# RunpeiDong/ACT

Hardware: AMD Instinct MI355X
Metric: stage2_pretrain_point_clouds_per_sec (higher is better)
Workload: dtype f32

## Files before the change

### act_amd/_abi.py

```python
import ctypes

_vp, _i, _f, _sz = ctypes.c_void_p, ctypes.c_int, ctypes.c_float, ctypes.c_size_t
_u, _u64, _ll, _str = ctypes.c_uint, ctypes.c_uint64, ctypes.c_longlong, ctypes.c_char_p
_d = ctypes.c_double
_P = ctypes.POINTER


class GemmEpilogue(ctypes.Structure):
    _fields_ = [("alpha", _f), ("act", _i), ("accumulate", _i), ("rows_per_scale", _i), ("ldr", _i), ("ldaux", _i),
                ("res_row_div", _i), ("bias", _vp), ("rowscale", _vp), ("res", _vp), ("aux", _vp)]


class GemmTnProblem(ctypes.Structure):
    _fields_ = [("A", _vp), ("lda", _i), ("B", _vp), ("ldb", _i), ("C", _vp), ("ldc", _i), ("M", _i), ("N", _i), ("bias_out", _vp)]


class GemmFx(ctypes.Structure):
    _fields_ = ([(n, _vp) for n in ("a_scale", "a_shift", "b_scale", "b_shift", "tile_stats", "gmax", "garg")] + [("group", _i), ("store_c", _i)]
                + [(n, _vp) for n in ("sa_src", "sa_arg", "ep_src", "ep_arg", "row_groups")])


class BlockParams(ctypes.Structure):
    _fields_ = [(n, _vp) for n in ("norm1_w", "norm1_b", "qkv_w", "qkv_b", "proj_w", "proj_b", "norm2_w", "norm2_b",
                                   "fc1_w", "fc1_b", "fc2_w", "fc2_b")]


class BlockDims(ctypes.Structure):
    _fields_ = [("B", _i), ("S", _i), ("D", _i), ("heads", _i), ("hidden", _i), ("eps", _f)]


class BlockStack(ctypes.Structure):
    _fields_ = [("depth", _i), ("blocks", _vp), ("gate1", _vp), ("gate2", _vp)]


class PrefixVit(ctypes.Structure):
    _fields_ = ([(n, _i) for n in ("B", "P", "G", "D", "heads", "hidden", "depth", "tokens_dims", "pos_hidden")] +
                [("eps", _f), ("drop_p", _f), ("seed_base", _u64), ("seed_dev", _vp)] +
                [(n, _vp) for n in ("pos_w0", "pos_b0", "pos_w1", "pos_b1", "pre_w", "pre_b", "post_w", "post_b", "norm_w", "norm_b")] +
                [("prompt_tok", _P(_vp)), ("prompt_pos", _P(_vp)), ("blocks", _P(BlockParams))])


class VitBf16x3(ctypes.Structure):
    _fields_ = [("w_planes", _vp), ("a_planes", _vp), ("a_planes_elems", _sz)]


class VitF16x3(ctypes.Structure):
    _fields_ = [("w_planes", _vp), ("w_inv_scale", _vp), ("a_scale", _vp), ("a_planes", _vp), ("a_planes_elems", _sz)]


class PointnetParams(ctypes.Structure):
    _fields_ = [(n, _vp) for n in ("c1_w", "c1_b", "bn1_w", "bn1_b", "c2_w", "c2_b", "c3_w", "c3_b", "bn2_w", "bn2_b", "c4_w", "c4_b",
                                   "bn1_mean", "bn1_var", "bn2_mean", "bn2_var")]


class PointnetGrads(ctypes.Structure):
    _fields_ = [(n, _vp) for n in ("c1_w", "c1_b", "bn1_w", "bn1_b", "c2_w", "c2_b", "c3_w", "c3_b", "bn2_w", "bn2_b", "c4_w", "c4_b")]


class PointnetDims(ctypes.Structure):
    _fields_ = [("BG", _i), ("n", _i), ("C", _i), ("eps1", _f), ("eps2", _f), ("momentum1", _f), ("momentum2", _f)]


class Dgcnn(ctypes.Structure):
    _fields_ = ([(n, _i) for n in ("B", "G", "k", "Cin", "Cout", "groups")] + [("eps", _f), ("slope", _f)] +
                [(n, _vp) for n in ("w_in", "b_in", "w5")] + [("stacked", _vp * 4), ("gn_w", _vp * 4), ("gn_b", _vp * 4)])


class DgcnnF16x3(ctypes.Structure):
    _fields_ = [("w5_planes", _vp), ("w5_inv_scale", _vp), ("a_scale", _f), ("a_planes", _vp), ("a_planes_elems", _sz), ("layers", _i),
                ("st_planes", _vp * 3), ("st_inv_scale", _vp * 3)]


class PointnetF16x3(ctypes.Structure):
    _fields_ = [("c4_planes", _vp), ("c4_inv_scale", _vp), ("a_scale", _f)]


class AugmentOp(ctypes.Structure):
    _fields_ = [("kind", _i), ("p0", _f), ("p1", _f), ("p2", _f), ("draws", _vp), ("draws2", _vp)]


STRUCTS = {
    "act_gemm_epilogue_t": GemmEpilogue, "act_gemm_tn_problem_t": GemmTnProblem, "act_gemm_fx_t": GemmFx,
    "act_block_params_t": BlockParams, "act_block_grads_t": BlockParams, "act_block_dims_t": BlockDims, "act_block_stack_t": BlockStack,
    "act_prefix_vit_t": PrefixVit, "act_vit_bf16x3_t": VitBf16x3, "act_vit_f16x3_t": VitF16x3,
    "act_pointnet_params_t": PointnetParams,
    "act_pointnet_grads_t": PointnetGrads, "act_pointnet_dims_t": PointnetDims, "act_dgcnn_t": Dgcnn, "act_dgcnn_f16x3_t": DgcnnF16x3,
    "act_pointnet_f16x3_t": PointnetF16x3,
    "act_augment_op_t": AugmentOp,
}

_epi, _probs, _fx = _P(GemmEpilogue), _P(GemmTnProblem), _P(GemmFx)
_dims, _blk, _x3 = _P(BlockDims), _P(BlockParams), _P(VitBf16x3)
_pnd, _pnp = _P(PointnetDims), _P(PointnetParams)

_TABLE = {
    "act_version": [],
    "act_arch": (_str, []),
    "act_prof_enable": [_i],
    "act_prof_reset": [],
    "act_prof_num_kernels": [],
    "act_prof_kernel_name": (_str, [_i]),
    "act_prof_read": [_i, _vp, _vp, _vp, _vp],
    "act_fps_scratch_floats": (_sz, [_i, _i]),
    "act_fps_f32": [_vp, _i, _i, _i, _vp, _vp, _i, _vp, _vp],
    "act_fps_chain_probe": [_i, _i, _vp, _vp, _vp, _vp],
    "act_knn_group_f32": [_vp, _vp, _i, _i, _i, _i, _vp, _i, _vp, _vp, _vp],
    "act_gather_points_f32": [_vp, _vp, _i, _i, _i, _i, _vp, _vp],
# ... 39 lines not shown
    "act_col_mean_var_f32": [_vp, _i, _i, _vp, _vp, _vp, _sz, _vp],
    "act_bn_bwd_sums_f32": [_vp, _vp, _vp, _vp, _vp, _vp, _i, _i, _i, _vp, _vp, _vp, _sz, _vp],
    "act_bn_bwd_apply_f32": [_vp, _vp, _vp, _vp, _vp, _vp, _vp, _vp, _f, _i, _i, _i, _vp, _vp],
    "act_group_max_f32": [_vp, _i, _i, _i, _vp, _vp, _vp],
    "act_group_max_bwd_f32": [_vp, _vp, _i, _i, _i, _i, _vp, _vp],
    "act_group_max_bwd_matmul_f32": [_vp, _vp, _i, _i, _i, _vp, _i, _i, _vp, _i, _vp],
    "act_group_live_i32": [_vp, _i, _i, _vp, _vp],
    "act_group_max_bwd_matmul_live_f32": [_vp, _vp, _i, _i, _i, _vp, _i, _i, _vp, _i, _vp, _vp],
    "act_group_max_bwd_wgrad_workspace": (_sz, [_i, _i, _i, _i]),
    "act_group_max_bwd_wgrad_f32": [_vp, _vp, _i, _i, _i, _vp, _i, _i, _vp, _vp, _vp, _i, _vp, _sz, _vp],
    "act_group_sum_f32": [_vp, _i, _i, _i, _vp, _vp],
    "act_edge_gn_lrelu_max_f32": [_vp, _i, _i, _vp, _i, _i, _i, _i, _i, _vp, _vp, _f, _f, _vp, _vp, _i, _i, _vp],
    "act_edge_gn_lrelu_max_bwd_f32": [_vp, _i, _i, _vp, _i, _i, _i, _i, _i, _vp, _vp, _vp, _f, _vp, _i, _vp, _vp, _vp, _vp],
    "act_edge_bwd_lds": [_i],
    "act_gn_gumbel_argmax_gather_f32": [_vp, _i, _i, _i, _i, _vp, _vp, _f, _f, _vp, _u64, _vp, _f, _vp, _i, _vp, _vp, _vp, _vp, _vp],
    "act_gumbel_softmax_fwd_f32": [_vp, _i, _i, _vp, _u64, _f, _vp, _vp],
    "act_gumbel_softmax_bwd_f32": [_vp, _vp, _i, _i, _f, _vp, _vp],
    "act_kl_uniform_fwd_f32": [_vp, _i, _i, _i, _vp, _vp, _vp, _vp],
    "act_kl_uniform_bwd_f32": [_vp, _vp, _vp, _vp, _i, _i, _i, _vp, _vp],
    "act_split_bf16x2_f32": [_vp, _i, _i, _i, _vp, _vp, _vp],
    "act_sgemm_nt_bf16x3_supported": [_i, _i, _i],
    "act_sgemm_nt_bf16x3_f32": [_i, _i, _i, _vp, _vp, _vp, _vp, _vp, _i, _epi, _vp],
    "act_layernorm_fwd_planes_f32": [_vp, _vp, _vp, _vp, _vp, _vp, _vp, _vp, _vp, _vp, _i, _i, _f, _vp],
    "act_prompt_layernorm_fwd_planes_f32": [_vp, _vp, _i, _i, _i, _f, _u64, _vp, _vp, _vp, _f, _vp, _vp, _vp],
    "act_attention_fwd_prefix_planes_f32": [_vp, _i, _vp, _i, _vp, _vp, _vp, _vp, _i, _i, _i, _f, _vp],
    "act_sgemm_nt_bf16x3_planes_f32": [_i, _i, _i, _vp, _vp, _vp, _vp, _vp, _i, _vp, _vp, _epi, _vp],
    "act_split_f16x2_f32": [_vp, _i, _i, _i, _f, _vp, _vp, _vp, _vp],
    "act_split_f16x2_ld_f32": [_vp, _i, _i, _i, _f, _vp, _vp, _i, _vp],
    "act_sgemm_nt_f16x3_supported": [_i, _i, _i],
    "act_sgemm_nt_f16x3_planes_f32": [_i, _i, _i, _vp, _vp, _f, _vp, _vp, _vp, _vp, _i, _vp, _vp, _f, _epi, _vp],
    "act_sgemm_nt_f16x3_pick_tile": [_i, _i, _i, _i],
    "act_sgemm_nt_f16x3_planes_tile_f32": [_i, _i, _i, _vp, _vp, _f, _vp, _vp, _vp, _vp, _i, _vp, _vp, _f, _epi, _vp, _i],
    "act_sgemm_nt_f16x3_planes_lda_f32": [_i, _i, _i, _vp, _vp, _i, _f, _vp, _vp, _vp, _vp, _i, _vp, _vp, _f, _epi, _vp, _i],
    "act_layernorm_fwd_f16_planes_f32": [_vp, _vp, _vp, _vp, _vp, _vp, _vp, _vp, _f, _vp, _vp, _i, _i, _f, _vp],
    "act_attention_fwd_prefix_f16_planes_f32": [_vp, _i, _vp, _i, _vp, _vp, _vp, _f, _vp, _i, _i, _i, _f, _vp],
    "act_prompt_layernorm_fwd_f16_planes_f32": [_vp, _vp, _i, _i, _i, _f, _u64, _vp, _vp, _vp, _f, _vp, _vp, _f, _vp],
    "act_split_f16x2_affine_relu_f32": [_vp, _i, _i, _i, _vp, _vp, _f, _vp, _vp, _vp],
    "act_sgemm_nt_f16x3_gmax_supported": [_i, _i, _i, _i],
    "act_sgemm_nt_f16x3_gmax_pick_tile": [_i, _i, _i, _i],
    "act_sgemm_nt_f16x3_gmax_f32": [_i, _i, _i, _vp, _i, _vp, _vp, _vp, _vp, _f, _vp, _vp, _vp, _vp, _i, _vp, _i, _i, _vp],
    "act_gemm_tune_set": [_i] * 7,
    "act_gemm_tune_get": [_i] * 5 + [_P(_i), _P(_i)],
    "act_gemm_tune_clear": [],
    "act_gemm_tile_info": [_i] + [_P(_i)] * 4,
    "act_scale_rows_f32": [_vp, _vp, _i, _i, _i, _vp, _vp],
    "act_bn_eval_affine_f32": [_vp, _vp, _vp, _vp, _f, _i, _vp, _vp, _vp],
    "act_composite_collect_begin": [],
    "act_composite_collect_end": [_P(_i), _i],
    "act_composite_shutdown": [],
    "act_block_saved_floats": (_sz, [_dims]),
    "act_block_fwd_f32": [_dims, _blk, _vp, _vp, _vp, _vp, _i, _vp, _vp, _vp, _sz, _vp],
    "act_block_bwd_scratch_floats": (_sz, [_dims]),
    "act_block_bwd_f32": [_dims, _blk, _vp, _vp, _vp, _vp, _vp, _blk, _vp, _vp, _sz, _vp, _sz, _vp, _vp],
    "act_block_stack_saved_floats": (_sz, [_dims, _i, _i]),
    "act_block_stack_bwd_scratch_floats": (_sz, [_dims, _i]),
    "act_block_stack_fwd_f32": [_dims, _P(BlockStack), _vp, _vp, _i, _vp, _vp, _vp, _sz, _vp],
    "act_block_stack_bwd_f32": [_dims, _P(BlockStack), _vp, _vp, _vp, _vp, _vp, _vp, _vp, _vp, _sz, _vp, _sz, _vp, _vp],
    "act_add_f32": [_vp, _vp, _vp, _ll, _vp],
    "act_prefix_block_saved_floats": (_sz, [_dims, _i]),
    "act_prefix_block_fwd_f32": [_dims, _i, _blk, _vp, _vp, _vp, _vp, _i, _vp, _vp, _vp, _sz, _vp],
    "act_prefix_block_fwd_kv_f32": [_dims, _i, _blk, _vp, _vp, _vp, _vp, _vp, _vp, _sz, _vp],
    "act_prompt_kv_sparse": [_i],
    "act_prompt_kv_workspace": (_sz, [_i, _i, _i, _i]),
    "act_prompt_kv_fwd_f32": [_vp, _vp, _i, _i, _i, _i, _f, _u64, _vp, _vp, _vp, _f, _vp, _vp, _vp, _vp, _sz, _vp, _sz, _vp],
    "act_prompt_kv_f16x3": [_i],
    "act_prompt_kv_fwd_f16x3_f32": [_vp, _vp, _i, _i, _i, _i, _f, _u64, _vp, _vp, _vp, _f, _vp, _vp, _vp, _f, _vp, _vp, _vp, _sz, _i, _vp],
    "act_prefix_block_bwd_scratch_floats": (_sz, [_dims, _i]),
    "act_prefix_block_bwd_f32": [_dims, _i, _blk, _vp, _vp, _vp, _vp, _vp, _vp, _vp, _sz, _vp],
    "act_prefix_vit_scratch_floats": (_sz, [_P(PrefixVit)]),
    "act_prefix_vit_fwd_bf16x3_f32": [_P(PrefixVit), _x3, _vp, _vp, _vp, _vp, _vp, _sz, _vp],
    "act_prefix_block_fwd_bf16x3_f32": [_dims, _i, _blk, _x3, _vp, _vp, _vp, _i, _vp, _vp, _vp, _sz, _vp],
    "act_prefix_block_bwd_bf16x3_f32": [_dims, _i, _blk, _x3, _vp, _vp, _vp, _vp, _vp, _vp, _vp, _sz, _vp],
    "act_prefix_vit_fwd_f32": [_P(PrefixVit), _vp, _vp, _vp, _vp, _vp, _sz, _vp],
    "act_prefix_vit_fwd_f16x3_f32": [_P(PrefixVit), _P(VitF16x3), _vp, _vp, _vp, _vp, _vp, _sz, _vp],
    "act_pointnet_saved_floats": (_sz, [_pnd]),
    "act_pointnet_fwd_f32": [_pnd, _pnp, _vp, _i, _i, _vp, _vp, _vp, _sz, _vp],
    "act_pointnet_fwd_groups_f32": [_pnd, _pnp, _vp, _i, _i, _vp, _vp, _vp, _i, _vp, _sz, _vp],
    "act_pointnet_fwd_groups_f16x3_f32": [_pnd, _pnp, _P(PointnetF16x3), _vp, _i, _i, _vp, _vp, _vp, _i, _vp, _sz, _vp],
    "act_pointnet_bwd_scratch_floats": (_sz, [_pnd]),
    "act_pointnet_bwd_f32": [_pnd, _pnp, _vp, _vp, _vp, _P(PointnetGrads), _vp, _vp, _sz, _vp],
    "act_dgcnn_scratch_floats": (_sz, [_P(Dgcnn)]),
    "act_dgcnn_features_f32": [_P(Dgcnn), _vp, _vp, _vp, _vp, _vp, _sz, _vp],
    "act_dgcnn_features_f16x3_f32": [_P(Dgcnn), _P(DgcnnF16x3), _vp, _vp, _vp, _vp, _vp, _sz, _vp],
    "act_log_softmax_fwd_f32": [_vp, _ll, _i, _vp, _vp],
    "act_log_softmax_bwd_f32": [_vp, _vp, _ll, _i, _vp, _vp],
    "act_nll_weighted_workspace": (_sz, [_ll]),
    "act_nll_weighted_fwd_f32": [_vp, _vp, _vp, _ll, _i, _vp, _vp, _vp, _vp, _sz, _vp],
    "act_nll_weighted_bwd_f32": [_vp, _vp, _vp, _vp, _ll, _i, _vp, _vp],
    "act_confusion_i64": [_vp, _vp, _ll, _i, _vp, _vp],
    "act_label_branch_fwd_f32": [_vp, _vp, _vp, _vp, _i, _i, _f, _f, _f, _vp, _vp, _vp, _vp],
    "act_label_branch_bwd_f32": [_vp, _vp, _vp, _vp, _vp, _i, _f, _f, _vp, _vp, _vp, _vp],
    "act_part_eval_f32": [_vp, _vp, _i, _i, _i, _vp, _vp, _i, _vp, _vp, _i, _i, _vp, _vp, _vp],
    "act_scene_member_workspace": (_sz, [_ll, _i, _i]),
    "act_scene_member_count": [_vp, _ll, _vp, _i, _i, _vp, _vp, _vp, _sz, _vp],
    "act_scene_member_fill": [_vp, _ll, _vp, _i, _i, _vp, _vp, _vp, _sz, _vp],
    "act_scene_rows": [_vp, _vp, _vp, _vp, _i, _ll, _i, _u, _u, _u, _vp, _vp],
    "act_scene_gather": [_vp, _ll, _vp, _vp, _vp, _vp, _i, _ll, _vp, _vp],
    "act_scene_vote": [_vp, _vp, _ll, _ll, _i, _vp, _vp, _vp, _vp],
    "act_scene_finish": [_vp, _vp, _ll, _i, _vp, _vp, _vp],
# ... 82 lines not shown
```

### act_amd/composite.py

```python
import ctypes
import math
import os
import weakref

import torch

from . import _C
from . import kernels as K
from ._abi import BlockDims, BlockParams, BlockStack, Dgcnn, PointnetDims, PointnetGrads, PointnetParams, PrefixVit, VitBf16x3, VitF16x3, DgcnnF16x3
from ._abi import PointnetF16x3
from ._abi import GemmFx

lib, check = _C.lib, _C.check
_vp, _i = ctypes.c_void_p, ctypes.c_int

ENABLED = os.environ.get("ACT_COMPOSITE", "1") != "0"


def _p(t):
    if t is None:
        return None
    if not t.is_cuda or not t.is_contiguous():
        raise _C.ActHipError("act_amd kernels need contiguous CUDA tensors (there is no CPU fallback)")
    _C._same_device(t)
# ... 198 lines not shown
        if dpos_in is not None:
            dpos_in = K._f32c(dpos_in).reshape(B * S, D)
        dpos = torch.empty(B, S, D, dtype=torch.float32, device=dev) if (ctx.has_pos and (depth > 1 or dpos_in is not None)) else None
        scratch = torch.empty(n_scratch, dtype=torch.float32, device=dev)
        grads, garr = (None,) * len(params), None
        if tw:
            grads = tuple(torch.empty_like(t) if t is not None else None for t in params)
            garr = _ptr_array(grads, dev.index)
        ws = K.workspace(dev)
        side, sws = None, None
        if tw == 2 and K.OVERLAP_DW:
            side = K.side_stream(dev, 1).cuda_stream
            sws = K.workspace(dev, stream_handle=side)
        args = (ctypes.byref(dims), ctypes.byref(st), saved.data_ptr(), dout.data_ptr(), dx.data_ptr(), dpos.data_ptr() if dpos is not None else None,
                dpos_in.data_ptr() if (dpos_in is not None and dpos is not None) else None,
                ctypes.cast(garr, _vp) if garr is not None else None, scratch.data_ptr(), ws.data_ptr(), ws.numel() * 4,
                sws.data_ptr() if sws is not None else None, (sws.numel() * 4 if sws is not None else 0))
        ensure_tuned(("stack_bwd", B, S, D, heads, hidden, depth, bool(tw)), lambda: lib.act_block_stack_bwd_f32(*args, _C.stream(), side), dev)
        check(lib.act_block_stack_bwd_f32(*args, _C.stream(), side), "act_block_stack_bwd_f32")
        return (dx, (dpos if dpos is not None else dx) if ctx.has_pos else None, None, None, None, None, None) + grads


_LEAVES = weakref.WeakKeyDictionary()
_VIT_LEAVES = weakref.WeakKeyDictionary()
_VIT_STRUCT = weakref.WeakKeyDictionary()
_VIT_PLANES = weakref.WeakKeyDictionary()
TEACHER_BF16X3 = os.environ.get("ACT_TEACHER_BF16X3", "0") == "1"
TEACHER_BF16X3_BWD = os.environ.get("ACT_TEACHER_BF16X3_BWD", "1") == "1"
TEACHER_F16X3 = os.environ.get("ACT_TEACHER_F16X3", "1") != "0"
_VIT_F16 = weakref.WeakKeyDictionary()
TOKENIZER_F16X3 = os.environ.get("ACT_TOKENIZER_F16X3", "1") != "0"
TOKENIZER_PN_F16X3 = os.environ.get("ACT_TOKENIZER_PN_F16X3", "1") != "0"
TOKENIZER_DGCNN_F16X3 = os.environ.get("ACT_TOKENIZER_DGCNN_F16X3", "1") != "0"
DGCNN_F16X3_MIN_T = 4096
_PN_F16 = weakref.WeakKeyDictionary()
_DGCNN_F16 = weakref.WeakKeyDictionary()


def _stack_leaves(blocks):
    cache = _LEAVES.get(blocks)
    if cache is None or len(cache) != len(blocks) or any(c[6] is not b for c, b in zip(cache, blocks)):
        cache = _LEAVES[blocks] = [(b.norm1, b.attn.qkv, b.attn.proj, b.norm2, b.mlp.fc1, b.mlp.fc2, b) for b in blocks]
    return cache


def _stock_blocks(blocks):
    from act_amd.models.act import Block
    for b in blocks:
        if type(b).forward is not Block.forward or b._forward_hooks or b._forward_pre_hooks or b._backward_hooks or b._backward_pre_hooks:
            return False
    return True


def block_stack(blocks, x, pos, gates, draws=None, tag="enc", chunk=None, taps=False):
    n = len(blocks)

    def per_block(x, draws):
        outs = []
        every = chunk if chunk else n
        for i, blk in enumerate(blocks):
            x = blk(x, pos, draws, f"{tag}.{i}", gates[i] if gates is not None else None)
            if (i + 1) % every == 0 or i == n - 1:
                outs.append(x)
        return outs if taps else x
    if not (ENABLED and STACK) or n == 0 or not _stock_blocks(blocks):
        return per_block(x, draws)
# ... 204 lines not shown
    if cache is None or cache[0] != sig:
        with torch.no_grad():
            planes = [K.split_bf16x2(w.detach()) for w in ws_]
        parr = (_vp * len(planes))(*[pl.data_ptr() for pl in planes])
        cache = _VIT_PLANES[tok] = (sig, planes, parr)
    a_planes = torch.empty(2 * act_elems, dtype=torch.bfloat16, device=dev)
    x3 = VitBf16x3(ctypes.cast(cache[2], _vp), a_planes.data_ptr(), a_planes.numel())
    return x3, (a_planes, cache)


def f16x3_act_scale(bound):
    bound = float(bound)
    if not math.isfinite(bound) or bound > 32768.0:
        return 0.0
    if bound < 2.0 ** -15:
        return 2.0 ** 30
    s = 2.0 ** (math.frexp(32768.0 / bound)[1] - 1)
    return s if bound * s <= 32768.0 else s / 2


def f16x3_vit_bounds(ts, depth, D):
    rows, rt = [], math.sqrt(D)
    for i in range(depth):
        n1w, n1b, wqkv, bqkv, _, _, n2w, n2b, w1, b1 = (None if t is None else t.detach().double() for t in ts[10 + _NPB * i: 20 + _NPB * i])
        u1, u2 = rt * n1w.abs() + n1b.abs(), rt * n2w.abs() + n2b.abs()
        v = wqkv[2 * D:].abs() @ u1 + (bqkv[2 * D:].abs() if bqkv is not None else 0)
        h = w1.abs() @ u2 + (b1.abs() if b1 is not None else 0)
        rows.append(torch.stack([u1.max(), v.max(), u2.max(), h.max()]))
    return torch.stack(rows)


def _vit_f16_planes(tok, ts, depth, act_elems, dev):
    blk = ts[10:10 + _NPB * depth]
    sig = tuple((t.data_ptr(), t._version) if t is not None else None for t in blk)
    cache = _VIT_F16.get(tok)
    if cache is None or cache[0] != sig:
        ws_ = [ts[10 + _NPB * i + j] for i in range(depth) for j in (2, 4, 8, 10)]
        with torch.no_grad():
            scales = [K.f16x3_row_scales(w) for w in ws_]
            planes = [K.split_f16x2(w.detach(), 1.0, sc[0]) for w, sc in zip(ws_, scales)]
            inv = [sc[1].contiguous() for sc in scales]
            a_scale = [f16x3_act_scale(b) for b in f16x3_vit_bounds(ts, depth, ws_[0].shape[1]).flatten().tolist()]
        parr = (_vp * len(planes))(*[pl.data_ptr() for pl in planes])
        iarr = (_vp * len(inv))(*[t.data_ptr() for t in inv])
        sarr = (ctypes.c_float * len(a_scale))(*a_scale)
        cache = _VIT_F16[tok] = (sig, planes, inv, a_scale, (parr, iarr, sarr))
    a_planes = torch.empty(2 * act_elems, dtype=torch.float16, device=dev)
    parr, iarr, sarr = cache[4]
    x3 = VitF16x3(ctypes.cast(parr, _vp), ctypes.cast(iarr, _vp), ctypes.cast(sarr, _vp), a_planes.data_ptr(), a_planes.numel())
    return x3, (a_planes, cache)


def _pointnet_structs(enc, BG, n):
    c1, bn1, _, c2 = enc.first_conv
    c3, bn2, _, c4 = enc.second_conv
    dims = PointnetDims(BG, n, c4.weight.shape[0], float(bn1.eps), float(bn2.eps), float(bn1.momentum), float(bn2.momentum))
    return dims, (c1, bn1, c2, c3, bn2, c4)


class PointnetFn(torch.autograd.Function):

    @staticmethod
    def forward(ctx, x, c1w, c1b, g1, b1, c2w, c2b, c3w, c3b, g2, b2, c4w, c4b, buffers, dims, training, groups=None, x3=None):
        dev = x.device
        x = K._f32c(x)
        need_grad = any(ctx.needs_input_grad)
        prm = PointnetParams(*[_p(t) for t in (c1w, c1b, g1, b1, c2w, c2b, c3w, c3b, g2, b2, c4w, c4b) + tuple(buffers)])
        saved = torch.empty(int(lib.act_pointnet_saved_floats(ctypes.byref(dims))), dtype=torch.float32, device=dev)
        out = torch.empty(dims.BG, dims.C, dtype=torch.float32, device=dev)
        ws = K.workspace(dev)
        ng = 0 if groups is None else int(groups.numel())
        args = (ctypes.byref(dims), ctypes.byref(prm), _p(x), int(training), int(need_grad), _p(saved), _p(out),
                _p(groups) if ng else None, ng, _p(ws), ws.numel() * 4)
        ensure_tuned(("pn_fwd", dims.BG, dims.n, dims.C, ng), lambda: lib.act_pointnet_fwd_groups_f32(*args, _C.stream()), dev)
        if x3 is not None and not need_grad:
            check(lib.act_pointnet_fwd_groups_f16x3_f32(args[0], args[1], ctypes.byref(x3), *args[2:], _C.stream()), "act_pointnet_fwd_groups_f16x3_f32")
        else:
            check(lib.act_pointnet_fwd_groups_f32(*args, _C.stream()), "act_pointnet_fwd_groups_f32")
        if need_grad:
            ctx.save_for_backward(x, saved, c1w, c1b, g1, b1, c2w, c2b, c3w, c3b, g2, b2, c4w, c4b)
            ctx.dims, ctx.training = dims, bool(training)
        return out

    @staticmethod
    def backward(ctx, dout):
        if not ctx.training:
            raise NotImplementedError("mini-PointNet backward in eval mode (running statistics) is off the training path")
        x, saved = ctx.saved_tensors[:2]
        params = ctx.saved_tensors[2:]
        dims = ctx.dims
        dev = dout.device
        dout = K._f32c(dout)
        prm = PointnetParams(*([_p(t) for t in params] + [None] * 4))
        grads = tuple(torch.empty_like(t) for t in params)
        gp = PointnetGrads(*[_p(g) for g in grads])
        scratch = torch.empty(int(lib.act_pointnet_bwd_scratch_floats(ctypes.byref(dims))), dtype=torch.float32, device=dev)
        ws = K.workspace(dev)
        args = (ctypes.byref(dims), ctypes.byref(prm), _p(x), _p(saved), _p(dout), ctypes.byref(gp), _p(scratch), _p(ws), ws.numel() * 4)
        ensure_tuned(("pn_bwd", dims.BG, dims.n, dims.C), lambda: lib.act_pointnet_bwd_f32(*args, _C.stream()), dev)
        check(lib.act_pointnet_bwd_f32(*args, _C.stream()), "act_pointnet_bwd_f32")
        return (None,) + grads + (None, None, None, None, None)


def f16x3_pointnet_bound(gmax, bmax, R):
    return math.sqrt(R) * gmax + bmax


def _pointnet_f16_planes(enc, R):
    bn2, c4 = enc.second_conv[1], enc.second_conv[3]
    sig = tuple((t.data_ptr(), t._version) for t in (c4.weight, bn2.weight, bn2.bias))
    cache = _PN_F16.get(enc)
    if cache is None or cache[0] != sig:
        with torch.no_grad():
            w = c4.weight.detach().reshape(c4.weight.shape[0], c4.weight.shape[1])
            scale, inv = K.f16x3_row_scales(w)
            planes = K.split_f16x2(w, 1.0, scale)
            inv = inv.contiguous()
            gmax, bmax = torch.stack([bn2.weight.detach().double().abs().max(), bn2.bias.detach().double().abs().max()]).tolist()
        cache = _PN_F16[enc] = (sig, planes, inv, gmax, bmax, {})
    _, planes, inv, gmax, bmax, scales = cache
    a_scale = scales.get(R)
    if a_scale is None:
        a_scale = scales[R] = f16x3_act_scale(f16x3_pointnet_bound(gmax, bmax, R))
    return PointnetF16x3(planes.data_ptr(), inv.data_ptr(), a_scale), cache


def pointnet_forward(enc, point_groups, need=None):
    bs, g, n, _ = point_groups.shape
    groups = None
    if need is not None and need.shape[1] < g and n in (32, 64):
        ids = (need + torch.arange(bs, device=need.device).unsqueeze(1) * g).reshape(-1).to(torch.int32)
        pad = (-ids.numel()) % (128 // n)
        groups = torch.cat([ids, ids[-1:].expand(pad)]) if pad else ids
        groups = groups.contiguous()
    dims, (c1, bn1, c2, c3, bn2, c4) = _pointnet_structs(enc, bs * g, n)
    training = enc.training
    if training:
        for bn in (bn1, bn2):
            if bn.num_batches_tracked is not None:
                bn.num_batches_tracked.add_(1)
    w2 = lambda c: c.weight.view(c.weight.shape[0], c.weight.shape[1])
    x3 = keep = None
    if (TOKENIZER_PN_F16X3 and groups is None and training and not torch.is_grad_enabled()
            and not any(p.requires_grad for p in enc.parameters())):
        x3, keep = _pointnet_f16_planes(enc, bs * g * n)
    out = PointnetFn.apply(point_groups.reshape(bs * g * n, 3), w2(c1), c1.bias, bn1.weight, bn1.bias, w2(c2), c2.bias, w2(c3), c3.bias,
                           bn2.weight, bn2.bias, w2(c4), c4.bias,
                           (bn1.running_mean, bn1.running_var, bn2.running_mean, bn2.running_var), dims, training, groups, x3)
    del keep
    return out.reshape(bs, g, dims.C)


def dgcnn_features(dg, f, idx, stacked):
    B, G, Cin = f.shape
    dev = f.device
    w5 = dg.layer5[0].weight
    m = Dgcnn()
    gn0 = dg.layer1[1]
    m.B, m.G, m.k, m.Cin, m.Cout, m.groups = B, G, idx.shape[1], Cin, w5.shape[0], gn0.num_groups
    m.eps, m.slope = float(gn0.eps), 0.2
    m.w_in, m.b_in, m.w5 = _p(dg.input_trans.weight), _p(dg.input_trans.bias), _p(w5)
    for l, layer in enumerate((dg.layer1, dg.layer2, dg.layer3, dg.layer4)):
        m.stacked[l], m.gn_w[l], m.gn_b[l] = _p(stacked[l]), _p(layer[1].weight), _p(layer[1].bias)
    scratch = torch.empty(int(lib.act_dgcnn_scratch_floats(ctypes.byref(m))), dtype=torch.float32, device=dev)
    h = torch.empty(B * G, m.Cout, dtype=torch.float32, device=dev)
    ws = K.workspace(dev)
    f = K._f32c(f)
    args = (ctypes.byref(m), _p(f), _p(idx), _p(h), _p(scratch), _p(ws), ws.numel() * 4)
    ensure_tuned(("dgcnn", B, G, Cin, m.Cout), lambda: lib.act_dgcnn_features_f32(*args, _C.stream()), dev)
    head, layers = TOKENIZER_F16X3 and m.Cout >= 1024, TOKENIZER_DGCNN_F16X3 and B * G >= DGCNN_F16X3_MIN_T
    if head or layers:
        x3, keep = _dgcnn_f16_planes(dg, B * G, G, m.k, dev, head=head, layers=layers)
        check(lib.act_dgcnn_features_f16x3_f32(args[0], ctypes.byref(x3), *args[1:], _C.stream()), "act_dgcnn_features_f16x3_f32")
        del keep
        return h
    check(lib.act_dgcnn_features_f32(*args, _C.stream()), "act_dgcnn_features_f32")
    return h


def f16x3_dgcnn_bound(gmax, bmax, couts, groups, G, k):
    return max(math.sqrt((c // g) * G * k) * gm + bm for gm, bm, c, g in zip(gmax, bmax, couts, groups))


def _dgcnn_f16_planes(dg, T, G, k, dev, head=True, layers=None):
    if layers is None:
        layers = TOKENIZER_DGCNN_F16X3 and T >= DGCNN_F16X3_MIN_T
    convs = [layer[0] for layer in (dg.layer2, dg.layer3, dg.layer4)]
    gns = [layer[1] for layer in (dg.layer1, dg.layer2, dg.layer3, dg.layer4)]
    w5 = dg.layer5[0].weight
    sig = tuple((t.data_ptr(), t._version) for t in [w5] + [t for gn in gns for t in (gn.weight, gn.bias)] + [c.weight for c in convs])
    cache = _DGCNN_F16.get(dg)
    if cache is None or cache[0] != sig:
        with torch.no_grad():
            mx = torch.stack([t.detach().double().abs().max() for gn in gns for t in (gn.weight, gn.bias)]).tolist()
        cache = _DGCNN_F16[dg] = [sig, None, None, mx[0::2], mx[1::2], [gn.num_channels for gn in gns], [gn.num_groups for gn in gns], {}, None]

    def planes_of(w):
        scale, inv = K.f16x3_row_scales(w)
        return K.split_f16x2(w, 1.0, scale), inv.contiguous()
    if head and cache[1] is None:
        with torch.no_grad():
            cache[1], cache[2] = planes_of(w5.detach().reshape(w5.shape[0], w5.shape[1]))
    if layers and cache[8] is None:
        with torch.no_grad():
            cache[8] = [planes_of(dg._stacked_weight(c).detach()) for c in convs]
    _, planes, inv, gmax, bmax, couts, groups, scales, st = cache
    a_scale = scales.get((G, k))
    if a_scale is None:
        a_scale = scales[(G, k)] = f16x3_act_scale(f16x3_dgcnn_bound(gmax, bmax, couts, groups, G, k))
    a_planes = torch.empty(2 * T * sum(couts), dtype=torch.float16, device=dev)
    x3 = DgcnnF16x3(planes.data_ptr() if head else None, inv.data_ptr() if head else None, a_scale, a_planes.data_ptr(), a_planes.numel())
    if layers:
        x3.layers = 1
        for i, (p, v) in enumerate(st):
            x3.st_planes[i], x3.st_inv_scale[i] = p.data_ptr(), v.data_ptr()
    return x3, (a_planes, cache)
```

### act_amd/csrc/composite.hip

```cpp
#include "common.h"
#include "split_planes.h"
#include <atomic>
#include <mutex>
#include <unordered_map>
#include <vector>
#include <stdlib.h>

#define CK(expr) do { const int rc__ = (expr); if (rc__ != 0) return rc__; } while (0)
#define RUN(expr) do { if (!t_collect) { const int rc__ = (expr); if (rc__ != 0) return rc__; } } while (0)

namespace {

struct GemmShape { int ak, bk, M, N, K; };
thread_local std::vector<GemmShape>* t_collect = nullptr;
inline bool collecting(int ak, int bk, int M, int N, int K) {
    if (!t_collect) return false;
    t_collect->push_back({ak, bk, M, N, K});
    return true;
}

struct EventRing {
    std::vector<hipEvent_t> ev;
    size_t next = 0;
    hipEvent_t get() {
// ... 57 lines not shown
    return c.used;
}
struct BlockBwdScratch { float *dy2, *dh, *dn2, *dx1, *dy1, *datt, *dqkv, *dn1; };
size_t carve_block_bwd(float* base, const act_block_dims_t& d, BlockBwdScratch& sc) {
    const size_t T = (size_t)d.B * d.S, D = d.D, Hd = d.hidden;
    Carver c(base);
    sc.dy2 = c.take(T * D); sc.dh = c.take(T * Hd); sc.dn2 = c.take(T * D); sc.dx1 = c.take(T * D); sc.dy1 = c.take(T * D);
    sc.datt = c.take(T * D); sc.dqkv = c.take(T * 3 * D); sc.dn1 = c.take(T * D);
    return c.used;
}
bool bad_dims(const act_block_dims_t* d) {
    return !d || d->B <= 0 || d->S <= 0 || d->D <= 0 || d->heads <= 0 || d->D % d->heads || d->hidden <= 0;
}

struct PrefixSaved { float *n1p, *meanp, *rstdp, *kvp, *xin, *n1x, *mean1, *rstd1, *qkvx, *att, *lse, *x1, *n2, *mean2, *rstd2, *hpre, *a; };
size_t carve_prefix(float* base, const act_block_dims_t& d, int P, PrefixSaved& sv) {
    const size_t TG = (size_t)d.B * d.S, TP = (size_t)d.B * P, D = d.D, Hd = d.hidden;
    Carver c(base);
    sv.n1p = c.take(TP * D); sv.kvp = c.take(TP * 2 * D); sv.xin = c.take(TG * D); sv.n1x = c.take(TG * D); sv.qkvx = c.take(TG * 3 * D);
    sv.att = c.take(TG * D); sv.x1 = c.take(TG * D); sv.n2 = c.take(TG * D); sv.hpre = c.take(TG * Hd); sv.a = c.take(TG * Hd);
    sv.meanp = c.take(TP); sv.rstdp = c.take(TP); sv.mean1 = c.take(TG); sv.rstd1 = c.take(TG); sv.mean2 = c.take(TG); sv.rstd2 = c.take(TG);
    sv.lse = c.take((size_t)d.B * d.heads * d.S);
    return c.used;
}
struct PrefixBwdScratch { float *dh, *dn2, *dx1, *datt, *dkvp, *dqkvx, *dn1x, *dn1p; };
size_t carve_prefix_bwd(float* base, const act_block_dims_t& d, int P, PrefixBwdScratch& sc) {
    const size_t TG = (size_t)d.B * d.S, TP = (size_t)d.B * P, D = d.D, Hd = d.hidden;
    Carver c(base);
    sc.dh = c.take(TG * Hd); sc.dn2 = c.take(TG * D); sc.dx1 = c.take(TG * D); sc.datt = c.take(TG * D); sc.dkvp = c.take(TP * 2 * D);
    sc.dqkvx = c.take(TG * 3 * D); sc.dn1x = c.take(TG * D); sc.dn1p = c.take(TP * D);
    return c.used;
}

struct X3Linear { const uint16_t *w1, *w2; const float* inv; PlaneFmt a_fmt; };
inline X3Linear x3_linear_of(const uint16_t* planes, size_t plane_elems, PlaneFmt a_fmt, const float* inv = nullptr) {
    return X3Linear{planes, planes ? planes + plane_elems : nullptr, inv, a_fmt};
}
inline bool x3_takes(const X3Linear& l, int M, int N, int K) {
    return l.w1 && (l.a_fmt.is_f16() ? act_sgemm_nt_f16x3_supported(M, N, K) : act_sgemm_nt_bf16x3_supported(M, N, K));
}
int x3_split(PlaneFmt fmt, const float* A, int M, int K, uint16_t* dst, hipStream_t s) {
    if (fmt.is_f16()) return act_split_f16x2_f32(A, M, K, K, fmt.f16_scale, nullptr, dst, dst + (size_t)M * K, s);
    return act_split_bf16x2_f32(A, M, K, K, dst, dst + (size_t)M * K, s);
}
int x3_multiply(const X3Linear& l, int M, int N, int K, const uint16_t* a, float* C, uint16_t* emit, PlaneFmt emit_fmt, const act_gemm_epilogue_t& e,
                hipStream_t s) {
    const uint16_t* a2 = a + (size_t)M * K; uint16_t* emit2 = emit ? emit + (size_t)M * N : nullptr;
    if (l.a_fmt.is_f16())
        return act_sgemm_nt_f16x3_planes_f32(M, N, K, a, a2, l.a_fmt.f16_scale, l.w1, l.w2, l.inv, emit ? nullptr : C, N, emit, emit2,
                                             emit ? emit_fmt.f16_scale : 0.f, &e, s);
    return act_sgemm_nt_bf16x3_planes_f32(M, N, K, a, a2, l.w1, l.w2, emit ? nullptr : C, N, emit, emit2, &e, s);
}
int x3_linear(const X3Linear& l, int M, int N, int K, const float* A, const uint16_t* pre, uint16_t* stage, float* C, uint16_t* emit, PlaneFmt emit_fmt,
              const act_gemm_epilogue_t& e, hipStream_t s) {
    if (t_collect) return 0;
    if (!pre) CK(x3_split(l.a_fmt, A, M, K, stage, s));
    return x3_multiply(l, M, N, K, pre ? pre : stage, C, emit, emit_fmt, e, s);
}
int x3_layernorm(PlaneFmt fmt, const float* x, const float* pos, const float* gamma, const float* beta, float* xin_out, uint16_t* dst, float* mean, float* rstd,
                 int T, int D, float eps, hipStream_t s) {
    uint16_t* dst2 = dst + (size_t)T * D;
    if (fmt.is_f16()) return act_layernorm_fwd_f16_planes_f32(x, pos, gamma, beta, xin_out, nullptr, dst, dst2, fmt.f16_scale, mean, rstd, T, D, eps, s);
    return act_layernorm_fwd_planes_f32(x, pos, gamma, beta, xin_out, nullptr, dst, dst2, mean, rstd, T, D, eps, s);
}
int x3_attention(PlaneFmt fmt, const float* kvp, int P, const float* qkvx, int G, float* att, uint16_t* dst, float* lse, int B, int H, int hd, hipStream_t s) {
    uint16_t* dst2 = dst + (size_t)B * G * H * hd;
    if (fmt.is_f16()) return act_attention_fwd_prefix_f16_planes_f32(kvp, P, qkvx, G, att, dst, dst2, fmt.f16_scale, lse, B, H, hd, attn_scale(hd), s);
    return act_attention_fwd_prefix_planes_f32(kvp, P, qkvx, G, att, dst, dst2, lse, B, H, hd, attn_scale(hd), s);
}

struct X3Block { X3Linear kv, qkv, proj, fc1, fc2; uint16_t* a_planes; size_t a_elems; bool n1p_is_planes; };
inline X3Block x3_block_bf16(const act_block_dims_t& d, const uint16_t* const* w_planes, uint16_t* a_planes, size_t a_elems) {
    const size_t D = d.D, Hd = d.hidden; const PlaneFmt bf = PlaneFmt::bf16();
    X3Block b{};
    b.qkv = x3_linear_of(w_planes[0], 3 * D * D, bf); b.proj = x3_linear_of(w_planes[1], D * D, bf);
    b.fc1 = x3_linear_of(w_planes[2], Hd * D, bf); b.fc2 = x3_linear_of(w_planes[3], D * Hd, bf);
    if (b.qkv.w1) b.kv = X3Linear{b.qkv.w1 + D * D, b.qkv.w2 + D * D, nullptr, bf};
    b.a_planes = a_planes; b.a_elems = a_elems;
    return b;
}
inline bool x3_fits(const act_block_dims_t& d, int P, size_t a_elems) {
    const size_t TG = (size_t)d.B * d.S, TP = (size_t)d.B * P;
    return a_elems >= 2 * TG * d.hidden + 2 * (TG > TP ? TG : TP) * d.D;
}
constexpr int kPromptKvTile = 0;

int prefix_block_core(const act_block_dims_t& d, int P, const act_block_params_t& w, const float* x, const float* pos, const float* n1p,
                      bool keep, PrefixSaved& sv, float* out, float* ws, size_t wsb, hipStream_t s, const X3Block* x3 = nullptr, bool kvp_ready = false) {
    const int B = d.B, G = d.S, D = d.D, H = d.heads, hd = D / H, Hd = d.hidden, TG = B * G, TP = B * P;
    static const X3Block none{};
    const X3Block& b = (x3 && x3_fits(d, P, x3->a_elems)) ? *x3 : none;
    uint16_t* tmp =b.a_planes ? b.a_planes + (size_t)2 * TG * Hd : nullptr;
    uint16_t* qkv_in = x3_takes(b.qkv, TG, 3 * D, D) ? tmp : nullptr;
    uint16_t* proj_in = x3_takes(b.proj, TG, D, D) ? tmp : nullptr;
    uint16_t* fc1_in = x3_takes(b.fc1, TG, Hd, D) ? tmp : nullptr;
    uint16_t* fc2_in = (fc1_in && x3_takes(b.fc2, TG, D, Hd)) ? b.a_planes : nullptr;
    const X3Linear fc2 = fc2_in ? b.fc2 : X3Linear{};
    auto linear = [&](const X3Linear& l, int M, int N, int K, const float* A, const float* W, float* C, const act_gemm_epilogue_t& e,
                      const uint16_t* pre = nullptr, uint16_t* emit = nullptr, const X3Linear* next = nullptr) -> int {
        if (x3_takes(l, M, N, K)) return x3_linear(l, M, N, K, A, pre, tmp, C, emit, next ? next->a_fmt : PlaneFmt::bf16(), e, s);
        return gemm_nt(M, N, K, A, K, W, K, C, N, e, ws, wsb, s);
    };
    float *mean1 = keep ? sv.mean1 : nullptr, *rstd1 = keep ? sv.rstd1 : nullptr, *mean2 = keep ? sv.mean2 : nullptr, *rstd2 = keep ? sv.rstd2 : nullptr;
    float* lse = keep ? sv.lse : nullptr;
    act_gemm_epilogue_t e = epi0();
    e.bias = w.qkv_b ? w.qkv_b + D : nullptr;
    if (!kvp_ready) CK(linear(b.kv, TP, 2 * D, D, n1p, w.qkv_w + (size_t)D * D, sv.kvp, e, b.n1p_is_planes ? tmp : nullptr));
    RUN(qkv_in ? x3_layernorm(b.qkv.a_fmt, x, pos, w.norm1_w, w.norm1_b, sv.xin, qkv_in, mean1, rstd1, TG, D, d.eps, s)
               : act_layernorm_fwd_f32(x, pos, w.norm1_w, w.norm1_b, sv.xin, sv.n1x, mean1, rstd1, TG, D, d.eps, s));
    e = epi0(); e.bias = w.qkv_b;
    CK(linear(b.qkv, TG, 3 * D, D, sv.n1x, w.qkv_w, sv.qkvx, e, qkv_in));
    RUN(proj_in ? x3_attention(b.proj.a_fmt, sv.kvp, P, sv.qkvx, G, keep ? sv.att : nullptr, proj_in, lse, B, H, hd, s)
                : act_attention_fwd_prefix_f32(sv.kvp, P, sv.qkvx, G, sv.att, lse, B, H, hd, attn_scale(hd), s));
    e = epi0(); e.bias = w.proj_b; e.res = sv.xin; e.ldr = D;
    CK(linear(b.proj, TG, D, D, sv.att, w.proj_w, sv.x1, e, proj_in));
    RUN(fc1_in ? x3_layernorm(b.fc1.a_fmt, sv.x1, nullptr, w.norm2_w, w.norm2_b, nullptr, fc1_in, mean2, rstd2, TG, D, d.eps, s)
               : act_layernorm_fwd_f32(sv.x1, nullptr, w.norm2_w, w.norm2_b, nullptr, sv.n2, mean2, rstd2, TG, D, d.eps, s));
    e = epi0(); e.bias = w.fc1_b; e.act = ACT_EPI_GELU; e.aux = keep ? sv.hpre : nullptr; e.ldaux = Hd;
    CK(linear(b.fc1, TG, Hd, D, sv.n2, w.fc1_w, sv.a, e, fc1_in, fc2_in, &fc2));
    e = epi0(); e.bias = w.fc2_b; e.res = sv.x1; e.ldr = D;
    CK(linear(fc2, TG, D, Hd, sv.a, w.fc2_w, out, e, fc2_in));
    return 0;
}

}

extern "C" {

int act_composite_shutdown(void) {
    std::lock_guard<std::mutex> g(g_ring_mu);
    int n = 0;
    for (auto& kv : g_rings)
        for (hipEvent_t e : kv.second.ev) { (void)hipEventDestroy(e); ++n; }
    g_rings.clear();
    return n;
}

int act_composite_collect_begin(void) {
    if (t_collect) return ACT_E_BADARG;
    t_collect = new std::vector<GemmShape>();
    return 0;
}
int act_composite_collect_end(int* shapes, int max) {
    if (!t_collect) return ACT_E_BADARG;
    const int n = (int)t_collect->size();
    for (int i = 0; i < n && i < max && shapes; ++i) {
        const GemmShape& g = (*t_collect)[i];
        shapes[5 * i] = g.ak; shapes[5 * i + 1] = g.bk; shapes[5 * i + 2] = g.M; shapes[5 * i + 3] = g.N; shapes[5 * i + 4] = g.K;
    }
    delete t_collect; t_collect = nullptr;
    return n;
}

size_t act_block_saved_floats(const act_block_dims_t* d) {
// ... 181 lines not shown
    if (!w || !x || !saved || !out || !kvp) return ACT_E_NULLPTR;
    if (bad_dims(d) || P <= 0) return ACT_E_BADARG;
    PrefixSaved sv; carve_prefix(saved, *d, P, sv);
    sv.kvp = const_cast<float*>(kvp);
    return prefix_block_core(*d, P, *w, x, pos, nullptr, false, sv, out, ws, wsb, (hipStream_t)stream, nullptr, true);
}

static std::atomic<int> g_prompt_kv_sparse{[] { const char* e = getenv("ACT_PROMPT_KV_SPARSE"); return !(e && e[0] == '0') ? 1 : 0; }()};
int act_prompt_kv_sparse(int on) { return on < 0 ? g_prompt_kv_sparse.load() : g_prompt_kv_sparse.exchange(on ? 1 : 0); }
size_t act_prompt_kv_workspace(int B, int P, int D, int N) {
    if (!act_prompt_kv_shape_ok(B, P, D, N)) return 0;
    ActPromptKvWs w; act_prompt_kv_carve(nullptr, B, P, D, N, w);
    return w.floats * sizeof(float);
}
int act_prompt_kv_fwd_f32(const float* tok, const float* ppos, int B, int P, int D, int N, float drop_p, uint64_t seed, const uint64_t* seed_dev,
                          const float* gamma, const float* beta, float eps, const float* W, const float* bias, float* kvp, float* scratch,
                          size_t scratch_bytes, float* ws, size_t wsb, act_stream_t stream) {
    if (!tok || !ppos || !gamma || !beta || !W || !kvp) return ACT_E_NULLPTR;
    if (B < 0 || P <= 0 || D <= 0 || N <= 0 || drop_p < 0.f || drop_p >= 1.f) return ACT_E_BADARG;
    if (!g_prompt_kv_sparse.load() || !act_prompt_kv_shape_ok(B ? B : 1, P, D, N) || (reinterpret_cast<uintptr_t>(W) & 15)) return ACT_E_UNSUPPORTED;
    if (B == 0) return 0;
    ActPromptKvWs pw; act_prompt_kv_carve(scratch, B, P, D, N, pw);
    if (!scratch) return ACT_E_NULLPTR;
    if (scratch_bytes < pw.floats * sizeof(float) || (reinterpret_cast<uintptr_t>(scratch) & 15)) return ACT_E_BADARG;
    hipStream_t s = (hipStream_t)stream;
    RUN(act_prompt_kv_rows(tok, ppos, B, P, D, drop_p, seed, seed_dev, gamma, beta, eps, pw, s));
    CK(gemm_nt(P + 2, N, D, pw.arows, D, W, D, pw.base, N, epi0(), ws, wsb, s));
    RUN(act_prompt_kv_correct(tok, B, P, D, N, drop_p, gamma, W, bias, pw, kvp, s));
    return 0;
}

static std::atomic<int> g_prompt_kv_f16x3{[] { const char* e = getenv("ACT_PROMPT_KV_F16X3"); return !(e && e[0] == '0') ? 1 : 0; }()};
int act_prompt_kv_f16x3(int on) { return on < 0 ? g_prompt_kv_f16x3.load() : g_prompt_kv_f16x3.exchange(on ? 1 : 0); }
int act_prompt_kv_fwd_f16x3_f32(const float* tok, const float* ppos, int B, int P, int D, int N, float drop_p, uint64_t seed, const uint64_t* seed_dev,
                                const float* gamma, const float* beta, float eps, const uint16_t* w_h1, const uint16_t* w_h2, const float* w_inv,
                                float a_scale, const float* bias, float* kv, uint16_t* planes, size_t planes_elems, int tile, act_stream_t stream) {
    if (B <= 0 || P <= 0 || D <= 0 || N <= 0) return ACT_E_BADARG;
    const size_t rows = (size_t)B * P;
    if (!g_prompt_kv_f16x3.load() || !(a_scale > 0.f) || !w_h1 || !w_h2 || !w_inv || !planes || planes_elems < 2 * rows * (size_t)D ||
        rows > (size_t)0x7fffffff || !act_sgemm_nt_f16x3_supported((int)rows, N, D))
        return ACT_E_UNSUPPORTED;
    if (!tok || !ppos || !gamma || !beta || !kv) return ACT_E_NULLPTR;
    if (drop_p < 0.f || drop_p >= 1.f || (tile != 0 && tile != 128 && !(tile == 192 && N % 192 == 0)) ||
        (((uintptr_t)planes | (uintptr_t)w_h1 | (uintptr_t)w_h2 | (uintptr_t)w_inv) & 15))
        return ACT_E_BADARG;
    uint16_t* p2 = planes + rows * D;
    RUN(act_prompt_layernorm_fwd_f16_planes_f32(tok, ppos, B, P, D, drop_p, seed, seed_dev, gamma, beta, eps, planes, p2, a_scale, stream));
    act_gemm_epilogue_t e = epi0(); e.bias = bias;
    RUN(act_sgemm_nt_f16x3_planes_tile_f32((int)rows, N, D, planes, p2, a_scale, w_h1, w_h2, w_inv, kv, N, nullptr, nullptr, 0.f, &e, stream, tile));
    return 0;
}

int act_prefix_block_fwd_bf16x3_f32(const act_block_dims_t* d, int P, const act_block_params_t* w, const act_vit_bf16x3_t* x3, const float* x, const float* pos,
                                    const float* prm, int keep_for_backward, float* saved, float* out, float* ws, size_t wsb, act_stream_t stream) {
    if (!w || !x || !saved || !out || !prm || !x3 || !x3->w_planes || !x3->a_planes) return ACT_E_NULLPTR;
    if (bad_dims(d) || P <= 0) return ACT_E_BADARG;
    hipStream_t s = (hipStream_t)stream;
    const bool keep = keep_for_backward != 0;
    PrefixSaved sv; carve_prefix(saved, *d, P, sv);
    X3Block xb = x3_block_bf16(*d, x3->w_planes, x3->a_planes, x3->a_planes_elems);
    const int TP = d->B * P, D = d->D;
    if (x3_fits(*d, P, xb.a_elems) && x3_takes(xb.kv, TP, 2 * D, D)) {
        uint16_t* tp = xb.a_planes + (size_t)2 * d->B * d->S * d->hidden;
        RUN(x3_layernorm(xb.kv.a_fmt, prm, nullptr, w->norm1_w, w->norm1_b, nullptr, tp, keep ? sv.meanp : nullptr, keep ? sv.rstdp : nullptr, TP, D, d->eps, s));
        xb.n1p_is_planes = true;
    } else {
        RUN(act_layernorm_fwd_f32(prm, nullptr, w->norm1_w, w->norm1_b, nullptr, sv.n1p, keep ? sv.meanp : nullptr, keep ? sv.rstdp : nullptr, TP, D, d->eps, s));
    }
    return prefix_block_core(*d, P, *w, x, pos, sv.n1p, keep, sv, out, ws, wsb, s, &xb);
}

int act_prefix_block_bwd_f32(const act_block_dims_t* d, int P, const act_block_params_t* w, const float* prm, const float* saved,
                             const float* dout, float* dx, float* dprm, float* scratch, float* ws, size_t wsb, act_stream_t stream) {
    if (!w || !prm || !saved || !dout || !dx || !dprm || !scratch) return ACT_E_NULLPTR;
    if (bad_dims(d) || P <= 0) return ACT_E_BADARG;
    hipStream_t s = (hipStream_t)stream;
    const int B = d->B, G = d->S, D = d->D, H = d->heads, hd = D / H, Hd = d->hidden, TG = B * G, TP = B * P;
    PrefixSaved sv; carve_prefix(const_cast<float*>(saved), *d, P, sv);
    PrefixBwdScratch sc; carve_prefix_bwd(scratch, *d, P, sc);
    act_gemm_epilogue_t e = epi0(); e.act = ACT_EPI_MUL_GELU_GRAD; e.aux = sv.hpre; e.ldaux = Hd;
    CK(gemm_nn(TG, Hd, D, dout, D, w->fc2_w, Hd, sc.dh, Hd, e, ws, wsb, s));
    CK(gemm_nn(TG, D, Hd, sc.dh, Hd, w->fc1_w, D, sc.dn2, D, epi0(), ws, wsb, s));
// ... 47 lines not shown
    act_block_dims_t d{m.B, m.G, m.D, m.heads, m.hidden, m.eps};
    PrefixSaved sv;
    Carver c(base);
    pos_h = c.take(TG * m.pos_hidden); pos = c.take(TG * D); xa = c.take(TG * D); xb = c.take(TG * D); n1p = c.take(TP * D); feat = c.take(TG * D);
    blk = c.take(carve_prefix(nullptr, d, m.P, sv));
    float* kv_scratch = c.take(act_prompt_kv_workspace(m.B, m.P, m.D, 2 * m.D) / sizeof(float));
    if (pkv) *pkv = kv_scratch;
    return c.used;
}
static bool bad_vit(const act_prefix_vit_t* m) {
    return !m || m->B <= 0 || m->P <= 0 || m->G <= 0 || m->D <= 0 || m->heads <= 0 || m->D % m->heads || m->hidden <= 0 || m->depth <= 0 ||
           m->tokens_dims <= 0 || m->pos_hidden <= 0;
}
size_t act_prefix_vit_scratch_floats(const act_prefix_vit_t* m) {
    if (bad_vit(m)) return 0;
    float *a, *b, *c, *d, *e, *f, *g;
    return carve_vit(nullptr, *m, a, b, c, d, e, f, g);
}

static int prefix_vit_fwd(const act_prefix_vit_t* m, const act_vit_bf16x3_t* x3, const act_vit_f16x3_t* h3, const float* tokens, const float* center, float* out,
                          float* scratch, float* ws, size_t wsb, act_stream_t stream);
int act_prefix_vit_fwd_f32(const act_prefix_vit_t* m, const float* tokens, const float* center, float* out, float* scratch, float* ws,
                           size_t wsb, act_stream_t stream) {
    return prefix_vit_fwd(m, nullptr, nullptr, tokens, center, out, scratch, ws, wsb, stream);
}
int act_prefix_vit_fwd_bf16x3_f32(const act_prefix_vit_t* m, const act_vit_bf16x3_t* x3, const float* tokens, const float* center, float* out,
                                  float* scratch, float* ws, size_t wsb, act_stream_t stream) {
    if (!x3 || !x3->w_planes || !x3->a_planes) return ACT_E_NULLPTR;
    return prefix_vit_fwd(m, x3, nullptr, tokens, center, out, scratch, ws, wsb, stream);
}
int act_prefix_vit_fwd_f16x3_f32(const act_prefix_vit_t* m, const act_vit_f16x3_t* h3, const float* tokens, const float* center, float* out,
                                 float* scratch, float* ws, size_t wsb, act_stream_t stream) {
    if (!h3 || !h3->w_planes || !h3->w_inv_scale || !h3->a_scale || !h3->a_planes) return ACT_E_NULLPTR;
    return prefix_vit_fwd(m, nullptr, h3, tokens, center, out, scratch, ws, wsb, stream);
}
static int prefix_vit_fwd(const act_prefix_vit_t* m, const act_vit_bf16x3_t* x3, const act_vit_f16x3_t* h3, const float* tokens, const float* center, float* out,
                          float* scratch, float* ws, size_t wsb, act_stream_t stream) {
    if (bad_vit(m)) return ACT_E_BADARG;
    if (!tokens || !center || !out || !scratch || !m->blocks || !m->prompt_tok || !m->prompt_pos) return ACT_E_NULLPTR;
    hipStream_t s = (hipStream_t)stream;
    const int TG = m->B * m->G, D = m->D;
    float *pos_h, *pos, *xa, *xb, *n1p, *blk, *feat, *pkv;
    carve_vit(scratch, *m, pos_h, pos, xa, xb, n1p, blk, feat, &pkv);
    const size_t pkv_bytes = act_prompt_kv_workspace(m->B, m->P, m->D, 2 * m->D);
    const act_block_dims_t d{m->B, m->G, m->D, m->heads, m->hidden, m->eps};
    PrefixSaved sv; carve_prefix(blk, d, m->P, sv);
    act_gemm_epilogue_t e = epi0(); e.bias = m->pos_b0; e.act = ACT_EPI_GELU;
    CK(gemm_nt(TG, m->pos_hidden, 3, center, 3, m->pos_w0, 3, pos_h, m->pos_hidden, e, ws, wsb, s));
    e = epi0(); e.bias = m->pos_b1;
    CK(gemm_nt(TG, D, m->pos_hidden, pos_h, m->pos_hidden, m->pos_w1, m->pos_hidden, pos, D, e, ws, wsb, s));
    e = epi0(); e.bias = m->pre_b;
    CK(gemm_nt(TG, D, m->tokens_dims, tokens, m->tokens_dims, m->pre_w, m->tokens_dims, xa, D, e, ws, wsb, s));
    float* cur = xa; float* nxt = xb;
    for (int i = 0; i < m->depth; ++i) {
        const act_block_params_t& w = m->blocks[i];
        const uint64_t seed = (m->seed_base + 7919ull * (uint64_t)(i + 1)) & ((1ull << 62) - 1);
        X3Block hb{};
        if (h3) {
            hb.a_planes = h3->a_planes; hb.a_elems = h3->a_planes_elems;
            const size_t sD = D, sHd = m->hidden, elems[4] = {3 * sD * sD, sD * sD, sHd * sD, sD * sHd};
            X3Linear* lin[4] = {&hb.qkv, &hb.proj, &hb.fc1, &hb.fc2};
            for (int j = 0; j < 4; ++j) {
                const float sa = h3->a_scale[4 * i + j];
                if (sa > 0.f && h3->w_planes[4 * i + j] && h3->w_inv_scale[4 * i + j])
                    *lin[j] = x3_linear_of(h3->w_planes[4 * i + j], elems[j], PlaneFmt::f16(sa), h3->w_inv_scale[4 * i + j]);
            }
            if (hb.qkv.w1) hb.kv = X3Linear{hb.qkv.w1 + sD * sD, hb.qkv.w2 + sD * sD, hb.qkv.inv + sD, hb.qkv.a_fmt};
        }
        if (h3 && !x3) {
            uint16_t* tp = x3_fits(d, m->P, hb.a_elems) ? hb.a_planes + (size_t)2 * TG * m->hidden : nullptr;
            const int rc = act_prompt_kv_fwd_f16x3_f32(m->prompt_tok[i], m->prompt_pos[i], m->B, m->P, D, 2 * D, m->drop_p, seed, m->seed_dev, w.norm1_w, w.norm1_b,
                                                       m->eps, hb.kv.w1, hb.kv.w2, hb.kv.inv, hb.kv.a_fmt.f16_scale, w.qkv_b ? w.qkv_b + D : nullptr, sv.kvp, tp,
                                                       tp ? hb.a_elems - (size_t)2 * TG * m->hidden : 0, kPromptKvTile, stream);
            if (rc == 0) {
                (void)collecting(1, 1, m->B * m->P, 2 * D, D);
                CK(prefix_block_core(d, m->P, w, cur, pos, nullptr, false, sv, nxt, ws, wsb, s, &hb, true));
                float* t = cur; cur = nxt; nxt = t;
                continue;
            }
            if (rc != ACT_E_UNSUPPORTED) return rc;
        }
        if (!x3) {
            const int rc = act_prompt_kv_fwd_f32(m->prompt_tok[i], m->prompt_pos[i], m->B, m->P, D, 2 * D, m->drop_p, seed, m->seed_dev, w.norm1_w, w.norm1_b,
                                                 m->eps, w.qkv_w + (size_t)D * D, w.qkv_b ? w.qkv_b + D : nullptr, sv.kvp, pkv, pkv_bytes, ws, wsb, stream);
            if (rc == 0) {
                (void)collecting(1, 1, m->B * m->P, 2 * D, D);
                CK(prefix_block_core(d, m->P, w, cur, pos, nullptr, false, sv, nxt, ws, wsb, s, h3 ? &hb : nullptr, true));
                float* t = cur; cur = nxt; nxt = t;
                continue;
            }
            if (rc != ACT_E_UNSUPPORTED) return rc;
        }
        X3Block xb{};
        if (x3) xb = x3_block_bf16(d, x3->w_planes + 4 * i, x3->a_planes, x3->a_planes_elems);
        if (x3 && x3_fits(d, m->P, x3->a_planes_elems) && x3_takes(xb.kv, m->B * m->P, 2 * D, D)) {
            uint16_t* tp = x3->a_planes + (size_t)2 * TG * m->hidden;
            RUN(act_prompt_layernorm_fwd_planes_f32(m->prompt_tok[i], m->prompt_pos[i], m->B, m->P, D, m->drop_p, seed, m->seed_dev, w.norm1_w, w.norm1_b,
                                                   m->eps, tp, tp + (size_t)m->B * m->P * D, s));
            xb.n1p_is_planes = true;
        } else
        RUN(act_prompt_layernorm_fwd_f32(m->prompt_tok[i], m->prompt_pos[i], m->B, m->P, D, m->drop_p, seed, m->seed_dev, w.norm1_w, w.norm1_b,
                                        m->eps, n1p, s));
        CK(prefix_block_core(d, m->P, w, cur, pos, n1p, false, sv, nxt, ws, wsb, s, x3 ? &xb : (h3 ? &hb : nullptr)));
        float* t = cur; cur = nxt; nxt = t;
    }
    RUN(act_layernorm_fwd_f32(cur, nullptr, m->norm_w, m->norm_b, nullptr, feat, nullptr, nullptr, TG, D, m->eps, s));
// ... 115 lines not shown
        CK(gemm_nt(1, 512, 256, w->c2_b, 256, w->c3_w + 256, 512, sv.b32, 512, epi0(), ws, wsb, s));
    }
    e = epi0(); e.bias = w->c3_b;
    CK(gemm_nt(BG, 512, 256, sv.fg, 256, w->c3_w, 512, sv.gw, 512, e, ws, wsb, s));
    e = epi0(); e.res = sv.gw; e.ldr = 512; e.res_row_div = n;
    if (!fused) {
        CK(gemm_nt(R, 512, 256, sv.h2, 256, w->c3_w + 256, 512, sv.h3, 512, e, ws, wsb, s));
        CK(stats(sv.h3, 512, w->bn2_w, w->bn2_b, w->bn2_mean, w->bn2_var, d->eps2, d->momentum2, sv.st2));
        RUN(act_affine_act_f32(sv.h3, scale2, shift2, 1, R, 512, sv.a3, s));
        e = epi0(); e.bias = w->c4_b;
        CK(gemm_nt(R, C, 512, sv.a3, 512, w->c4_w, 512, sv.h4, C, e, ws, wsb, s));
        RUN(act_group_max_f32(sv.h4, BG, n, C, out, keep_for_backward ? sv.arg2 : nullptr, s));
        return 0;
    }
    if (composed) {
        e.bias = sv.b32;
        act_gemm_fx_t fx{}; fx.a_scale = scale1; fx.a_shift = shift1; fx.tile_stats = training ? sv.tstats : nullptr; fx.store_c = 1;
        CK(gemm_fx(1, 1, R, 512, 128, sv.h1, 128, sv.w32, 128, sv.h3, 512, e, fx, ws, wsb, s));
        if (training) RUN(act_bn_tiles_finalize_f32(sv.tstats, R / 128, 128, 512, w->bn2_w, w->bn2_b, d->eps2, d->momentum2, w->bn2_mean, w->bn2_var, sv.st2,
                                                    sv.st2 + 512, scale2, shift2, s));
        else RUN(act_bn_eval_affine_f32(w->bn2_w, w->bn2_b, w->bn2_mean, w->bn2_var, d->eps2, 512, scale2, shift2, s));
    } else if (training) {
        act_gemm_fx_t fx{}; fx.tile_stats = sv.tstats; fx.store_c = 1;
        CK(gemm_fx(1, 1, R, 512, 256, sv.h2, 256, w->c3_w + 256, 512, sv.h3, 512, e, fx, ws, wsb, s));
        RUN(act_bn_tiles_finalize_f32(sv.tstats, R / 128, 128, 512, w->bn2_w, w->bn2_b, d->eps2, d->momentum2, w->bn2_mean, w->bn2_var, sv.st2, sv.st2 + 512,
                                      scale2, shift2, s));
    } else {
        CK(gemm_nt(R, 512, 256, sv.h2, 256, w->c3_w + 256, 512, sv.h3, 512, e, ws, wsb, s));
        RUN(act_bn_eval_affine_f32(w->bn2_w, w->bn2_b, w->bn2_mean, w->bn2_var, d->eps2, 512, scale2, shift2, s));
    }
    if (x3 && x3->c4_planes && x3->c4_inv_scale && x3->a_scale > 0.f && !keep_for_backward && !groups && C % 128 == 0 &&
        act_sgemm_nt_f16x3_gmax_supported(R, C, 512, n)) {
        if (collecting(1, 1, R, C, 512)) return 0;
        return act_sgemm_nt_f16x3_gmax_f32(R, C, 512, sv.h3, 512, scale2, shift2, nullptr, nullptr, x3->a_scale, x3->c4_planes,
                                           x3->c4_planes + (size_t)C * 512, x3->c4_inv_scale, w->c4_b, n, out, C, 0, s);
    }
    {
        act_gemm_fx_t fx{}; fx.a_scale = scale2; fx.a_shift = shift2; fx.gmax = out; fx.garg = keep_for_backward ? sv.arg2 : nullptr; fx.group = n; fx.store_c = 0;
        e = epi0(); e.bias = w->c4_b;
        if (groups) {
            if (!t_collect) {
                if (hipMemsetAsync(out, 0, (size_t)BG * C * sizeof(float), s) != hipSuccess) return ACT_E_BADARG;
                if (keep_for_backward && hipMemsetAsync(sv.arg2, 0xFF, (size_t)BG * C * sizeof(int32_t), s) != hipSuccess) return ACT_E_BADARG;
            }
            fx.row_groups = groups;
            CK(gemm_fx(1, 1, n_groups * n, C, 512, sv.h3, 512, w->c4_w, 512, nullptr, C, e, fx, ws, wsb, s));
        } else {
            CK(gemm_fx(1, 1, R, C, 512, sv.h3, 512, w->c4_w, 512, nullptr, C, e, fx, ws, wsb, s));
        }
    }
    return 0;
}

int act_pointnet_bwd_f32(const act_pointnet_dims_t* d, const act_pointnet_params_t* w, const float* x, const float* saved, const float* dout,
                         const act_pointnet_grads_t* g, float* scratch, float* ws, size_t wsb, act_stream_t stream) {
    if (!w || !x || !saved || !dout || !g || !scratch) return ACT_E_NULLPTR;
    if (bad_pn(d)) return ACT_E_BADARG;
    hipStream_t s = (hipStream_t)stream;
    const int BG = d->BG, n = d->n, C = d->C, R = BG * n;
    const bool fused = pn_fused(*d), composed = pn_compose(*d);
    PnSaved sv; carve_pn(const_cast<float*>(saved), *d, sv);
    PnBwdScratch sc; carve_pn_bwd(scratch, *d, sc);
    auto st = [](float* base, int Cc, int which) { return base + which * Cc; };
    auto wgrad_act = [&](const float* dy, int N_, const float* h, const float* a, float* stt, int Cc, float* dw) -> int {
        if (!fused) return gemm_tn(N_, Cc, R, dy, N_, a, Cc, dw, Cc, ws, wsb, s);
        if (N_ % 128 == 0 && Cc % 128 == 0) {
            act_gemm_fx_t fx{}; fx.b_scale = st(stt, Cc, 2); fx.b_shift = st(stt, Cc, 3);
            return gemm_fx(0, 0, N_, Cc, R, dy, N_, h, Cc, dw, Cc, epi0(), fx, ws, wsb, s);
// ... 29 lines not shown
    CK(gemm_tn(512, 256, BG, sc.dgw, 512, sv.fg, 256, g->c3_w, 512, ws, wsb, s));
    CK(colsum(sc.dgw, BG, 512, g->c3_b, ws, wsb, s));
    CK(gemm_nn(BG, 256, 512, sc.dgw, 512, w->c3_w, 512, sc.dfg, 256, epi0(), ws, wsb, s));
    if (composed) {
        act_gemm_epilogue_t ea = epi0(); ea.accumulate = 1;
        CK(wgrad_act(sc.dh3, 512, sv.h1, nullptr, sv.st1, 128, sc.g32));
        CK(gemm_nt(512, 256, 128, sc.g32, 128, w->c2_w, 128, g->c3_w + 256, 512, epi0(), ws, wsb, s));
        CK(gemm_nt(512, 256, 1, g->c3_b, 1, w->c2_b, 1, g->c3_w + 256, 512, ea, ws, wsb, s));
        RUN(act_group_max_bwd_wgrad_f32(sc.dfg, sv.arg1, BG, n, 256, sv.h1, 128, 128, st(sv.st1, 128, 2), st(sv.st1, 128, 3), g->c2_w, 128, ws, wsb, s));
        CK(gemm_tn(256, 128, 512, w->c3_w + 256, 512, sc.g32, 128, g->c2_w, 128, ea, ws, wsb, s));
        CK(colsum(sc.dfg, BG, 256, g->c2_b, ws, wsb, s));
        CK(gemm_nn(1, 256, 512, g->c3_b, 512, w->c3_w + 256, 512, g->c2_b, 256, ea, ws, wsb, s));
        RUN(act_group_max_bwd_matmul_live_f32(sc.dfg, sv.arg1, BG, n, 256, w->c2_w, 128, 128, sc.da1, 128, nullptr, s));
        CK(gemm_nn(R, 128, 512, sc.dh3, 512, sv.w32, 128, sc.da1, 128, ea, ws, wsb, s));
    } else {
        if (pool_on_load) {
            act_gemm_fx_t fe{}; fe.ep_src = sc.dfg; fe.ep_arg = sv.arg1; fe.group = n;
            CK(gemm_fx(1, 0, R, 256, 512, sc.dh3, 512, w->c3_w + 256, 512, sc.dh2, 256, epi0(), fe, ws, wsb, s));
        } else {
            CK(gemm_nn(R, 256, 512, sc.dh3, 512, w->c3_w + 256, 512, sc.dh2, 256, epi0(), ws, wsb, s));
            RUN(act_group_max_bwd_f32(sc.dfg, sv.arg1, BG, n, 256, 1, sc.dh2, s));
        }
        CK(wgrad_act(sc.dh2, 256, sv.h1, sv.a1, sv.st1, 128, g->c2_w));
        CK(colsum(sc.dh2, R, 256, g->c2_b, ws, wsb, s));
        CK(gemm_nn(R, 128, 256, sc.dh2, 256, w->c2_w, 128, sc.da1, 128, epi0(), ws, wsb, s));
    }
    RUN(act_bn_bwd_f32(sv.h1, sc.da1, st(sv.st1, 128, 2), st(sv.st1, 128, 3), st(sv.st1, 128, 0), st(sv.st1, 128, 1), 1, R, 128, sc.dh1, g->bn1_w, g->bn1_b,
                       ws, wsb, s));
    CK(gemm_tn(128, 3, R, sc.dh1, 128, x, 3, g->c1_w, 3, ws, wsb, s));
    CK(colsum(sc.dh1, R, 128, g->c1_b, ws, wsb, s));
    return 0;
}

static const int kDgcnnCin[4] = {128, 256, 512, 512}, kDgcnnCout[4] = {256, 512, 512, 1024};
static size_t carve_dgcnn(float* base, const act_dgcnn_t& m, float*& x0, float*& yz, float*& cat, float*& stats) {
    const size_t T = (size_t)m.B * m.G;
    Carver c(base);
    x0 = c.take(T * 128); yz = c.take(T * 2048); cat = c.take(T * 2304); stats = c.take((size_t)18 * m.B * m.groups);
    return c.used;
}
size_t act_dgcnn_scratch_floats(const act_dgcnn_t* m) {
    if (!m || m->B <= 0 || m->G <= 0 || m->groups <= 0) return 0;
    float *a, *b, *c, *d; return carve_dgcnn(nullptr, *m, a, b, c, d);
}
static int dgcnn_features(const act_dgcnn_t* m, const act_dgcnn_f16x3_t* x3, const float* f, const int64_t* idx, float* h, float* scratch, float* ws, size_t wsb,
                          act_stream_t stream);
int act_dgcnn_features_f32(const act_dgcnn_t* m, const float* f, const int64_t* idx, float* h, float* scratch, float* ws, size_t wsb,
                           act_stream_t stream) {
    return dgcnn_features(m, nullptr, f, idx, h, scratch, ws, wsb, stream);
}
int act_dgcnn_features_f16x3_f32(const act_dgcnn_t* m, const act_dgcnn_f16x3_t* x3, const float* f, const int64_t* idx, float* h, float* scratch,
                                 float* ws, size_t wsb, act_stream_t stream) {
    return dgcnn_features(m, x3, f, idx, h, scratch, ws, wsb, stream);
}
static int dgcnn_features(const act_dgcnn_t* m, const act_dgcnn_f16x3_t* x3, const float* f, const int64_t* idx, float* h, float* scratch, float* ws, size_t wsb,
                          act_stream_t stream) {
    if (!m || !f || !idx || !h || !scratch) return ACT_E_NULLPTR;
    if (m->B <= 0 || m->G <= 0 || m->k <= 0 || m->Cin <= 0 || m->Cout <= 0 || m->groups <= 0) return ACT_E_BADARG;
    hipStream_t s = (hipStream_t)stream;
    const int T = m->B * m->G;
    float *x0, *yz, *cat, *stats;
    carve_dgcnn(scratch, *m, x0, yz, cat, stats);
    const bool planes_ok = x3 && x3->a_planes && x3->a_scale > 0.f && x3->a_planes_elems >= (size_t)2 * T * 2304 && T % 128 == 0 &&
                           ((uintptr_t)x3->a_planes & 15) == 0;
    bool layers = planes_ok && x3->layers;
    for (int l = 1; layers && l < 4; ++l)
        layers = x3->st_planes[l - 1] && x3->st_inv_scale[l - 1] && act_sgemm_nt_f16x3_supported(T, 2 * kDgcnnCout[l], kDgcnnCin[l]);
    const bool head = planes_ok && x3->w5_planes && x3->w5_inv_scale && act_sgemm_nt_f16x3_supported(T, m->Cout, 2304) &&
                      (layers || !x3->layers);
    uint16_t* const ap1 = planes_ok ? x3->a_planes : nullptr;
    uint16_t* const ap2 = planes_ok ? x3->a_planes + (size_t)T * 2304 : nullptr;
    act_gemm_epilogue_t e = epi0(); e.bias = m->b_in;
    CK(gemm_nt(T, 128, m->Cin, f, m->Cin, m->w_in, m->Cin, x0, 128, e, ws, wsb, s));
    const float* xin = x0; int ldx = 128, off = 0;
    for (int l = 0; l < 4; ++l) {
        const int cin = kDgcnnCin[l], cout = kDgcnnCout[l];
        if (layers && l > 0 && !t_collect) {
            const size_t prev = (size_t)(off - cin);
            const uint16_t* w1 = x3->st_planes[l - 1];
            const act_gemm_epilogue_t e0 = epi0();
            RUN(act_sgemm_nt_f16x3_planes_lda_f32(T, 2 * cout, cin, ap1 + prev, ap2 + prev, 2304, x3->a_scale, w1, w1 + (size_t)2 * cout * cin,
                                                  x3->st_inv_scale[l - 1], yz, 2 * cout, nullptr, nullptr, 0.f, &e0, s, 0));
        } else {
            CK(gemm_nt(T, 2 * cout, cin, xin, ldx, m->stacked[l], cin, yz, 2 * cout, epi0(), ws, wsb, s));
        }
        RUN(act_edge_gn_lrelu_max_f32(yz, 2 * cout, cout, idx, m->B, m->G, m->k, cout, m->groups, m->gn_w[l], m->gn_b[l], m->eps, m->slope, stats,
                                     cat, 2304, off, s));
        if (layers && (l < 3 || head) && !t_collect)
            RUN(act_split_f16x2_ld_f32(cat + off, T, cout, 2304, x3->a_scale, ap1 + off, ap2 + off, 2304, s));
        xin = cat + off; ldx = 2304; off += cout;
    }
    if (head) {
        const X3Linear w5 = x3_linear_of(x3->w5_planes, (size_t)m->Cout * 2304, PlaneFmt::f16(x3->a_scale), x3->w5_inv_scale);
        return x3_linear(w5, T, m->Cout, 2304, cat, layers ? x3->a_planes : nullptr, x3->a_planes, h, nullptr, w5.a_fmt, epi0(), s);
    }
    CK(gemm_nt(T, m->Cout, 2304, cat, 2304, m->w5, 2304, h, m->Cout, epi0(), ws, wsb, s));
    return 0;
}

}
```

### act_amd/csrc/gemm_bf16x3.hip

```cpp
#include "gemm_common.h"
#include "split_planes.h"
#include <stdlib.h>

typedef short bf16x8 __attribute__((ext_vector_type(8)));
typedef _Float16 f16x8 __attribute__((ext_vector_type(8)));
typedef unsigned u32x4v __attribute__((ext_vector_type(4)));

namespace {

__device__ __forceinline__ float4 x3_affine_relu4(const float4& a, const float4& sc, const float4& sh) {
    return make_float4(fmaxf(__builtin_fmaf(a.x, sc.x, sh.x), 0.f), fmaxf(__builtin_fmaf(a.y, sc.y, sh.y), 0.f),
                       fmaxf(__builtin_fmaf(a.z, sc.z, sh.z), 0.f), fmaxf(__builtin_fmaf(a.w, sc.w, sh.w), 0.f));
}
__device__ __forceinline__ float4 x3_scale4(const float4& a, float s) { return make_float4(a.x * s, a.y * s, a.z * s, a.w * s); }

template <bool F16, bool AFF = false>
__global__ __launch_bounds__(256) void split_planes_kernel(const float* __restrict__ x, int K4, int ldx, int ldp4, long long n4, float scale,
                                                           const float* __restrict__ row_scale, unsigned short* __restrict__ p1, unsigned short* __restrict__ p2,
                                                           const float* __restrict__ col_scale = nullptr, const float* __restrict__ col_shift = nullptr) {
    for (long long i = (long long)blockIdx.x * blockDim.x + threadIdx.x; i < n4; i += (long long)gridDim.x * blockDim.x) {
        const long long row = i / K4; const int c4 = (int)(i - row * K4);
        const float4 v = *reinterpret_cast<const float4*>(x + row * ldx + c4 * 4);
        const size_t o4 = (size_t)(row * ldp4 + c4);
        if constexpr (AFF) {
            const float4 sc = x3_scale4(*reinterpret_cast<const float4*>(col_scale + c4 * 4), scale), sh = x3_scale4(*reinterpret_cast<const float4*>(col_shift + c4 * 4), scale);
            store_planes4<F16>(p1, p2, o4, x3_affine_relu4(v, sc, sh), 1.0f);
        } else {
            store_planes4<F16>(p1, p2, o4, v, F16 && row_scale ? scale * row_scale[row] : scale);
        }
    }
}

constexpr int BK = 32;
constexpr int LROW = 40;

struct X3Params {
    const unsigned short *Ah, *Al, *Bh, *Bl;
    float* C; int ldc;
    unsigned short *Oh, *Ol;
    int M, N, K;
    act_gemm_epilogue_t epi;
    const float* b_inv; float a_inv, o_scale;
    const float *A32, *a_sc, *a_sh; int lda; float a_fold;
    int group;
};

__device__ __forceinline__ void x3_affine_split8(const u32x4v& a0, const u32x4v& a1, const float* sc, const float* sh, u32x4v& h1, u32x4v& h2) {
#pragma unroll
    for (int half = 0; half < 2; ++half) {
        const float4 c = *reinterpret_cast<const float4*>(sc + half * (LROW / 2)), s = *reinterpret_cast<const float4*>(sh + half * (LROW / 2));
        const float4 v = x3_affine_relu4(__builtin_bit_cast(float4, half ? a1 : a0), c, s);
        const float e[4] = {v.x, v.y, v.z, v.w};
        unsigned h[4], l[4];
#pragma unroll
        for (int j = 0; j < 4; ++j) split_f16x2(e[j], h[j], l[j]);
        h1[2 * half] = h[0] | (h[1] << 16); h1[2 * half + 1] = h[2] | (h[3] << 16);
        h2[2 * half] = l[0] | (l[1] << 16); h2[2 * half + 1] = l[2] | (l[3] << 16);
        __builtin_amdgcn_sched_barrier(0);
    }
}

template <bool F16>
__device__ __forceinline__ f32x4 x3_mfma(const bf16x8& b, const bf16x8& a, const f32x4& c) {
    if constexpr (F16) return __builtin_amdgcn_mfma_f32_16x16x32_f16(__builtin_bit_cast(f16x8, b), __builtin_bit_cast(f16x8, a), c, 0, 0, 0);
    else return __builtin_amdgcn_mfma_f32_16x16x32_bf16(b, a, c, 0, 0, 0);
}

constexpr int x3_wgs_per_cu(int waves) { return waves <= 4 ? 2 : 1; }

template <int BM, int BN, int WGM, int WGN, int ACT, bool PLANES, bool F16, bool A32 = false, bool GMAX = false>
__global__ __launch_bounds__(64 * WGM * WGN, x3_wgs_per_cu(WGM * WGN) * WGM * WGN / 4) void sgemm_nt_bf16x3_kernel(const X3Params p) {
    static_assert(F16 || !(A32 || GMAX), "the on-load split and the group max belong to the f16 form");
    static_assert(!GMAX || (BM / WGM == 64 && !PLANES), "a group of 32 or 64 rows lies inside one wave's 64-row block");
    constexpr int NT = 64 * WGM * WGN, RP = NT / 4;
    constexpr int WM = BM / WGM, WN = BN / WGN;
    constexpr int TM = WM / 16, TN = WN / 16;
    constexpr int PA = BM * LROW, PB = BN * LROW;
    constexpr int NA = (BM + RP - 1) / RP, NB = (BN + RP - 1) / RP;
    constexpr int STAGE = 2 * (PA + PB);
    static_assert(WM % 16 == 0 && WN % 16 == 0 && BM % 16 == 0 && BN % 16 == 0, "whole 16 x 16 blocks per wave, whole waves per staging row test");
    __shared__ __attribute__((aligned(16))) unsigned short L[2 * STAGE];
    const int tid = threadIdx.x, lane = tid & 63, wave = tid >> 6;
    const int wm = wave / WGN, wn = wave % WGN;
    const int tiles_n = p.N / BN, tiles_m = p.M / BM;
    int wg = blockIdx.x;
    {
        const int nwg = tiles_m * tiles_n, q = nwg >> 3, r = nwg & 7, xcd = wg & 7, loc = wg >> 3;
        wg = (xcd < r ? xcd * (q + 1) : r * (q + 1) + (xcd - r) * q) + loc;
    }
    constexpr int GM = 8;
    const int per_group = GM * tiles_n, group = wg / per_group, first_m = group * GM;
    const int gsz = min(tiles_m - first_m, GM), in_group = wg - group * per_group;
    const int tile_m = first_m + in_group % gsz, tile_n = in_group / gsz;
    const int m0 = tile_m * BM, n0 = tile_n * BN;
    const int K = p.K, ntiles = K / BK, last = ntiles - 1;

    constexpr int X = F16 ? 1 : 0;
    f32x4 acc[X + 1][TM][TN];
#pragma unroll
    for (int x = 0; x <= X; ++x)
#pragma unroll
        for (int i = 0; i < TM; ++i)
#pragma unroll
            for (int j = 0; j < TN; ++j) acc[x][i][j] = f32x4{0.f, 0.f, 0.f, 0.f};

    const int srow = tid >> 2, sch = tid & 3;
    const int lda = p.lda;
    const size_t goa = (size_t)(m0 + srow) * lda + sch * 8, gob = (size_t)(n0 + srow) * K + sch * 8;
    const float* gA32[2] = {A32 ? p.A32 + goa : nullptr, A32 ? p.A32 + goa + 4 : nullptr};
    const unsigned short* gA[2] = {A32 ? nullptr : p.Ah + goa, A32 ? nullptr : p.Al + goa};
    const unsigned short* gB[2] = {p.Bh + gob, p.Bl + gob};
    u32x4v ra0[2][NA], rb0[2][NB], ra1[2][NA], rb1[2][NB];
    const int s_off = srow * LROW + sch * 8;
    const int r = lane & 15, g = lane >> 4;
    const int a_off = (wm * WM + r) * LROW + g * 8, b_off = (wn * WN + r) * LROW + g * 8;
    const long long ta = (long long)(min(srow + RP * (NA - 1), BM - 1) - srow) * lda, tb = (long long)(min(srow + RP * (NB - 1), BN - 1) - srow) * K;
    const float* Lf = reinterpret_cast<const float*>(L);
    const int sx_off = sch * 2 * (LROW / 2) + 16;
#define X3_WHOLE(I, ROWS) (RP * ((I) + 1) <= (ROWS))
#define X3_LOAD(RA, RB, T)                                                                                                             \
    _Pragma("unroll") for (int s_ = 0; s_ < 2; ++s_) {                                                                                 \
        _Pragma("unroll") for (int i_ = 0; i_ < NA; ++i_)                                                                              \
            if constexpr (A32)                                                                                                         \
                RA[s_][i_] = *reinterpret_cast<const u32x4v*>(gA32[s_] + (X3_WHOLE(i_, BM) ? (long long)(RP * i_) * lda : ta) + (T) * BK); \
            else                                                                                                                       \
                RA[s_][i_] = *reinterpret_cast<const u32x4v*>(gA[s_] + (X3_WHOLE(i_, BM) ? (long long)(RP * i_) * lda : ta) + (T) * BK); \
        _Pragma("unroll") for (int i_ = 0; i_ < NB; ++i_)                                                                              \
            RB[s_][i_] = *reinterpret_cast<const u32x4v*>(gB[s_] + (X3_WHOLE(i_, BN) ? (long long)(RP * i_) * K : tb) + (T) * BK);      \
    }
#define X3_STORE(RA, RB, STG, T)                                                                                                       \
    if constexpr (A32) {                                                                                                               \
        __builtin_amdgcn_sched_barrier(0);                                                                                             \
        _Pragma("unroll") for (int i_ = 0; i_ < NA; ++i_)                                                                              \
            if (X3_WHOLE(i_, BM) || srow + RP * i_ < BM) {                                                                             \
                u32x4v h1_, h2_;                                                                                                       \
                x3_affine_split8(RA[0][i_], RA[1][i_], Lf + sx_off + (T) * 8 * (LROW / 2), Lf + PA / 2 + sx_off + (T) * 8 * (LROW / 2), h1_, h2_); \
                *reinterpret_cast<u32x4v*>(&L[(STG) * STAGE + s_off + RP * i_ * LROW]) = h1_;                                          \
                *reinterpret_cast<u32x4v*>(&L[(STG) * STAGE + PA + s_off + RP * i_ * LROW]) = h2_;                                     \
            }                                                                                                                          \
    }                                                                                                                                  \
    _Pragma("unroll") for (int s_ = 0; s_ < 2; ++s_) {                                                                                 \
        _Pragma("unroll") for (int i_ = 0; i_ < NA; ++i_)                                                                              \
            if (!A32 && (X3_WHOLE(i_, BM) || srow + RP * i_ < BM))                                                                     \
                *reinterpret_cast<u32x4v*>(&L[(STG) * STAGE + s_ * PA + s_off + RP * i_ * LROW]) = RA[s_][i_];                         \
        _Pragma("unroll") for (int i_ = 0; i_ < NB; ++i_)                                                                              \
            if (X3_WHOLE(i_, BN) || srow + RP * i_ < BN)                                                                               \
                *reinterpret_cast<u32x4v*>(&L[(STG) * STAGE + 2 * PA + s_ * PB + s_off + RP * i_ * LROW]) = RB[s_][i_];                \
    }
#define X3_COMPUTE(STG)                                                                                                                \
    {                                                                                                                                  \
        const unsigned short* As_ = L + (STG) * STAGE; const unsigned short* Bs_ = As_ + 2 * PA;                                       \
        bf16x8 af[TM][2];                                                                                                              \
        _Pragma("unroll") for (int i_ = 0; i_ < TM; ++i_)                                                                              \
            _Pragma("unroll") for (int s_ = 0; s_ < 2; ++s_) af[i_][s_] = *reinterpret_cast<const bf16x8*>(&As_[s_ * PA + a_off + i_ * 16 * LROW]); \
        _Pragma("unroll") for (int j_ = 0; j_ < TN; ++j_) {                                                                            \
            bf16x8 bf[2];                                                                                                              \
            _Pragma("unroll") for (int s_ = 0; s_ < 2; ++s_) bf[s_] = *reinterpret_cast<const bf16x8*>(&Bs_[s_ * PB + b_off + j_ * 16 * LROW]); \
             \
             \
            _Pragma("unroll") for (int i_ = 0; i_ < TM; ++i_) acc[X][i_][j_] = x3_mfma<F16>(bf[0], af[i_][1], acc[X][i_][j_]);           \
            _Pragma("unroll") for (int i_ = 0; i_ < TM; ++i_) acc[X][i_][j_] = x3_mfma<F16>(bf[1], af[i_][0], acc[X][i_][j_]);           \
// ... 53 lines not shown
            for (int i = 0; i < TM; ++i) {
                const float4 v = value(i, j, m0 + wm * WM + i * 16 + r, col);
                float4& d = m[i / (TM / 2)];
                d.x = fmaxf(d.x, v.x); d.y = fmaxf(d.y, v.y); d.z = fmaxf(d.z, v.z); d.w = fmaxf(d.w, v.w);
            }
            if (p.group == 64) { m[0].x = fmaxf(m[0].x, m[1].x); m[0].y = fmaxf(m[0].y, m[1].y); m[0].z = fmaxf(m[0].z, m[1].z); m[0].w = fmaxf(m[0].w, m[1].w); }
#pragma unroll
            for (int h = 0; h < 2; ++h) {
                if (h == 1 && p.group == 64) break;
#pragma unroll
                for (int off = 1; off < 16; off <<= 1) {
                    m[h].x = fmaxf(m[h].x, __shfl_xor(m[h].x, off)); m[h].y = fmaxf(m[h].y, __shfl_xor(m[h].y, off));
                    m[h].z = fmaxf(m[h].z, __shfl_xor(m[h].z, off)); m[h].w = fmaxf(m[h].w, __shfl_xor(m[h].w, off));
                }
                if (r == 0) {
                    float* cp = p.C + (size_t)((m0 + wm * WM + h * 32) / p.group) * p.ldc + col;
                    if (vec) *reinterpret_cast<float4*>(cp) = m[h]; else { cp[0] = m[h].x; cp[1] = m[h].y; cp[2] = m[h].z; cp[3] = m[h].w; }
                }
            }
        }
        return;
    }
#pragma unroll
    for (int i = 0; i < TM; ++i)
#pragma unroll
        for (int j = 0; j < TN; ++j) {
            const int row = m0 + wm * WM + i * 16 + r;
            const int col = n0 + wn * WN + j * 16 + g * 4;
            const float4 v = value(i, j, row, col);
            if (!PLANES || p.C) {
                float* cp = p.C + (size_t)row * p.ldc + col;
                if (vec) *reinterpret_cast<float4*>(cp) = v; else { cp[0] = v.x; cp[1] = v.y; cp[2] = v.z; cp[3] = v.w; }
            }
            if constexpr (PLANES) store_planes4<F16>(p.Oh, p.Ol, ((size_t)row * p.N + col) >> 2, v, p.o_scale);
        }
}

template <int BM, int BN, int WGM, int WGN, bool F16>
int launch_x3(const X3Params& p, hipStream_t s) {
    const dim3 grid((p.M / BM) * (p.N / BN)), block(64 * WGM * WGN);
    const bool planes = p.Oh != nullptr;
    switch (p.epi.act) {
        case ACT_EPI_NONE:
            if (planes) hipLaunchKernelGGL((sgemm_nt_bf16x3_kernel<BM, BN, WGM, WGN, ACT_EPI_NONE, true, F16>), grid, block, 0, s, p);
            else        hipLaunchKernelGGL((sgemm_nt_bf16x3_kernel<BM, BN, WGM, WGN, ACT_EPI_NONE, false, F16>), grid, block, 0, s, p);
            break;
        case ACT_EPI_GELU:
            if (planes) hipLaunchKernelGGL((sgemm_nt_bf16x3_kernel<BM, BN, WGM, WGN, ACT_EPI_GELU, true, F16>), grid, block, 0, s, p);
            else        hipLaunchKernelGGL((sgemm_nt_bf16x3_kernel<BM, BN, WGM, WGN, ACT_EPI_GELU, false, F16>), grid, block, 0, s, p);
            break;
        case ACT_EPI_MUL_GELU_GRAD:
            if (planes) hipLaunchKernelGGL((sgemm_nt_bf16x3_kernel<BM, BN, WGM, WGN, ACT_EPI_MUL_GELU_GRAD, true, F16>), grid, block, 0, s, p);
            else        hipLaunchKernelGGL((sgemm_nt_bf16x3_kernel<BM, BN, WGM, WGN, ACT_EPI_MUL_GELU_GRAD, false, F16>), grid, block, 0, s, p);
            break;
        default: return ACT_E_BADARG;
    }
    ACT_LAUNCH_CHECK();
    return 0;
}

template <int BM, int BN, int WGM, int WGN>
int launch_x3_gmax(const X3Params& p, bool a32, hipStream_t s) {
    const dim3 grid((p.M / BM) * (p.N / BN)), block(64 * WGM * WGN);
    if (a32) hipLaunchKernelGGL((sgemm_nt_bf16x3_kernel<BM, BN, WGM, WGN, ACT_EPI_NONE, false, true, true, true>), grid, block, 0, s, p);
    else     hipLaunchKernelGGL((sgemm_nt_bf16x3_kernel<BM, BN, WGM, WGN, ACT_EPI_NONE, false, true, false, true>), grid, block, 0, s, p);
    ACT_LAUNCH_CHECK();
    return 0;
// ... 21 lines not shown
                                   act_stream_t stream) {
    return split_planes<true>(x, R, K, ldx, scale, row_scale, h1, h2, K, stream);
}
extern "C" int act_split_f16x2_ld_f32(const float* x, int R, int K, int ldx, float scale, uint16_t* h1, uint16_t* h2, int ldp, act_stream_t stream) {
    if (ldp & 7) return ACT_E_BADARG;
    return split_planes<true>(x, R, K, ldx, scale, nullptr, h1, h2, ldp, stream);
}

extern "C" int act_sgemm_nt_bf16x3_supported(int M, int N, int K) { return M > 0 && N > 0 && K > 0 && M % 128 == 0 && N % 128 == 0 && K % 64 == 0; }
extern "C" int act_sgemm_nt_f16x3_supported(int M, int N, int K) { return act_sgemm_nt_bf16x3_supported(M, N, K); }

extern "C" int act_sgemm_nt_f16x3_pick_tile(int M, int N, int K, int cus) {
    if (!act_sgemm_nt_f16x3_supported(M, N, K) || cus <= 0) return 0;
    if (N % 384) return 128;
    const long long t128 = (long long)(M / 128) * (N / 128), t192 = (long long)(M / 128) * (N / 192);
    const long long tail = t128 % (2 * cus);
    const long long c128 = t128 / (2 * cus) * 4 + (tail == 0 ? 0 : tail <= cus ? 2 : 4), c192 = (t192 + cus - 1) / cus * 3;
    return 8 * c192 <= 7 * c128 ? 192 : 128;
}

namespace {
int x3_cu_count() {
    static const int n = [] {
        int dev = 0, v = 0;
        if (hipGetDevice(&dev) != hipSuccess || hipDeviceGetAttribute(&v, hipDeviceAttributeMultiprocessorCount, dev) != hipSuccess || v <= 0) v = 256;
        return v;
    }();
    return n;
}
bool x3_only_128() {
    static const bool v = [] { const char* e = getenv("ACT_X3_TILE"); return e && atoi(e) == 128; }();
    return v;
}
template <bool F16>
int multiply_planes(int M, int N, int K, const uint16_t* a1, const uint16_t* a2, float a_scale, const uint16_t* b1, const uint16_t* b2, const float* b_inv,
                    float* C, int ldc, uint16_t* o1, uint16_t* o2, float out_scale, const act_gemm_epilogue_t* epilogue, act_stream_t stream, int tile,
                    int lda = 0) {
    if (lda == 0) lda = K;
    if (lda < K || (lda & 7)) return ACT_E_BADARG;
    if (!a1 || !a2 || !b1 || !b2 || (F16 && !b_inv) || (!C && !o1) || ((o1 == nullptr) != (o2 == nullptr))) return ACT_E_NULLPTR;
    if (!act_sgemm_nt_bf16x3_supported(M, N, K) || (C && ldc < N) || (F16 && (!(a_scale > 0.f) || (o1 && !(out_scale > 0.f))))) return ACT_E_BADARG;
    if ((((uintptr_t)a1 | (uintptr_t)a2 | (uintptr_t)b1 | (uintptr_t)b2 | (uintptr_t)o1 | (uintptr_t)o2 | (uintptr_t)b_inv) & 15)) return ACT_E_BADARG;
    if (F16 && tile != 0 && tile != 128 && !(tile == 192 && N % 192 == 0)) return ACT_E_BADARG;
    if (F16 && tile == 0) tile = x3_only_128() ? 128 : act_sgemm_nt_f16x3_pick_tile(M, N, K, x3_cu_count());
    X3Params p{};
    p.Ah = a1; p.Al = a2; p.Bh = b1; p.Bl = b2; p.C = C; p.ldc = ldc; p.M = M; p.N = N; p.K = K; p.Oh = o1; p.Ol = o2; p.lda = lda;
    if (F16) { p.b_inv = b_inv; p.a_inv = 1.0f / a_scale; p.o_scale = out_scale; }
    if (epilogue) p.epi = *epilogue; else { p.epi = act_gemm_epilogue_t{}; p.epi.alpha = 1.0f; }
    if (p.epi.accumulate || (p.epi.act != ACT_EPI_NONE && p.epi.act != ACT_EPI_GELU && p.epi.act != ACT_EPI_MUL_GELU_GRAD)) return ACT_E_BADARG;
    hipStream_t s = (hipStream_t)stream;
    ActProfScope ps(KID_GEMM_BF16X3, s, 2.0 * M * (double)N * K, 4.0 * ((double)M * K + (double)N * K + (double)M * N));
    if constexpr (F16) return tile == 192 ? launch_x3<128, 192, 2, 4, true>(p, s) : launch_x3<128, 128, 2, 2, true>(p, s);
    else return launch_x3<128, 128, 2, 2, false>(p, s);
}
}

extern "C" int act_split_f16x2_affine_relu_f32(const float* x, int R, int K, int ldx, const float* col_scale, const float* col_shift, float scale, uint16_t* h1,
                                               uint16_t* h2, act_stream_t stream) {
    if (!x || !col_scale || !col_shift || !h1 || !h2) return ACT_E_NULLPTR;
    if (R < 0 || K <= 0 || (K & 3) || ldx < K || (ldx & 3) || !(scale > 0.f)) return ACT_E_BADARG;
    if (((uintptr_t)x | (uintptr_t)h1 | (uintptr_t)h2 | (uintptr_t)col_scale | (uintptr_t)col_shift) & 15) return ACT_E_BADARG;
    const long long n4 = (long long)R * K / 4; if (n4 == 0) return 0;
    hipStream_t s = (hipStream_t)stream;
    ActProfScope ps(KID_ELTWISE, s, 0.0, 8.0 * R * (double)K);
    long long g = (n4 + 255) / 256; if (g > 8192) g = 8192;
    hipLaunchKernelGGL((split_planes_kernel<true, true>), dim3((unsigned)g), dim3(256), 0, s, x, K / 4, ldx, K / 4, n4, scale, nullptr, h1, h2, col_scale, col_shift);
    ACT_LAUNCH_CHECK(); return 0;
}
extern "C" int act_sgemm_nt_f16x3_gmax_supported(int M, int N, int K, int group) {
    return act_sgemm_nt_f16x3_supported(M, N, K) && K <= 512 && (group == 32 || group == 64);
}
extern "C" int act_sgemm_nt_f16x3_gmax_pick_tile(int M, int N, int K, int cus) { return act_sgemm_nt_f16x3_pick_tile(M, N, K, cus); }
extern "C" int act_sgemm_nt_f16x3_gmax_f32(int M, int N, int K, const float* A, int lda, const float* a_col_scale, const float* a_col_shift,
                                           const uint16_t* a_h1, const uint16_t* a_h2, float a_scale, const uint16_t* b_h1, const uint16_t* b_h2,
                                           const float* b_inv_scale, const float* bias, int group, float* out, int ldo, int tile, act_stream_t stream) {
    const bool a32 = A != nullptr;
    if (!b_h1 || !b_h2 || !b_inv_scale || !out || (a32 ? (!a_col_scale || !a_col_shift) : (!a_h1 || !a_h2))) return ACT_E_NULLPTR;
    if (!act_sgemm_nt_f16x3_gmax_supported(M, N, K, group) || ldo < N || !(a_scale > 0.f) || (a32 && (lda < K || (lda & 3)))) return ACT_E_BADARG;
    if (((uintptr_t)A | (uintptr_t)a_col_scale | (uintptr_t)a_col_shift | (uintptr_t)a_h1 | (uintptr_t)a_h2 | (uintptr_t)b_h1 | (uintptr_t)b_h2 |
         (uintptr_t)b_inv_scale) & 15) return ACT_E_BADARG;
    if (tile != 0 && tile != 128 && !(tile == 192 && N % 192 == 0)) return ACT_E_BADARG;
    if (tile == 0) tile = x3_only_128() ? 128 : act_sgemm_nt_f16x3_gmax_pick_tile(M, N, K, x3_cu_count());
    X3Params p{};
    p.A32 = A; p.lda = a32 ? lda : K; p.a_sc = a_col_scale; p.a_sh = a_col_shift; p.a_fold = a_scale; p.Ah = a_h1; p.Al = a_h2; p.Bh = b_h1; p.Bl = b_h2;
    p.C = out; p.ldc = ldo; p.M = M; p.N = N; p.K = K; p.group = group; p.b_inv = b_inv_scale; p.a_inv = 1.0f / a_scale;
    p.epi = act_gemm_epilogue_t{}; p.epi.alpha = 1.0f; p.epi.bias = bias;
    hipStream_t s = (hipStream_t)stream;
    ActProfScope ps(KID_GEMM_BF16X3, s, 2.0 * M * (double)N * K, 4.0 * ((double)M * K + (double)N * K + (double)(M / group) * N));
    return tile == 192 ? launch_x3_gmax<128, 192, 2, 4>(p, a32, s) : launch_x3_gmax<128, 128, 2, 2>(p, a32, s);
}

extern "C" int act_sgemm_nt_bf16x3_f32(int M, int N, int K, const uint16_t* a_hi, const uint16_t* a_lo, const uint16_t* b_hi, const uint16_t* b_lo,
                                       float* C, int ldc, const act_gemm_epilogue_t* epilogue, act_stream_t stream) {
    return multiply_planes<false>(M, N, K, a_hi, a_lo, 0.f, b_hi, b_lo, nullptr, C, ldc, nullptr, nullptr, 0.f, epilogue, stream, 128);
}
extern "C" int act_sgemm_nt_bf16x3_planes_f32(int M, int N, int K, const uint16_t* a_hi, const uint16_t* a_lo, const uint16_t* b_hi, const uint16_t* b_lo,
                                              float* C, int ldc, uint16_t* out_hi, uint16_t* out_lo, const act_gemm_epilogue_t* epilogue,
                                              act_stream_t stream) {
    return multiply_planes<false>(M, N, K, a_hi, a_lo, 0.f, b_hi, b_lo, nullptr, C, ldc, out_hi, out_lo, 0.f, epilogue, stream, 128);
}
extern "C" int act_sgemm_nt_f16x3_planes_f32(int M, int N, int K, const uint16_t* a_h1, const uint16_t* a_h2, float a_scale, const uint16_t* b_h1,
                                             const uint16_t* b_h2, const float* b_inv_scale, float* C, int ldc, uint16_t* out_h1, uint16_t* out_h2,
                                             float out_scale, const act_gemm_epilogue_t* epilogue, act_stream_t stream) {
    return multiply_planes<true>(M, N, K, a_h1, a_h2, a_scale, b_h1, b_h2, b_inv_scale, C, ldc, out_h1, out_h2, out_scale, epilogue, stream, 0);
}
extern "C" int act_sgemm_nt_f16x3_planes_tile_f32(int M, int N, int K, const uint16_t* a_h1, const uint16_t* a_h2, float a_scale, const uint16_t* b_h1,
                                                  const uint16_t* b_h2, const float* b_inv_scale, float* C, int ldc, uint16_t* out_h1, uint16_t* out_h2,
                                                  float out_scale, const act_gemm_epilogue_t* epilogue, act_stream_t stream, int tile) {
    return multiply_planes<true>(M, N, K, a_h1, a_h2, a_scale, b_h1, b_h2, b_inv_scale, C, ldc, out_h1, out_h2, out_scale, epilogue, stream, tile);
}
extern "C" int act_sgemm_nt_f16x3_planes_lda_f32(int M, int N, int K, const uint16_t* a_h1, const uint16_t* a_h2, int lda, float a_scale, const uint16_t* b_h1,
                                                 const uint16_t* b_h2, const float* b_inv_scale, float* C, int ldc, uint16_t* out_h1, uint16_t* out_h2,
                                                 float out_scale, const act_gemm_epilogue_t* epilogue, act_stream_t stream, int tile) {
    if (lda <= 0) return ACT_E_BADARG;
    return multiply_planes<true>(M, N, K, a_h1, a_h2, a_scale, b_h1, b_h2, b_inv_scale, C, ldc, out_h1, out_h2, out_scale, epilogue, stream, tile, lda);
}
```

### act_amd/kernels.py

```python
import ctypes
import os

import numpy as np

import torch

from . import _C
from ._abi import GemmEpilogue, GemmTnProblem

EPI_NONE, EPI_GELU, EPI_RELU, EPI_MUL_GELU_GRAD, EPI_MUL_RELU_MASK = 0, 1, 2, 3, 4

lib, ptr, stream, check = _C.lib, _C.ptr, _C.stream, _C.check

_WS = {}
_WS_BYTES = 160 << 20


def workspace(device, nbytes=_WS_BYTES, stream_handle=None):
    idx = device.index if device.index is not None else torch.cuda.current_device()
    key = (idx, _C.stream_handle(idx) if stream_handle is None else stream_handle)
    w = _WS.get(key)
    if w is None or w.numel() * 4 < nbytes:
        w = torch.empty(max(nbytes, _WS_BYTES) // 4, dtype=torch.float32, device=device)
        _WS[key] = w
# ... 174 lines not shown
    check(lib.act_split_f16x2_f32(_C.ptr_rows(x), R, Kd, x.stride(0), float(scale), ptr(_f32c(row_scale)) if row_scale is not None else None,
                                  ptr(out[0]), ptr(out[1]), stream()), "act_split_f16x2_f32")
    return out


def layernorm_f16_planes(x, gamma, beta, eps, scale, pos=None):
    x = _f32c(x)
    T, D = x.shape
    planes = torch.empty(2, T, D, dtype=torch.float16, device=x.device)
    check(lib.act_layernorm_fwd_f16_planes_f32(ptr(x), ptr(_f32c(pos)) if pos is not None else None, ptr(gamma), ptr(beta), None, None, ptr(planes[0]),
                                               ptr(planes[1]), float(scale), None, None, T, D, float(eps), stream()), "act_layernorm_fwd_f16_planes_f32")
    return planes


def gemm_nt_f16x3(a_planes, a_scale, b_planes, b_inv_scale, bias=None, act=EPI_NONE, res=None, out=None, planes_out=None, out_scale=1.0, tile=0):
    M, N, Kd, a1, a2, b1, b2, out, o1, o2, e = _x3_problem("gemm_nt_f16x3", torch.float16, a_planes, b_planes, bias, act, res, out, planes_out)
    b_inv_scale = _f32c(b_inv_scale)
    if b_inv_scale.numel() != N:
        raise _C.ActHipError("gemm_nt_f16x3: b_inv_scale must hold one value per row of b")
    check(lib.act_sgemm_nt_f16x3_planes_tile_f32(M, N, Kd, a1, a2, float(a_scale), b1, b2, ptr(b_inv_scale), ptr(out), out.stride(0), o1, o2, float(out_scale),
                                                 ctypes.byref(e), stream(), int(tile)), "act_sgemm_nt_f16x3_planes_tile_f32")
    return out


def split_f16x2_affine_relu(x, col_scale, col_shift, scale):
    x = _f32rows(x, "x")
    R, Kd = x.shape
    out = torch.empty(2, R, Kd, dtype=torch.float16, device=x.device)
    check(lib.act_split_f16x2_affine_relu_f32(_C.ptr_rows(x), R, Kd, x.stride(0), ptr(_f32c(col_scale)), ptr(_f32c(col_shift)), float(scale), ptr(out[0]),
                                              ptr(out[1]), stream()), "act_split_f16x2_affine_relu_f32")
    return out


def gemm_nt_f16x3_gmax(a, a_scale, b_planes, b_inv_scale, group, bias=None, col_scale=None, col_shift=None, tile=0):
    planes = a.dtype == torch.float16
    b_planes, b_inv_scale = b_planes.contiguous(), _f32c(b_inv_scale)
    N, Kd = b_planes.shape[1], b_planes.shape[2]
    if planes:
        a = a.contiguous()
        M = a.shape[1]
        args = (None, 0, None, None, ptr(a[0]), ptr(a[1]))
    else:
        a = _f32rows(a, "a")
        M = a.shape[0]
        args = (_C.ptr_rows(a), a.stride(0), ptr(_f32c(col_scale)), ptr(_f32c(col_shift)), None, None)
    if a.shape[-1] != Kd or b_inv_scale.numel() != N or M % int(group):
        raise _C.ActHipError("gemm_nt_f16x3_gmax: shapes do not match")
    out = torch.empty(M // int(group), N, dtype=torch.float32, device=a.device)
    check(lib.act_sgemm_nt_f16x3_gmax_f32(M, N, Kd, *args, float(a_scale), ptr(b_planes[0]), ptr(b_planes[1]), ptr(b_inv_scale),
                                          ptr(_f32c(bias)) if bias is not None else None, int(group), ptr(out), N, int(tile), stream()),
          "act_sgemm_nt_f16x3_gmax_f32")
    return out


_GEMM_CACHE = {}
AUTOTUNE = os.environ.get("ACT_GEMM_AUTOTUNE", "1") != "0"
AUTOTUNE_FULL = os.environ.get("ACT_GEMM_AUTOTUNE", "1") == "full"
_TUNE_FILE = os.environ.get("ACT_GEMM_TUNE_FILE") or os.path.join(os.path.dirname(os.path.abspath(__file__)), "gemm_tune_gfx950.json")
_GEMM_TABLE = {}
_MAX_SPLIT = int(os.environ.get("ACT_GEMM_MAX_SPLIT", "0"))
if os.environ.get("ACT_GEMM_TUNE_TABLE", "1") != "0" and os.path.exists(_TUNE_FILE):
    import json as _json
    with open(_TUNE_FILE) as _fh:
        _GEMM_TABLE = {tuple(int(v) for v in k.split(",")): tuple(c) for k, c in _json.load(_fh)["configs"].items()}
    if _MAX_SPLIT > 0:
        _GEMM_TABLE = {k: c for k, c in _GEMM_TABLE.items() if c[1] <= _MAX_SPLIT or k[4] > 8192}
_NEW_TUNED = {}
if os.environ.get("ACT_GEMM_TUNE_SAVE"):
    import atexit as _atexit

    def _dump_tuned(path=os.environ["ACT_GEMM_TUNE_SAVE"].replace("%p", str(os.getpid()))):
        import json
        merged = dict(_GEMM_TABLE); merged.update(_NEW_TUNED)
        with open(path, "w") as f:
            json.dump({"arch": "gfx950", "key": "a_kmajor,b_kmajor,M,N,K", "value": "[tile id, split-K]",
                       "configs": {",".join(str(v) for v in k): list(c) for k, c in sorted(merged.items())}}, f, indent=0)
    _atexit.register(_dump_tuned)


def stable_split(M, N, K, ws_bytes):
    nb = -(-M // 64) * -(-N // 64)
    if nb >= 384 or K < 1024:
        return 1
    s = max(1, min(8, K // 256, int(round(512.0 / nb))))
    while s > 1 and s * M * N * 4 > ws_bytes:
# ... 2471 lines not shown
```

### include/act_hip.h

```cpp
#ifndef ACT_HIP_H
#define ACT_HIP_H
#include <stdint.h>
#include <stddef.h>
#ifdef __cplusplus
extern "C" {
#endif

typedef void* act_stream_t;

#define ACT_E_BADARG   (-1)
#define ACT_E_NULLPTR  (-2)
#define ACT_E_UNSUPPORTED (-3)

int         act_version(void);
const char* act_arch(void);

int         act_prof_enable(int on);
int         act_prof_reset(void);
int         act_prof_num_kernels(void);
const char* act_prof_kernel_name(int id);
int         act_prof_read(int id, double* total_ms, long long* launches, double* flops, double* bytes);

size_t act_fps_scratch_floats(int B, int N);
int act_fps_f32(const float* xyz, int B, int N, int G, int32_t* idx_out, float* centers_out,
// ... 178 lines not shown
int act_gumbel_softmax_bwd_f32(const float* y, const float* dy, int R, int C, float tau, float* dlogits, act_stream_t stream);
int act_kl_uniform_fwd_f32(const float* logits, int B, int G, int C, float* lse, float* qbar, float* klv_out, act_stream_t stream);
int act_kl_uniform_bwd_f32(const float* logits, const float* lse, const float* qbar, const float* grad_klv, int B, int G, int C,
                           float* dlogits, act_stream_t stream);

int act_split_bf16x2_f32(const float* x, int R, int K, int ldx, uint16_t* hi, uint16_t* lo, act_stream_t stream);
int act_sgemm_nt_bf16x3_supported(int M, int N, int K);
int act_sgemm_nt_bf16x3_f32(int M, int N, int K, const uint16_t* a_hi, const uint16_t* a_lo, const uint16_t* b_hi, const uint16_t* b_lo,
                            float* C, int ldc, const act_gemm_epilogue_t* epilogue, act_stream_t stream);
int act_layernorm_fwd_planes_f32(const float* x, const float* pos, const float* gamma, const float* beta, float* xin_out, float* y,
                                 uint16_t* y_hi, uint16_t* y_lo, float* mean , float* rstd , int T, int D, float eps,
                                 act_stream_t stream);
int act_prompt_layernorm_fwd_planes_f32(const float* tok, const float* ppos, int B, int P, int D, float drop_p, uint64_t seed,
                                        const uint64_t* seed_dev, const float* gamma, const float* beta, float eps, uint16_t* y_hi, uint16_t* y_lo,
                                        act_stream_t stream);
int act_attention_fwd_prefix_planes_f32(const float* kv0, int S0, const float* qkv1, int Sq, float* out, uint16_t* out_hi, uint16_t* out_lo, float* lse,
                                        int B, int H, int head_dim, float scale, act_stream_t stream);
int act_sgemm_nt_bf16x3_planes_f32(int M, int N, int K, const uint16_t* a_hi, const uint16_t* a_lo, const uint16_t* b_hi, const uint16_t* b_lo,
                                   float* C, int ldc, uint16_t* out_hi, uint16_t* out_lo, const act_gemm_epilogue_t* epilogue, act_stream_t stream);

int act_split_f16x2_f32(const float* x, int R, int K, int ldx, float scale, const float* row_scale, uint16_t* h1, uint16_t* h2, act_stream_t stream);
int act_split_f16x2_ld_f32(const float* x, int R, int K, int ldx, float scale, uint16_t* h1, uint16_t* h2, int ldp, act_stream_t stream);
int act_sgemm_nt_f16x3_supported(int M, int N, int K);
int act_sgemm_nt_f16x3_planes_f32(int M, int N, int K, const uint16_t* a_h1, const uint16_t* a_h2, float a_scale, const uint16_t* b_h1,
                                  const uint16_t* b_h2, const float* b_inv_scale, float* C, int ldc, uint16_t* out_h1, uint16_t* out_h2, float out_scale,
                                  const act_gemm_epilogue_t* epilogue, act_stream_t stream);
int act_sgemm_nt_f16x3_pick_tile(int M, int N, int K, int cus);
int act_sgemm_nt_f16x3_planes_tile_f32(int M, int N, int K, const uint16_t* a_h1, const uint16_t* a_h2, float a_scale, const uint16_t* b_h1,
                                       const uint16_t* b_h2, const float* b_inv_scale, float* C, int ldc, uint16_t* out_h1, uint16_t* out_h2,
                                       float out_scale, const act_gemm_epilogue_t* epilogue, act_stream_t stream, int tile);
int act_sgemm_nt_f16x3_planes_lda_f32(int M, int N, int K, const uint16_t* a_h1, const uint16_t* a_h2, int lda, float a_scale, const uint16_t* b_h1,
                                      const uint16_t* b_h2, const float* b_inv_scale, float* C, int ldc, uint16_t* out_h1, uint16_t* out_h2,
                                      float out_scale, const act_gemm_epilogue_t* epilogue, act_stream_t stream, int tile);
int act_layernorm_fwd_f16_planes_f32(const float* x, const float* pos, const float* gamma, const float* beta, float* xin_out, float* y,
                                     uint16_t* y_h1, uint16_t* y_h2, float plane_scale, float* mean , float* rstd , int T, int D,
                                     float eps, act_stream_t stream);
int act_attention_fwd_prefix_f16_planes_f32(const float* kv0, int S0, const float* qkv1, int Sq, float* out, uint16_t* out_h1, uint16_t* out_h2,
                                            float plane_scale, float* lse, int B, int H, int head_dim, float scale, act_stream_t stream);
int act_prompt_layernorm_fwd_f16_planes_f32(const float* tok, const float* ppos, int B, int P, int D, float drop_p, uint64_t seed,
                                            const uint64_t* seed_dev, const float* gamma, const float* beta, float eps, uint16_t* y_h1, uint16_t* y_h2,
                                            float plane_scale, act_stream_t stream);
int act_split_f16x2_affine_relu_f32(const float* x, int R, int K, int ldx, const float* col_scale, const float* col_shift, float scale, uint16_t* h1,
                                    uint16_t* h2, act_stream_t stream);
int act_sgemm_nt_f16x3_gmax_supported(int M, int N, int K, int group);
int act_sgemm_nt_f16x3_gmax_pick_tile(int M, int N, int K, int cus);
int act_sgemm_nt_f16x3_gmax_f32(int M, int N, int K, const float* A, int lda, const float* a_col_scale, const float* a_col_shift, const uint16_t* a_h1,
                                const uint16_t* a_h2, float a_scale, const uint16_t* b_h1, const uint16_t* b_h2, const float* b_inv_scale,
                                const float* bias, int group, float* out, int ldo, int tile, act_stream_t stream);

int act_gemm_tune_set(int a_kmajor, int b_kmajor, int M, int N, int K, int tile, int splits);
int act_gemm_tune_get(int a_kmajor, int b_kmajor, int M, int N, int K, int* tile, int* splits);
int act_gemm_tune_clear(void);
#define ACT_GEMM_LAYOUT_TN 1
#define ACT_GEMM_LAYOUT_TT 2
#define ACT_GEMM_LAYOUT_NN 4
#define ACT_GEMM_LAYOUT_NT 8
#define ACT_GEMM_NEED_ANY           0
#define ACT_GEMM_NEED_FULL_OR_MTAIL 1
#define ACT_GEMM_NEED_FULL          2
#define ACT_GEMM_NEED_OFFSET32      4
int act_gemm_tile_info(int tile, int* bm, int* bn, int* layouts, int* need);

int act_scale_rows_f32(const float* x, const float* gate, int T, int D, int rows_per_scale, float* y, act_stream_t stream);
int act_bn_eval_affine_f32(const float* gamma, const float* beta, const float* running_mean, const float* running_var, float eps,
                           int C, float* scale, float* shift, act_stream_t stream);

int act_composite_collect_begin(void);
int act_composite_collect_end(int* shapes, int max);
int act_composite_shutdown(void);

typedef struct {
    const float *norm1_w, *norm1_b, *qkv_w, *qkv_b , *proj_w, *proj_b, *norm2_w, *norm2_b,
                *fc1_w, *fc1_b, *fc2_w, *fc2_b;
} act_block_params_t;
typedef struct {
    float *norm1_w, *norm1_b, *qkv_w, *qkv_b , *proj_w, *proj_b, *norm2_w, *norm2_b, *fc1_w, *fc1_b, *fc2_w, *fc2_b;
} act_block_grads_t;
typedef struct { int B, S, D, heads, hidden; float eps; } act_block_dims_t;

size_t act_block_saved_floats(const act_block_dims_t* d);
int act_block_fwd_f32(const act_block_dims_t* d, const act_block_params_t* w, const float* x, const float* pos,
// ... 5 lines not shown
                      float* workspace, size_t workspace_bytes, float* side_workspace, size_t side_workspace_bytes,
                      act_stream_t stream, act_stream_t side_stream);

typedef struct {
    int depth;
    const act_block_params_t* blocks;
    const float* const* gate1;
    const float* const* gate2;
} act_block_stack_t;
size_t act_block_stack_saved_floats(const act_block_dims_t* d, int depth, int keep_for_backward);
size_t act_block_stack_bwd_scratch_floats(const act_block_dims_t* d, int depth);
int act_block_stack_fwd_f32(const act_block_dims_t* d, const act_block_stack_t* st, const float* x, const float* pos, int keep_for_backward,
                            float* saved, float* out, float* workspace, size_t workspace_bytes, act_stream_t stream);
int act_block_stack_bwd_f32(const act_block_dims_t* d, const act_block_stack_t* st, const float* saved, const float* dout, float* dx, float* dpos,
                            const float* dpos_in, const act_block_grads_t* grads, float* scratch, float* workspace, size_t workspace_bytes, float* side_workspace,
                            size_t side_workspace_bytes, act_stream_t stream, act_stream_t side_stream);
int act_add_f32(const float* a, const float* b, float* out, long long n, act_stream_t stream);

size_t act_prefix_block_saved_floats(const act_block_dims_t* d, int P);
int act_prefix_block_fwd_f32(const act_block_dims_t* d, int P, const act_block_params_t* w, const float* x, const float* pos,
                             const float* prm, const float* n1p, int keep_for_backward, float* saved, float* out,
                             float* workspace, size_t workspace_bytes, act_stream_t stream);
int act_prefix_block_fwd_kv_f32(const act_block_dims_t* d, int P, const act_block_params_t* w, const float* x, const float* pos,
                                const float* kvp, float* saved, float* out, float* workspace, size_t workspace_bytes, act_stream_t stream);
int act_prompt_kv_sparse(int on );
size_t act_prompt_kv_workspace(int B, int P, int D, int N);
int act_prompt_kv_fwd_f32(const float* tok, const float* ppos, int B, int P, int D, int N, float drop_p, uint64_t seed,
                          const uint64_t* seed_dev, const float* gamma, const float* beta, float eps, const float* W, const float* bias,
                          float* kvp, float* scratch, size_t scratch_bytes, float* workspace, size_t workspace_bytes, act_stream_t stream);
int act_prompt_kv_f16x3(int on );
int act_prompt_kv_fwd_f16x3_f32(const float* tok, const float* ppos, int B, int P, int D, int N, float drop_p, uint64_t seed, const uint64_t* seed_dev,
                                const float* gamma, const float* beta, float eps, const uint16_t* w_h1, const uint16_t* w_h2, const float* w_inv,
                                float a_scale, const float* bias, float* kv, uint16_t* planes, size_t planes_elems, int tile, act_stream_t stream);
size_t act_prefix_block_bwd_scratch_floats(const act_block_dims_t* d, int P);
int act_prefix_block_bwd_f32(const act_block_dims_t* d, int P, const act_block_params_t* w, const float* prm, const float* saved,
                             const float* dout, float* dx, float* dprm, float* scratch, float* workspace, size_t workspace_bytes,
                             act_stream_t stream);

typedef struct {
    int B, P, G, D, heads, hidden, depth, tokens_dims, pos_hidden;
    float eps, drop_p;
    uint64_t seed_base;
    const uint64_t* seed_dev;
    const float *pos_w0, *pos_b0, *pos_w1, *pos_b1, *pre_w, *pre_b, *post_w, *post_b, *norm_w, *norm_b;
    const float* const* prompt_tok;
    const float* const* prompt_pos;
    const act_block_params_t* blocks;
} act_prefix_vit_t;
size_t act_prefix_vit_scratch_floats(const act_prefix_vit_t* m);
typedef struct {
    const uint16_t* const* w_planes;
    uint16_t* a_planes;
    size_t a_planes_elems;
} act_vit_bf16x3_t;
int act_prefix_vit_fwd_bf16x3_f32(const act_prefix_vit_t* m, const act_vit_bf16x3_t* x3, const float* tokens, const float* center, float* out,
                                  float* scratch, float* workspace, size_t workspace_bytes, act_stream_t stream);
int act_prefix_block_fwd_bf16x3_f32(const act_block_dims_t* d, int P, const act_block_params_t* w, const act_vit_bf16x3_t* x3, const float* x, const float* pos,
                                    const float* prm, int keep_for_backward, float* saved, float* out, float* workspace, size_t workspace_bytes,
                                    act_stream_t stream);
int act_prefix_block_bwd_bf16x3_f32(const act_block_dims_t* d, int P, const act_block_params_t* w, const act_vit_bf16x3_t* x3, const float* prm,
                                    const float* saved, const float* dout, float* dx, float* dprm, float* scratch, float* workspace,
                                    size_t workspace_bytes, act_stream_t stream);
int act_prefix_vit_fwd_f32(const act_prefix_vit_t* m, const float* tokens, const float* center, float* out, float* scratch,
                           float* workspace, size_t workspace_bytes, act_stream_t stream);
typedef struct {
    const uint16_t* const* w_planes;
    const float* const* w_inv_scale;
    const float* a_scale;
    uint16_t* a_planes;
    size_t a_planes_elems;
} act_vit_f16x3_t;
int act_prefix_vit_fwd_f16x3_f32(const act_prefix_vit_t* m, const act_vit_f16x3_t* x3, const float* tokens, const float* center, float* out,
                                 float* scratch, float* workspace, size_t workspace_bytes, act_stream_t stream);

typedef struct {
    const float *c1_w, *c1_b, *bn1_w, *bn1_b, *c2_w, *c2_b, *c3_w, *c3_b, *bn2_w, *bn2_b, *c4_w, *c4_b;
    float *bn1_mean, *bn1_var, *bn2_mean, *bn2_var;
} act_pointnet_params_t;
typedef struct { float *c1_w, *c1_b, *bn1_w, *bn1_b, *c2_w, *c2_b, *c3_w, *c3_b, *bn2_w, *bn2_b, *c4_w, *c4_b; } act_pointnet_grads_t;
typedef struct { int BG, n, C; float eps1, eps2, momentum1, momentum2; } act_pointnet_dims_t;
size_t act_pointnet_saved_floats(const act_pointnet_dims_t* d);
int act_pointnet_fwd_f32(const act_pointnet_dims_t* d, const act_pointnet_params_t* w, const float* x, int training,
                         int keep_for_backward, float* saved, float* out, float* workspace, size_t workspace_bytes,
                         act_stream_t stream);
int act_pointnet_fwd_groups_f32(const act_pointnet_dims_t* d, const act_pointnet_params_t* w, const float* x, int training, int keep_for_backward,
                                float* saved, float* out, const int32_t* groups, int n_groups, float* workspace, size_t workspace_bytes,
                                act_stream_t stream);
typedef struct {
    const uint16_t* c4_planes;
    const float* c4_inv_scale;
    float a_scale;
} act_pointnet_f16x3_t;
int act_pointnet_fwd_groups_f16x3_f32(const act_pointnet_dims_t* d, const act_pointnet_params_t* w, const act_pointnet_f16x3_t* x3, const float* x,
                                      int training, int keep_for_backward, float* saved, float* out, const int32_t* groups, int n_groups,
                                      float* workspace, size_t workspace_bytes, act_stream_t stream);
size_t act_pointnet_bwd_scratch_floats(const act_pointnet_dims_t* d);
int act_pointnet_bwd_f32(const act_pointnet_dims_t* d, const act_pointnet_params_t* w, const float* x, const float* saved,
                         const float* dout, const act_pointnet_grads_t* grads, float* scratch, float* workspace,
                         size_t workspace_bytes, act_stream_t stream);

typedef struct {
    int B, G, k, Cin, Cout, groups;
    float eps, slope;
    const float *w_in, *b_in, *w5;
    const float* stacked[4];
    const float* gn_w[4];
    const float* gn_b[4];
} act_dgcnn_t;
size_t act_dgcnn_scratch_floats(const act_dgcnn_t* m);
int act_dgcnn_features_f32(const act_dgcnn_t* m, const float* f, const int64_t* idx, float* h, float* scratch, float* workspace,
                           size_t workspace_bytes, act_stream_t stream);
typedef struct {
    const uint16_t* w5_planes;
    const float* w5_inv_scale;
    float a_scale;
    uint16_t* a_planes;
    size_t a_planes_elems;
    int layers;
    const uint16_t* st_planes[3];
    const float* st_inv_scale[3];
} act_dgcnn_f16x3_t;
int act_dgcnn_features_f16x3_f32(const act_dgcnn_t* m, const act_dgcnn_f16x3_t* x3, const float* f, const int64_t* idx, float* h, float* scratch,
                                 float* workspace, size_t workspace_bytes, act_stream_t stream);

int act_log_softmax_fwd_f32(const float* z, long long R, int C, float* out, act_stream_t stream);
int act_log_softmax_bwd_f32(const float* logp, const float* dout, long long R, int C, float* dz, act_stream_t stream);
size_t act_nll_weighted_workspace(long long R);
int act_nll_weighted_fwd_f32(const float* logp, const int64_t* target, const float* weight, long long R, int C, float* loss, float* wsum,
                             int64_t* correct, float* workspace, size_t workspace_bytes, act_stream_t stream);
int act_nll_weighted_bwd_f32(const int64_t* target, const float* weight, const float* wsum, const float* gloss, long long R, int C, float* dlogp,
                             act_stream_t stream);
int act_confusion_i64(const float* pred, const int64_t* target, long long R, int C, int64_t* cm, act_stream_t stream);

int act_label_branch_fwd_f32(const float* cls, const float* W, const float* gamma, const float* beta, int B, int training, float eps, float momentum,
                             float slope, float* running_mean, float* running_var, float* y, act_stream_t stream);
int act_label_branch_bwd_f32(const float* cls, const float* W, const float* gamma, const float* beta, const float* dy, int B, float eps, float slope,
                             float* dW, float* dgamma, float* dbeta, act_stream_t stream);
int act_part_eval_f32(const float* logp, const int64_t* target, int B, int N, int P, const int32_t* part2cat, const int32_t* cat_first, int ncat,
                      int32_t* pred, int32_t* counts, int shape_offset, int num_shapes, int64_t* seen, int64_t* correct, act_stream_t stream);

size_t act_scene_member_workspace(long long P, int gx, int gy);
int act_scene_member_count(const double* xyz, long long P, const double* table, int gx, int gy, int32_t* counts, int32_t* offsets, void* ws,
                           size_t ws_bytes, act_stream_t stream);
int act_scene_member_fill(const double* xyz, long long P, const double* table, int gx, int gy, const int32_t* offsets, int32_t* members, void* ws,
                          size_t ws_bytes, act_stream_t stream);
int act_scene_rows(const int32_t* members, const int32_t* member_off, const int32_t* block_ids, const int32_t* row_off, int nb, long long R,
                   int block_points, unsigned seed, unsigned room, unsigned vote, int32_t* rows, act_stream_t stream);
int act_scene_gather(const double* xyz, long long P, const double* table, const int32_t* rows, const int32_t* block_ids, const int32_t* row_off,
                     int nb, long long R, float* out, act_stream_t stream);
int act_scene_vote(const float* logp, const int32_t* rows, long long n, long long P, int C, const int32_t* label, const float* labelweights,
                   int32_t* votes, act_stream_t stream);
int act_scene_finish(const int32_t* votes, const int32_t* label, long long P, int C, int32_t* pred, int64_t* cm, act_stream_t stream);

// ... 159 lines not shown
```

Measured before the change: 7285.

## Add K-tiled weight and activation plane layout for f16x3 GEMMs

Adds a K-tiled layout (32-wide K blocks stored contiguously across rows) for the f16 split weight planes. Those planes are repacked once and cached. New layout-aware GEMM entry points are used in the ViT blocks (fc1/fc2 selected by a bitmask), DGCNN and prompt KV paths. The fc1 output planes can also be emitted in K-tiled form for fc2 to consume directly. The aim is more contiguous, coalesced global loads of B and A tiles in the GEMM inner loop, at the cost of a repack step, new kernel variants, alignment checks and extra cache keys.

Measured after the change: 7465, median of 6. 2.5% higher.

```diff
diff --git a/act_amd/_abi.py b/act_amd/_abi.py
--- a/act_amd/_abi.py
+++ b/act_amd/_abi.py
@@ -45,7 +45,7 @@
 
 
 class VitF16x3(ctypes.Structure):
-    _fields_ = [("w_planes", _vp), ("w_inv_scale", _vp), ("a_scale", _vp), ("a_planes", _vp), ("a_planes_elems", _sz)]
+    _fields_ = [("w_planes", _vp), ("w_inv_scale", _vp), ("a_scale", _vp), ("a_planes", _vp), ("a_planes_elems", _sz), ("w_layout", _i)]
 
 
 class PointnetParams(ctypes.Structure):
@@ -68,11 +68,11 @@
 
 class DgcnnF16x3(ctypes.Structure):
     _fields_ = [("w5_planes", _vp), ("w5_inv_scale", _vp), ("a_scale", _f), ("a_planes", _vp), ("a_planes_elems", _sz), ("layers", _i),
-                ("st_planes", _vp * 3), ("st_inv_scale", _vp * 3)]
+                ("st_planes", _vp * 3), ("st_inv_scale", _vp * 3), ("w_layout", _i)]
 
 
 class PointnetF16x3(ctypes.Structure):
-    _fields_ = [("c4_planes", _vp), ("c4_inv_scale", _vp), ("a_scale", _f)]
+    _fields_ = [("c4_planes", _vp), ("c4_inv_scale", _vp), ("a_scale", _f), ("w_layout", _i)]
 
 
 class AugmentOp(ctypes.Structure):
@@ -178,6 +178,10 @@
     "act_sgemm_nt_f16x3_pick_tile": [_i, _i, _i, _i],
     "act_sgemm_nt_f16x3_planes_tile_f32": [_i, _i, _i, _vp, _vp, _f, _vp, _vp, _vp, _vp, _i, _vp, _vp, _f, _epi, _vp, _i],
     "act_sgemm_nt_f16x3_planes_lda_f32": [_i, _i, _i, _vp, _vp, _i, _f, _vp, _vp, _vp, _vp, _i, _vp, _vp, _f, _epi, _vp, _i],
+    "act_repack_ktile_u16": [_vp, _vp, _i, _i, _vp],
+    "act_split_f16x2_kt_f32": [_vp, _i, _i, _i, _f, _vp, _vp, _i, _vp],
+    "act_sgemm_nt_f16x3_planes_layout_f32": [_i, _i, _i, _vp, _vp, _i, _i, _i, _f, _vp, _vp, _i, _i, _vp, _vp, _i, _vp, _vp, _f, _i, _epi, _vp, _i],
+    "act_x3_kt": [_i],
     "act_layernorm_fwd_f16_planes_f32": [_vp, _vp, _vp, _vp, _vp, _vp, _vp, _vp, _f, _vp, _vp, _i, _i, _f, _vp],
     "act_attention_fwd_prefix_f16_planes_f32": [_vp, _i, _vp, _i, _vp, _vp, _vp, _f, _vp, _i, _i, _i, _f, _vp],
     "act_prompt_layernorm_fwd_f16_planes_f32": [_vp, _vp, _i, _i, _i, _f, _u64, _vp, _vp, _vp, _f, _vp, _vp, _f, _vp],
@@ -185,6 +189,7 @@
     "act_sgemm_nt_f16x3_gmax_supported": [_i, _i, _i, _i],
     "act_sgemm_nt_f16x3_gmax_pick_tile": [_i, _i, _i, _i],
     "act_sgemm_nt_f16x3_gmax_f32": [_i, _i, _i, _vp, _i, _vp, _vp, _vp, _vp, _f, _vp, _vp, _vp, _vp, _i, _vp, _i, _i, _vp],
+    "act_sgemm_nt_f16x3_gmax_layout_f32": [_i, _i, _i, _vp, _i, _vp, _vp, _vp, _vp, _f, _vp, _vp, _i, _i, _vp, _vp, _i, _vp, _i, _i, _vp],
     "act_gemm_tune_set": [_i] * 7,
     "act_gemm_tune_get": [_i] * 5 + [_P(_i), _P(_i)],
     "act_gemm_tune_clear": [],
@@ -211,6 +216,7 @@
     "act_prompt_kv_fwd_f32": [_vp, _vp, _i, _i, _i, _i, _f, _u64, _vp, _vp, _vp, _f, _vp, _vp, _vp, _vp, _sz, _vp, _sz, _vp],
     "act_prompt_kv_f16x3": [_i],
     "act_prompt_kv_fwd_f16x3_f32": [_vp, _vp, _i, _i, _i, _i, _f, _u64, _vp, _vp, _vp, _f, _vp, _vp, _vp, _f, _vp, _vp, _vp, _sz, _i, _vp],
+    "act_prompt_kv_fwd_f16x3_layout_f32": [_vp, _vp, _i, _i, _i, _i, _f, _u64, _vp, _vp, _vp, _f, _vp, _vp, _i, _i, _vp, _f, _vp, _vp, _vp, _sz, _i, _vp],
     "act_prefix_block_bwd_scratch_floats": (_sz, [_dims, _i]),
     "act_prefix_block_bwd_f32": [_dims, _i, _blk, _vp, _vp, _vp, _vp, _vp, _vp, _vp, _sz, _vp],
     "act_prefix_vit_scratch_floats": (_sz, [_P(PrefixVit)]),
diff --git a/act_amd/composite.py b/act_amd/composite.py
--- a/act_amd/composite.py
+++ b/act_amd/composite.py
@@ -254,6 +254,8 @@
 TOKENIZER_F16X3 = os.environ.get("ACT_TOKENIZER_F16X3", "1") != "0"
 TOKENIZER_PN_F16X3 = os.environ.get("ACT_TOKENIZER_PN_F16X3", "1") != "0"
 TOKENIZER_DGCNN_F16X3 = os.environ.get("ACT_TOKENIZER_DGCNN_F16X3", "1") != "0"
+X3_KT_VIT = 0b1100
+X3_KT_PN = False
 DGCNN_F16X3_MIN_T = 4096
 _PN_F16 = weakref.WeakKeyDictionary()
 _DGCNN_F16 = weakref.WeakKeyDictionary()
@@ -524,13 +526,15 @@
 
 def _vit_f16_planes(tok, ts, depth, act_elems, dev):
     blk = ts[10:10 + _NPB * depth]
-    sig = tuple((t.data_ptr(), t._version) if t is not None else None for t in blk)
+    kt = X3_KT_VIT if K.x3_kt() else 0
+    sig = tuple((t.data_ptr(), t._version) if t is not None else None for t in blk) + (kt,)
     cache = _VIT_F16.get(tok)
     if cache is None or cache[0] != sig:
         ws_ = [ts[10 + _NPB * i + j] for i in range(depth) for j in (2, 4, 8, 10)]
         with torch.no_grad():
             scales = [K.f16x3_row_scales(w) for w in ws_]
             planes = [K.split_f16x2(w.detach(), 1.0, sc[0]) for w, sc in zip(ws_, scales)]
+            planes = [K.repack_ktile(pl) if (kt >> (j % 4)) & 1 else pl for j, pl in enumerate(planes)]
             inv = [sc[1].contiguous() for sc in scales]
             a_scale = [f16x3_act_scale(b) for b in f16x3_vit_bounds(ts, depth, ws_[0].shape[1]).flatten().tolist()]
         parr = (_vp * len(planes))(*[pl.data_ptr() for pl in planes])
@@ -539,7 +543,7 @@
         cache = _VIT_F16[tok] = (sig, planes, inv, a_scale, (parr, iarr, sarr))
     a_planes = torch.empty(2 * act_elems, dtype=torch.float16, device=dev)
     parr, iarr, sarr = cache[4]
-    x3 = VitF16x3(ctypes.cast(parr, _vp), ctypes.cast(iarr, _vp), ctypes.cast(sarr, _vp), a_planes.data_ptr(), a_planes.numel())
+    x3 = VitF16x3(ctypes.cast(parr, _vp), ctypes.cast(iarr, _vp), ctypes.cast(sarr, _vp), a_planes.data_ptr(), a_planes.numel(), cache[0][-1])
     return x3, (a_planes, cache)
 
 
@@ -600,13 +604,16 @@
 
 def _pointnet_f16_planes(enc, R):
     bn2, c4 = enc.second_conv[1], enc.second_conv[3]
-    sig = tuple((t.data_ptr(), t._version) for t in (c4.weight, bn2.weight, bn2.bias))
+    kt = bool(X3_KT_PN and K.x3_kt())
+    sig = tuple((t.data_ptr(), t._version) for t in (c4.weight, bn2.weight, bn2.bias)) + (kt,)
     cache = _PN_F16.get(enc)
     if cache is None or cache[0] != sig:
         with torch.no_grad():
             w = c4.weight.detach().reshape(c4.weight.shape[0], c4.weight.shape[1])
             scale, inv = K.f16x3_row_scales(w)
             planes = K.split_f16x2(w, 1.0, scale)
+            if kt:
+                planes = K.repack_ktile(planes)
             inv = inv.contiguous()
             gmax, bmax = torch.stack([bn2.weight.detach().double().abs().max(), bn2.bias.detach().double().abs().max()]).tolist()
         cache = _PN_F16[enc] = (sig, planes, inv, gmax, bmax, {})
@@ -614,7 +621,7 @@
     a_scale = scales.get(R)
     if a_scale is None:
         a_scale = scales[R] = f16x3_act_scale(f16x3_pointnet_bound(gmax, bmax, R))
-    return PointnetF16x3(planes.data_ptr(), inv.data_ptr(), a_scale), cache
+    return PointnetF16x3(planes.data_ptr(), inv.data_ptr(), a_scale, int(cache[0][-1])), cache
 
 
 def pointnet_forward(enc, point_groups, need=None):
@@ -680,7 +687,8 @@
     convs = [layer[0] for layer in (dg.layer2, dg.layer3, dg.layer4)]
     gns = [layer[1] for layer in (dg.layer1, dg.layer2, dg.layer3, dg.layer4)]
     w5 = dg.layer5[0].weight
-    sig = tuple((t.data_ptr(), t._version) for t in [w5] + [t for gn in gns for t in (gn.weight, gn.bias)] + [c.weight for c in convs])
+    kt = K.x3_kt()
+    sig = tuple((t.data_ptr(), t._version) for t in [w5] + [t for gn in gns for t in (gn.weight, gn.bias)] + [c.weight for c in convs]) + (kt,)
     cache = _DGCNN_F16.get(dg)
     if cache is None or cache[0] != sig:
         with torch.no_grad():
@@ -689,7 +697,8 @@
 
     def planes_of(w):
         scale, inv = K.f16x3_row_scales(w)
-        return K.split_f16x2(w, 1.0, scale), inv.contiguous()
+        planes = K.split_f16x2(w, 1.0, scale)
+        return (K.repack_ktile(planes) if kt else planes), inv.contiguous()
     if head and cache[1] is None:
         with torch.no_grad():
             cache[1], cache[2] = planes_of(w5.detach().reshape(w5.shape[0], w5.shape[1]))
@@ -702,6 +711,7 @@
         a_scale = scales[(G, k)] = f16x3_act_scale(f16x3_dgcnn_bound(gmax, bmax, couts, groups, G, k))
     a_planes = torch.empty(2 * T * sum(couts), dtype=torch.float16, device=dev)
     x3 = DgcnnF16x3(planes.data_ptr() if head else None, inv.data_ptr() if head else None, a_scale, a_planes.data_ptr(), a_planes.numel())
+    x3.w_layout = int(kt)
     if layers:
         x3.layers = 1
         for i, (p, v) in enumerate(st):
diff --git a/act_amd/csrc/composite.hip b/act_amd/csrc/composite.hip
--- a/act_amd/csrc/composite.hip
+++ b/act_amd/csrc/composite.hip
@@ -113,10 +113,16 @@
     return c.used;
 }
 
-struct X3Linear { const uint16_t *w1, *w2; const float* inv; PlaneFmt a_fmt; };
-inline X3Linear x3_linear_of(const uint16_t* planes, size_t plane_elems, PlaneFmt a_fmt, const float* inv = nullptr) {
-    return X3Linear{planes, planes ? planes + plane_elems : nullptr, inv, a_fmt};
-}
+struct X3Linear { const uint16_t *w1, *w2; const float* inv; PlaneFmt a_fmt; int layout = ACT_X3_ROWMAJOR, rows_total = 0; };
+inline X3Linear x3_linear_of(const uint16_t* planes, size_t plane_elems, PlaneFmt a_fmt, const float* inv = nullptr, int layout = ACT_X3_ROWMAJOR,
+                             int rows_total = 0) {
+    return X3Linear{planes, planes ? planes + plane_elems : nullptr, inv, a_fmt, layout, rows_total};
+}
+inline X3Linear x3_rows_from(const X3Linear& l, size_t r0, size_t K) {
+    const size_t o = l.layout == ACT_X3_KTILE ? r0 * 32 : r0 * K;
+    return X3Linear{l.w1 + o, l.w2 + o, l.inv ? l.inv + r0 : nullptr, l.a_fmt, l.layout, l.rows_total};
+}
+static std::atomic<int> g_x3_kt{[] { const char* e = getenv("ACT_X3_KT"); return !(e && e[0] == '0') ? 1 : 0; }()};
 inline bool x3_takes(const X3Linear& l, int M, int N, int K) {
     return l.w1 && (l.a_fmt.is_f16() ? act_sgemm_nt_f16x3_supported(M, N, K) : act_sgemm_nt_bf16x3_supported(M, N, K));
 }
@@ -125,18 +131,19 @@
     return act_split_bf16x2_f32(A, M, K, K, dst, dst + (size_t)M * K, s);
 }
 int x3_multiply(const X3Linear& l, int M, int N, int K, const uint16_t* a, float* C, uint16_t* emit, PlaneFmt emit_fmt, const act_gemm_epilogue_t& e,
-                hipStream_t s) {
+                hipStream_t s, bool a_kt = false, bool emit_kt = false) {
     const uint16_t* a2 = a + (size_t)M * K; uint16_t* emit2 = emit ? emit + (size_t)M * N : nullptr;
     if (l.a_fmt.is_f16())
-        return act_sgemm_nt_f16x3_planes_f32(M, N, K, a, a2, l.a_fmt.f16_scale, l.w1, l.w2, l.inv, emit ? nullptr : C, N, emit, emit2,
-                                             emit ? emit_fmt.f16_scale : 0.f, &e, s);
+        return act_sgemm_nt_f16x3_planes_layout_f32(M, N, K, a, a2, a_kt ? ACT_X3_KTILE : ACT_X3_ROWMAJOR, 0, M, l.a_fmt.f16_scale, l.w1, l.w2, l.layout,
+                                                    l.rows_total, l.inv, emit ? nullptr : C, N, emit, emit2, emit ? emit_fmt.f16_scale : 0.f,
+                                                    emit_kt ? ACT_X3_KTILE : ACT_X3_ROWMAJOR, &e, s, 0);
     return act_sgemm_nt_bf16x3_planes_f32(M, N, K, a, a2, l.w1, l.w2, emit ? nullptr : C, N, emit, emit2, &e, s);
 }
 int x3_linear(const X3Linear& l, int M, int N, int K, const float* A, const uint16_t* pre, uint16_t* stage, float* C, uint16_t* emit, PlaneFmt emit_fmt,
-              const act_gemm_epilogue_t& e, hipStream_t s) {
+              const act_gemm_epilogue_t& e, hipStream_t s, bool pre_kt = false, bool emit_kt = false) {
     if (t_collect) return 0;
     if (!pre) CK(x3_split(l.a_fmt, A, M, K, stage, s));
-    return x3_multiply(l, M, N, K, pre ? pre : stage, C, emit, emit_fmt, e, s);
+    return x3_multiply(l, M, N, K, pre ? pre : stage, C, emit, emit_fmt, e, s, pre && pre_kt, emit_kt);
 }
 int x3_layernorm(PlaneFmt fmt, const float* x, const float* pos, const float* gamma, const float* beta, float* xin_out, uint16_t* dst, float* mean, float* rstd,
                  int T, int D, float eps, hipStream_t s) {
@@ -177,9 +184,10 @@
     uint16_t* fc1_in = x3_takes(b.fc1, TG, Hd, D) ? tmp : nullptr;
     uint16_t* fc2_in = (fc1_in && x3_takes(b.fc2, TG, D, Hd)) ? b.a_planes : nullptr;
     const X3Linear fc2 = fc2_in ? b.fc2 : X3Linear{};
+    const bool hid_kt = fc2_in && fc2.layout == ACT_X3_KTILE && g_x3_kt.load() && ((uintptr_t)fc2_in & 127) == 0;
     auto linear = [&](const X3Linear& l, int M, int N, int K, const float* A, const float* W, float* C, const act_gemm_epilogue_t& e,
-                      const uint16_t* pre = nullptr, uint16_t* emit = nullptr, const X3Linear* next = nullptr) -> int {
-        if (x3_takes(l, M, N, K)) return x3_linear(l, M, N, K, A, pre, tmp, C, emit, next ? next->a_fmt : PlaneFmt::bf16(), e, s);
+                      const uint16_t* pre = nullptr, uint16_t* emit = nullptr, const X3Linear* next = nullptr, bool pre_kt = false, bool emit_kt = false) -> int {
+        if (x3_takes(l, M, N, K)) return x3_linear(l, M, N, K, A, pre, tmp, C, emit, next ? next->a_fmt : PlaneFmt::bf16(), e, s, pre_kt, emit_kt);
         return gemm_nt(M, N, K, A, K, W, K, C, N, e, ws, wsb, s);
     };
     float *mean1 = keep ? sv.mean1 : nullptr, *rstd1 = keep ? sv.rstd1 : nullptr, *mean2 = keep ? sv.mean2 : nullptr, *rstd2 = keep ? sv.rstd2 : nullptr;
@@ -198,9 +206,9 @@
     RUN(fc1_in ? x3_layernorm(b.fc1.a_fmt, sv.x1, nullptr, w.norm2_w, w.norm2_b, nullptr, fc1_in, mean2, rstd2, TG, D, d.eps, s)
                : act_layernorm_fwd_f32(sv.x1, nullptr, w.norm2_w, w.norm2_b, nullptr, sv.n2, mean2, rstd2, TG, D, d.eps, s));
     e = epi0(); e.bias = w.fc1_b; e.act = ACT_EPI_GELU; e.aux = keep ? sv.hpre : nullptr; e.ldaux = Hd;
-    CK(linear(b.fc1, TG, Hd, D, sv.n2, w.fc1_w, sv.a, e, fc1_in, fc2_in, &fc2));
+    CK(linear(b.fc1, TG, Hd, D, sv.n2, w.fc1_w, sv.a, e, fc1_in, fc2_in, &fc2, false, hid_kt));
     e = epi0(); e.bias = w.fc2_b; e.res = sv.x1; e.ldr = D;
-    CK(linear(fc2, TG, D, Hd, sv.a, w.fc2_w, out, e, fc2_in));
+    CK(linear(fc2, TG, D, Hd, sv.a, w.fc2_w, out, e, fc2_in, nullptr, nullptr, hid_kt));
     return 0;
 }
 
@@ -448,9 +456,17 @@
 
 static std::atomic<int> g_prompt_kv_f16x3{[] { const char* e = getenv("ACT_PROMPT_KV_F16X3"); return !(e && e[0] == '0') ? 1 : 0; }()};
 int act_prompt_kv_f16x3(int on) { return on < 0 ? g_prompt_kv_f16x3.load() : g_prompt_kv_f16x3.exchange(on ? 1 : 0); }
+int act_x3_kt(int on) { return on < 0 ? g_x3_kt.load() : g_x3_kt.exchange(on ? 1 : 0); }
 int act_prompt_kv_fwd_f16x3_f32(const float* tok, const float* ppos, int B, int P, int D, int N, float drop_p, uint64_t seed, const uint64_t* seed_dev,
                                 const float* gamma, const float* beta, float eps, const uint16_t* w_h1, const uint16_t* w_h2, const float* w_inv,
                                 float a_scale, const float* bias, float* kv, uint16_t* planes, size_t planes_elems, int tile, act_stream_t stream) {
+    return act_prompt_kv_fwd_f16x3_layout_f32(tok, ppos, B, P, D, N, drop_p, seed, seed_dev, gamma, beta, eps, w_h1, w_h2, ACT_X3_ROWMAJOR, 0, w_inv, a_scale, bias,
+                                              kv, planes, planes_elems, tile, stream);
+}
+int act_prompt_kv_fwd_f16x3_layout_f32(const float* tok, const float* ppos, int B, int P, int D, int N, float drop_p, uint64_t seed, const uint64_t* seed_dev,
+                                       const float* gamma, const float* beta, float eps, const uint16_t* w_h1, const uint16_t* w_h2, int w_layout,
+                                       int w_rows_total, const float* w_inv, float a_scale, const float* bias, float* kv, uint16_t* planes,
+                                       size_t planes_elems, int tile, act_stream_t stream) {
     if (B <= 0 || P <= 0 || D <= 0 || N <= 0) return ACT_E_BADARG;
     const size_t rows = (size_t)B * P;
     if (!g_prompt_kv_f16x3.load() || !(a_scale > 0.f) || !w_h1 || !w_h2 || !w_inv || !planes || planes_elems < 2 * rows * (size_t)D ||
@@ -458,12 +474,14 @@
         return ACT_E_UNSUPPORTED;
     if (!tok || !ppos || !gamma || !beta || !kv) return ACT_E_NULLPTR;
     if (drop_p < 0.f || drop_p >= 1.f || (tile != 0 && tile != 128 && !(tile == 192 && N % 192 == 0)) ||
-        (((uintptr_t)planes | (uintptr_t)w_h1 | (uintptr_t)w_h2 | (uintptr_t)w_inv) & 15))
+        (((uintptr_t)planes | (uintptr_t)w_h1 | (uintptr_t)w_h2 | (uintptr_t)w_inv) & 15) || (w_layout != ACT_X3_ROWMAJOR && w_layout != ACT_X3_KTILE) ||
+        (w_layout == ACT_X3_KTILE && (w_rows_total < N || (((uintptr_t)w_h1 | (uintptr_t)w_h2) & 127))))
         return ACT_E_BADARG;
     uint16_t* p2 = planes + rows * D;
     RUN(act_prompt_layernorm_fwd_f16_planes_f32(tok, ppos, B, P, D, drop_p, seed, seed_dev, gamma, beta, eps, planes, p2, a_scale, stream));
     act_gemm_epilogue_t e = epi0(); e.bias = bias;
-    RUN(act_sgemm_nt_f16x3_planes_tile_f32((int)rows, N, D, planes, p2, a_scale, w_h1, w_h2, w_inv, kv, N, nullptr, nullptr, 0.f, &e, stream, tile));
+    RUN(act_sgemm_nt_f16x3_planes_layout_f32((int)rows, N, D, planes, p2, ACT_X3_ROWMAJOR, 0, 0, a_scale, w_h1, w_h2, w_layout, w_rows_total, w_inv, kv, N, nullptr,
+                                             nullptr, 0.f, ACT_X3_ROWMAJOR, &e, stream, tile));
     return 0;
 }
 
@@ -577,6 +595,7 @@
 int act_prefix_vit_fwd_f16x3_f32(const act_prefix_vit_t* m, const act_vit_f16x3_t* h3, const float* tokens, const float* center, float* out,
                                  float* scratch, float* ws, size_t wsb, act_stream_t stream) {
     if (!h3 || !h3->w_planes || !h3->w_inv_scale || !h3->a_scale || !h3->a_planes) return ACT_E_NULLPTR;
+    if (h3->w_layout & ~15) return ACT_E_BADARG;
     return prefix_vit_fwd(m, nullptr, h3, tokens, center, out, scratch, ws, wsb, stream);
 }
 static int prefix_vit_fwd(const act_prefix_vit_t* m, const act_vit_bf16x3_t* x3, const act_vit_f16x3_t* h3, const float* tokens, const float* center, float* out,
@@ -603,20 +622,22 @@
         X3Block hb{};
         if (h3) {
             hb.a_planes = h3->a_planes; hb.a_elems = h3->a_planes_elems;
-            const size_t sD = D, sHd = m->hidden, elems[4] = {3 * sD * sD, sD * sD, sHd * sD, sD * sHd};
+            const size_t sD = D, sHd = m->hidden, elems[4] = {3 * sD * sD, sD * sD, sHd * sD, sD * sHd}, kdim[4] = {sD, sD, sD, sHd};
             X3Linear* lin[4] = {&hb.qkv, &hb.proj, &hb.fc1, &hb.fc2};
             for (int j = 0; j < 4; ++j) {
                 const float sa = h3->a_scale[4 * i + j];
                 if (sa > 0.f && h3->w_planes[4 * i + j] && h3->w_inv_scale[4 * i + j])
-                    *lin[j] = x3_linear_of(h3->w_planes[4 * i + j], elems[j], PlaneFmt::f16(sa), h3->w_inv_scale[4 * i + j]);
+                    *lin[j] = x3_linear_of(h3->w_planes[4 * i + j], elems[j], PlaneFmt::f16(sa), h3->w_inv_scale[4 * i + j],
+                                           (h3->w_layout >> j) & 1 ? ACT_X3_KTILE : ACT_X3_ROWMAJOR, (int)(elems[j] / kdim[j]));
             }
-            if (hb.qkv.w1) hb.kv = X3Linear{hb.qkv.w1 + sD * sD, hb.qkv.w2 + sD * sD, hb.qkv.inv + sD, hb.qkv.a_fmt};
+            if (hb.qkv.w1) hb.kv = x3_rows_from(hb.qkv, sD, sD);
         }
         if (h3 && !x3) {
             uint16_t* tp = x3_fits(d, m->P, hb.a_elems) ? hb.a_planes + (size_t)2 * TG * m->hidden : nullptr;
-            const int rc = act_prompt_kv_fwd_f16x3_f32(m->prompt_tok[i], m->prompt_pos[i], m->B, m->P, D, 2 * D, m->drop_p, seed, m->seed_dev, w.norm1_w, w.norm1_b,
-                                                       m->eps, hb.kv.w1, hb.kv.w2, hb.kv.inv, hb.kv.a_fmt.f16_scale, w.qkv_b ? w.qkv_b + D : nullptr, sv.kvp, tp,
-                                                       tp ? hb.a_elems - (size_t)2 * TG * m->hidden : 0, kPromptKvTile, stream);
+            const int rc = act_prompt_kv_fwd_f16x3_layout_f32(m->prompt_tok[i], m->prompt_pos[i], m->B, m->P, D, 2 * D, m->drop_p, seed, m->seed_dev, w.norm1_w, w.norm1_b,
+                                                              m->eps, hb.kv.w1, hb.kv.w2, hb.kv.layout, hb.kv.rows_total, hb.kv.inv, hb.kv.a_fmt.f16_scale,
+                                                              w.qkv_b ? w.qkv_b + D : nullptr, sv.kvp, tp, tp ? hb.a_elems - (size_t)2 * TG * m->hidden : 0,
+                                                              kPromptKvTile, stream);
             if (rc == 0) {
                 (void)collecting(1, 1, m->B * m->P, 2 * D, D);
                 CK(prefix_block_core(d, m->P, w, cur, pos, nullptr, false, sv, nxt, ws, wsb, s, &hb, true));
@@ -798,8 +819,8 @@
     if (x3 && x3->c4_planes && x3->c4_inv_scale && x3->a_scale > 0.f && !keep_for_backward && !groups && C % 128 == 0 &&
         act_sgemm_nt_f16x3_gmax_supported(R, C, 512, n)) {
         if (collecting(1, 1, R, C, 512)) return 0;
-        return act_sgemm_nt_f16x3_gmax_f32(R, C, 512, sv.h3, 512, scale2, shift2, nullptr, nullptr, x3->a_scale, x3->c4_planes,
-                                           x3->c4_planes + (size_t)C * 512, x3->c4_inv_scale, w->c4_b, n, out, C, 0, s);
+        return act_sgemm_nt_f16x3_gmax_layout_f32(R, C, 512, sv.h3, 512, scale2, shift2, nullptr, nullptr, x3->a_scale, x3->c4_planes,
+                                                  x3->c4_planes + (size_t)C * 512, x3->w_layout, C, x3->c4_inv_scale, w->c4_b, n, out, C, 0, s);
     }
     {
         act_gemm_fx_t fx{}; fx.a_scale = scale2; fx.a_shift = shift2; fx.gmax = out; fx.garg = keep_for_backward ? sv.arg2 : nullptr; fx.group = n; fx.store_c = 0;
@@ -895,7 +916,7 @@
     return 0;
 }
 
-static const int kDgcnnCin[4] = {128, 256, 512, 512}, kDgcnnCout[4] = {256, 512, 512, 1024};
+static constexpr int kDgcnnCin[4] = {128, 256, 512, 512}, kDgcnnCout[4] = {256, 512, 512, 1024};
 static size_t carve_dgcnn(float* base, const act_dgcnn_t& m, float*& x0, float*& yz, float*& cat, float*& stats) {
     const size_t T = (size_t)m.B * m.G;
     Carver c(base);
@@ -933,29 +954,37 @@
                       (layers || !x3->layers);
     uint16_t* const ap1 = planes_ok ? x3->a_planes : nullptr;
     uint16_t* const ap2 = planes_ok ? x3->a_planes + (size_t)T * 2304 : nullptr;
+    const bool cat_kt = layers && x3->w_layout == ACT_X3_KTILE && g_x3_kt.load() && ((uintptr_t)x3->a_planes & 127) == 0;
+    static_assert(kDgcnnCout[0] % 64 == 0 && kDgcnnCout[1] % 64 == 0 && kDgcnnCout[2] % 64 == 0 && kDgcnnCout[3] % 64 == 0, "slice offsets on whole K-tile pairs");
+    const int w_layout = planes_ok ? x3->w_layout : ACT_X3_ROWMAJOR;
+    if (w_layout != ACT_X3_ROWMAJOR && w_layout != ACT_X3_KTILE) return ACT_E_BADARG;
     act_gemm_epilogue_t e = epi0(); e.bias = m->b_in;
     CK(gemm_nt(T, 128, m->Cin, f, m->Cin, m->w_in, m->Cin, x0, 128, e, ws, wsb, s));
     const float* xin = x0; int ldx = 128, off = 0;
     for (int l = 0; l < 4; ++l) {
         const int cin = kDgcnnCin[l], cout = kDgcnnCout[l];
         if (layers && l > 0 && !t_collect) {
-            const size_t prev = (size_t)(off - cin);
+            const size_t prev = cat_kt ? (size_t)((off - cin) / 32) * T * 32 : (size_t)(off - cin);
             const uint16_t* w1 = x3->st_planes[l - 1];
             const act_gemm_epilogue_t e0 = epi0();
-            RUN(act_sgemm_nt_f16x3_planes_lda_f32(T, 2 * cout, cin, ap1 + prev, ap2 + prev, 2304, x3->a_scale, w1, w1 + (size_t)2 * cout * cin,
-                                                  x3->st_inv_scale[l - 1], yz, 2 * cout, nullptr, nullptr, 0.f, &e0, s, 0));
+            RUN(act_sgemm_nt_f16x3_planes_layout_f32(T, 2 * cout, cin, ap1 + prev, ap2 + prev, cat_kt ? ACT_X3_KTILE : ACT_X3_ROWMAJOR, 2304, T, x3->a_scale, w1,
+                                                     w1 + (size_t)2 * cout * cin, w_layout, 2 * cout, x3->st_inv_scale[l - 1], yz, 2 * cout, nullptr, nullptr, 0.f,
+                                                     ACT_X3_ROWMAJOR, &e0, s, 0));
         } else {
             CK(gemm_nt(T, 2 * cout, cin, xin, ldx, m->stacked[l], cin, yz, 2 * cout, epi0(), ws, wsb, s));
         }
         RUN(act_edge_gn_lrelu_max_f32(yz, 2 * cout, cout, idx, m->B, m->G, m->k, cout, m->groups, m->gn_w[l], m->gn_b[l], m->eps, m->slope, stats,
                                      cat, 2304, off, s));
-        if (layers && (l < 3 || head) && !t_collect)
-            RUN(act_split_f16x2_ld_f32(cat + off, T, cout, 2304, x3->a_scale, ap1 + off, ap2 + off, 2304, s));
+        if (layers && (l < 3 || head) && !t_collect) {
+            const size_t o = (size_t)(off / 32) * T * 32;
+            RUN(cat_kt ? act_split_f16x2_kt_f32(cat + off, T, cout, 2304, x3->a_scale, ap1 + o, ap2 + o, T, s)
+                       : act_split_f16x2_ld_f32(cat + off, T, cout, 2304, x3->a_scale, ap1 + off, ap2 + off, 2304, s));
+        }
         xin = cat + off; ldx = 2304; off += cout;
     }
     if (head) {
-        const X3Linear w5 = x3_linear_of(x3->w5_planes, (size_t)m->Cout * 2304, PlaneFmt::f16(x3->a_scale), x3->w5_inv_scale);
-        return x3_linear(w5, T, m->Cout, 2304, cat, layers ? x3->a_planes : nullptr, x3->a_planes, h, nullptr, w5.a_fmt, epi0(), s);
+        const X3Linear w5 = x3_linear_of(x3->w5_planes, (size_t)m->Cout * 2304, PlaneFmt::f16(x3->a_scale), x3->w5_inv_scale, w_layout, m->Cout);
+        return x3_linear(w5, T, m->Cout, 2304, cat, layers ? x3->a_planes : nullptr, x3->a_planes, h, nullptr, w5.a_fmt, epi0(), s, cat_kt);
     }
     CK(gemm_nt(T, m->Cout, 2304, cat, 2304, m->w5, 2304, h, m->Cout, epi0(), ws, wsb, s));
     return 0;
diff --git a/act_amd/csrc/gemm_bf16x3.hip b/act_amd/csrc/gemm_bf16x3.hip
--- a/act_amd/csrc/gemm_bf16x3.hip
+++ b/act_amd/csrc/gemm_bf16x3.hip
@@ -17,11 +17,12 @@
 template <bool F16, bool AFF = false>
 __global__ __launch_bounds__(256) void split_planes_kernel(const float* __restrict__ x, int K4, int ldx, int ldp4, long long n4, float scale,
                                                            const float* __restrict__ row_scale, unsigned short* __restrict__ p1, unsigned short* __restrict__ p2,
-                                                           const float* __restrict__ col_scale = nullptr, const float* __restrict__ col_shift = nullptr) {
+                                                           const float* __restrict__ col_scale = nullptr, const float* __restrict__ col_shift = nullptr,
+                                                           int kt_rows = 0) {
     for (long long i = (long long)blockIdx.x * blockDim.x + threadIdx.x; i < n4; i += (long long)gridDim.x * blockDim.x) {
         const long long row = i / K4; const int c4 = (int)(i - row * K4);
         const float4 v = *reinterpret_cast<const float4*>(x + row * ldx + c4 * 4);
-        const size_t o4 = (size_t)(row * ldp4 + c4);
+        const size_t o4 = kt_rows ? ((size_t)(c4 >> 3) * kt_rows + row) * 8 + (c4 & 7) : (size_t)(row * ldp4 + c4);
         if constexpr (AFF) {
             const float4 sc = x3_scale4(*reinterpret_cast<const float4*>(col_scale + c4 * 4), scale), sh = x3_scale4(*reinterpret_cast<const float4*>(col_shift + c4 * 4), scale);
             store_planes4<F16>(p1, p2, o4, x3_affine_relu4(v, sc, sh), 1.0f);
@@ -32,6 +33,15 @@
 }
 
 constexpr int BK = 32;
+
+constexpr long long x3_kt_index(long long r, long long k, long long rows) { return ((k / BK) * rows + r) * BK + k % BK; }
+
+__global__ __launch_bounds__(256) void repack_ktile_kernel(const u32x4v* __restrict__ src, u32x4v* __restrict__ dst, int R, int K8, long long n8) {
+    for (long long i = (long long)blockIdx.x * blockDim.x + threadIdx.x; i < n8; i += (long long)gridDim.x * blockDim.x) {
+        const long long row = i / K8; const int c8 = (int)(i - row * K8);
+        dst[((long long)(c8 >> 2) * R + row) * 4 + (c8 & 3)] = src[i];
+    }
+}
 constexpr int LROW = 40;
 
 struct X3Params {
@@ -42,6 +52,8 @@
     act_gemm_epilogue_t epi;
     const float* b_inv; float a_inv, o_scale;
     const float *A32, *a_sc, *a_sh; int lda; float a_fold;
+    int ldb, kta, ktb;
+    int o_kt;
     int group;
 };
 
@@ -105,8 +117,9 @@
             for (int j = 0; j < TN; ++j) acc[x][i][j] = f32x4{0.f, 0.f, 0.f, 0.f};
 
     const int srow = tid >> 2, sch = tid & 3;
-    const int lda = p.lda;
-    const size_t goa = (size_t)(m0 + srow) * lda + sch * 8, gob = (size_t)(n0 + srow) * K + sch * 8;
+    const int lda = p.lda, ldb = p.ldb;
+    const long long kta = p.kta, ktb = p.ktb;
+    const size_t goa = (size_t)(m0 + srow) * lda + sch * 8, gob = (size_t)(n0 + srow) * ldb + sch * 8;
     const float* gA32[2] = {A32 ? p.A32 + goa : nullptr, A32 ? p.A32 + goa + 4 : nullptr};
     const unsigned short* gA[2] = {A32 ? nullptr : p.Ah + goa, A32 ? nullptr : p.Al + goa};
     const unsigned short* gB[2] = {p.Bh + gob, p.Bl + gob};
@@ -114,7 +127,7 @@
     const int s_off = srow * LROW + sch * 8;
     const int r = lane & 15, g = lane >> 4;
     const int a_off = (wm * WM + r) * LROW + g * 8, b_off = (wn * WN + r) * LROW + g * 8;
-    const long long ta = (long long)(min(srow + RP * (NA - 1), BM - 1) - srow) * lda, tb = (long long)(min(srow + RP * (NB - 1), BN - 1) - srow) * K;
+    const long long ta = (long long)(min(srow + RP * (NA - 1), BM - 1) - srow) * lda, tb = (long long)(min(srow + RP * (NB - 1), BN - 1) - srow) * ldb;
     const float* Lf = reinterpret_cast<const float*>(L);
     const int sx_off = sch * 2 * (LROW / 2) + 16;
 #define X3_WHOLE(I, ROWS) (RP * ((I) + 1) <= (ROWS))
@@ -122,11 +135,11 @@
     _Pragma("unroll") for (int s_ = 0; s_ < 2; ++s_) {                                                                                 \
         _Pragma("unroll") for (int i_ = 0; i_ < NA; ++i_)                                                                              \
             if constexpr (A32)                                                                                                         \
-                RA[s_][i_] = *reinterpret_cast<const u32x4v*>(gA32[s_] + (X3_WHOLE(i_, BM) ? (long long)(RP * i_) * lda : ta) + (T) * BK); \
+                RA[s_][i_] = *reinterpret_cast<const u32x4v*>(gA32[s_] + (X3_WHOLE(i_, BM) ? (long long)(RP * i_) * lda : ta) + (T) * kta); \
             else                                                                                                                       \
-                RA[s_][i_] = *reinterpret_cast<const u32x4v*>(gA[s_] + (X3_WHOLE(i_, BM) ? (long long)(RP * i_) * lda : ta) + (T) * BK); \
+                RA[s_][i_] = *reinterpret_cast<const u32x4v*>(gA[s_] + (X3_WHOLE(i_, BM) ? (long long)(RP * i_) * lda : ta) + (T) * kta); \
         _Pragma("unroll") for (int i_ = 0; i_ < NB; ++i_)                                                                              \
-            RB[s_][i_] = *reinterpret_cast<const u32x4v*>(gB[s_] + (X3_WHOLE(i_, BN) ? (long long)(RP * i_) * K : tb) + (T) * BK);      \
+            RB[s_][i_] = *reinterpret_cast<const u32x4v*>(gB[s_] + (X3_WHOLE(i_, BN) ? (long long)(RP * i_) * ldb : tb) + (T) * ktb);   \
     }
 #define X3_STORE(RA, RB, STG, T)                                                                                                       \
     if constexpr (A32) {                                                                                                               \
@@ -246,7 +259,8 @@
                 float* cp = p.C + (size_t)row * p.ldc + col;
                 if (vec) *reinterpret_cast<float4*>(cp) = v; else { cp[0] = v.x; cp[1] = v.y; cp[2] = v.z; cp[3] = v.w; }
             }
-            if constexpr (PLANES) store_planes4<F16>(p.Oh, p.Ol, ((size_t)row * p.N + col) >> 2, v, p.o_scale);
+            if constexpr (PLANES)
+                store_planes4<F16>(p.Oh, p.Ol, (p.o_kt ? ((size_t)(col >> 5) * p.M + row) * BK + (col & 31) : (size_t)row * p.N + col) >> 2, v, p.o_scale);
         }
 }
 
@@ -334,19 +348,32 @@
     static const bool v = [] { const char* e = getenv("ACT_X3_TILE"); return e && atoi(e) == 128; }();
     return v;
 }
+struct X3Layout { int layout = ACT_X3_ROWMAJOR, ld = 0, rows_total = 0; };
+bool x3_strides(const X3Layout& l, int rows, int K, const uint16_t* p1, const uint16_t* p2, int& ld, int& kt) {
+    if (l.layout == ACT_X3_KTILE) {
+        if (l.rows_total < rows || (long long)l.rows_total * BK > 0x7fffffffLL || (((uintptr_t)p1 | (uintptr_t)p2) & 127)) return false;
+        ld = BK; kt = l.rows_total * BK; return true;
+    }
+    if (l.layout != ACT_X3_ROWMAJOR) return false;
+    ld = l.ld ? l.ld : K; kt = BK;
+    return ld >= K && !(ld & 7);
+}
+
 template <bool F16>
 int multiply_planes(int M, int N, int K, const uint16_t* a1, const uint16_t* a2, float a_scale, const uint16_t* b1, const uint16_t* b2, const float* b_inv,
                     float* C, int ldc, uint16_t* o1, uint16_t* o2, float out_scale, const act_gemm_epilogue_t* epilogue, act_stream_t stream, int tile,
-                    int lda = 0) {
-    if (lda == 0) lda = K;
-    if (lda < K || (lda & 7)) return ACT_E_BADARG;
+                    const X3Layout& la = X3Layout{}, const X3Layout& lb = X3Layout{}, int out_layout = ACT_X3_ROWMAJOR) {
+    int lda, ldb, kta, ktb;
+    if (!x3_strides(la, M, K, a1, a2, lda, kta) || !x3_strides(lb, N, K, b1, b2, ldb, ktb)) return ACT_E_BADARG;
+    if (out_layout != ACT_X3_ROWMAJOR && (out_layout != ACT_X3_KTILE || !F16 || (((uintptr_t)o1 | (uintptr_t)o2) & 127))) return ACT_E_BADARG;
     if (!a1 || !a2 || !b1 || !b2 || (F16 && !b_inv) || (!C && !o1) || ((o1 == nullptr) != (o2 == nullptr))) return ACT_E_NULLPTR;
     if (!act_sgemm_nt_bf16x3_supported(M, N, K) || (C && ldc < N) || (F16 && (!(a_scale > 0.f) || (o1 && !(out_scale > 0.f))))) return ACT_E_BADARG;
     if ((((uintptr_t)a1 | (uintptr_t)a2 | (uintptr_t)b1 | (uintptr_t)b2 | (uintptr_t)o1 | (uintptr_t)o2 | (uintptr_t)b_inv) & 15)) return ACT_E_BADARG;
     if (F16 && tile != 0 && tile != 128 && !(tile == 192 && N % 192 == 0)) return ACT_E_BADARG;
     if (F16 && tile == 0) tile = x3_only_128() ? 128 : act_sgemm_nt_f16x3_pick_tile(M, N, K, x3_cu_count());
     X3Params p{};
-    p.Ah = a1; p.Al = a2; p.Bh = b1; p.Bl = b2; p.C = C; p.ldc = ldc; p.M = M; p.N = N; p.K = K; p.Oh = o1; p.Ol = o2; p.lda = lda;
+    p.Ah = a1; p.Al = a2; p.Bh = b1; p.Bl = b2; p.C = C; p.ldc = ldc; p.M = M; p.N = N; p.K = K; p.Oh = o1; p.Ol = o2;
+    p.lda = lda; p.ldb = ldb; p.kta = kta; p.ktb = ktb; p.o_kt = out_layout == ACT_X3_KTILE;
     if (F16) { p.b_inv = b_inv; p.a_inv = 1.0f / a_scale; p.o_scale = out_scale; }
     if (epilogue) p.epi = *epilogue; else { p.epi = act_gemm_epilogue_t{}; p.epi.alpha = 1.0f; }
     if (p.epi.accumulate || (p.epi.act != ACT_EPI_NONE && p.epi.act != ACT_EPI_GELU && p.epi.act != ACT_EPI_MUL_GELU_GRAD)) return ACT_E_BADARG;
@@ -373,10 +400,13 @@
     return act_sgemm_nt_f16x3_supported(M, N, K) && K <= 512 && (group == 32 || group == 64);
 }
 extern "C" int act_sgemm_nt_f16x3_gmax_pick_tile(int M, int N, int K, int cus) { return act_sgemm_nt_f16x3_pick_tile(M, N, K, cus); }
-extern "C" int act_sgemm_nt_f16x3_gmax_f32(int M, int N, int K, const float* A, int lda, const float* a_col_scale, const float* a_col_shift,
-                                           const uint16_t* a_h1, const uint16_t* a_h2, float a_scale, const uint16_t* b_h1, const uint16_t* b_h2,
-                                           const float* b_inv_scale, const float* bias, int group, float* out, int ldo, int tile, act_stream_t stream) {
+extern "C" int act_sgemm_nt_f16x3_gmax_layout_f32(int M, int N, int K, const float* A, int lda, const float* a_col_scale, const float* a_col_shift,
+                                                  const uint16_t* a_h1, const uint16_t* a_h2, float a_scale, const uint16_t* b_h1, const uint16_t* b_h2,
+                                                  int b_layout, int b_rows_total, const float* b_inv_scale, const float* bias, int group, float* out, int ldo,
+                                                  int tile, act_stream_t stream) {
     const bool a32 = A != nullptr;
+    int ldb, ktb;
+    if (!x3_strides(X3Layout{b_layout, 0, b_rows_total}, N, K, b_h1, b_h2, ldb, ktb)) return ACT_E_BADARG;
     if (!b_h1 || !b_h2 || !b_inv_scale || !out || (a32 ? (!a_col_scale || !a_col_shift) : (!a_h1 || !a_h2))) return ACT_E_NULLPTR;
     if (!act_sgemm_nt_f16x3_gmax_supported(M, N, K, group) || ldo < N || !(a_scale > 0.f) || (a32 && (lda < K || (lda & 3)))) return ACT_E_BADARG;
     if (((uintptr_t)A | (uintptr_t)a_col_scale | (uintptr_t)a_col_shift | (uintptr_t)a_h1 | (uintptr_t)a_h2 | (uintptr_t)b_h1 | (uintptr_t)b_h2 |
@@ -384,12 +414,20 @@
     if (tile != 0 && tile != 128 && !(tile == 192 && N % 192 == 0)) return ACT_E_BADARG;
     if (tile == 0) tile = x3_only_128() ? 128 : act_sgemm_nt_f16x3_gmax_pick_tile(M, N, K, x3_cu_count());
     X3Params p{};
+    p.ldb = ldb; p.kta = BK; p.ktb = ktb;
     p.A32 = A; p.lda = a32 ? lda : K; p.a_sc = a_col_scale; p.a_sh = a_col_shift; p.a_fold = a_scale; p.Ah = a_h1; p.Al = a_h2; p.Bh = b_h1; p.Bl = b_h2;
     p.C = out; p.ldc = ldo; p.M = M; p.N = N; p.K = K; p.group = group; p.b_inv = b_inv_scale; p.a_inv = 1.0f / a_scale;
     p.epi = act_gemm_epilogue_t{}; p.epi.alpha = 1.0f; p.epi.bias = bias;
     hipStream_t s = (hipStream_t)stream;
     ActProfScope ps(KID_GEMM_BF16X3, s, 2.0 * M * (double)N * K, 4.0 * ((double)M * K + (double)N * K + (double)(M / group) * N));
     return tile == 192 ? launch_x3_gmax<128, 192, 2, 4>(p, a32, s) : launch_x3_gmax<128, 128, 2, 2>(p, a32, s);
+}
+
+extern "C" int act_sgemm_nt_f16x3_gmax_f32(int M, int N, int K, const float* A, int lda, const float* a_col_scale, const float* a_col_shift,
+                                           const uint16_t* a_h1, const uint16_t* a_h2, float a_scale, const uint16_t* b_h1, const uint16_t* b_h2,
+                                           const float* b_inv_scale, const float* bias, int group, float* out, int ldo, int tile, act_stream_t stream) {
+    return act_sgemm_nt_f16x3_gmax_layout_f32(M, N, K, A, lda, a_col_scale, a_col_shift, a_h1, a_h2, a_scale, b_h1, b_h2, ACT_X3_ROWMAJOR, 0, b_inv_scale, bias,
+                                              group, out, ldo, tile, stream);
 }
 
 extern "C" int act_sgemm_nt_bf16x3_f32(int M, int N, int K, const uint16_t* a_hi, const uint16_t* a_lo, const uint16_t* b_hi, const uint16_t* b_lo,
@@ -415,5 +453,37 @@
                                                  const uint16_t* b_h2, const float* b_inv_scale, float* C, int ldc, uint16_t* out_h1, uint16_t* out_h2,
                                                  float out_scale, const act_gemm_epilogue_t* epilogue, act_stream_t stream, int tile) {
     if (lda <= 0) return ACT_E_BADARG;
-    return multiply_planes<true>(M, N, K, a_h1, a_h2, a_scale, b_h1, b_h2, b_inv_scale, C, ldc, out_h1, out_h2, out_scale, epilogue, stream, tile, lda);
-}
+    return multiply_planes<true>(M, N, K, a_h1, a_h2, a_scale, b_h1, b_h2, b_inv_scale, C, ldc, out_h1, out_h2, out_scale, epilogue, stream, tile,
+                                 X3Layout{ACT_X3_ROWMAJOR, lda, 0});
+}
+extern "C" int act_sgemm_nt_f16x3_planes_layout_f32(int M, int N, int K, const uint16_t* a_h1, const uint16_t* a_h2, int a_layout, int lda, int a_rows_total,
+                                                    float a_scale, const uint16_t* b_h1, const uint16_t* b_h2, int b_layout, int b_rows_total,
+                                                    const float* b_inv_scale, float* C, int ldc, uint16_t* out_h1, uint16_t* out_h2, float out_scale,
+                                                    int out_layout, const act_gemm_epilogue_t* epilogue, act_stream_t stream, int tile) {
+    if (lda < 0) return ACT_E_BADARG;
+    return multiply_planes<true>(M, N, K, a_h1, a_h2, a_scale, b_h1, b_h2, b_inv_scale, C, ldc, out_h1, out_h2, out_scale, epilogue, stream, tile,
+                                 X3Layout{a_layout, lda, a_rows_total}, X3Layout{b_layout, 0, b_rows_total}, out_layout);
+}
+
+extern "C" int act_repack_ktile_u16(const uint16_t* src, uint16_t* dst, int R, int K, act_stream_t stream) {
+    if (!src || !dst) return ACT_E_NULLPTR;
+    if (R < 0 || K <= 0 || (K % BK) || src == dst || (((uintptr_t)src | (uintptr_t)dst) & 15)) return ACT_E_BADARG;
+    const long long n8 = (long long)R * K / 8; if (n8 == 0) return 0;
+    hipStream_t s = (hipStream_t)stream;
+    ActProfScope ps(KID_ELTWISE, s, 0.0, 4.0 * R * (double)K);
+    long long g = (n8 + 255) / 256; if (g > 8192) g = 8192;
+    hipLaunchKernelGGL(repack_ktile_kernel, dim3((unsigned)g), dim3(256), 0, s, reinterpret_cast<const u32x4v*>(src), reinterpret_cast<u32x4v*>(dst), R, K / 8, n8);
+    ACT_LAUNCH_CHECK(); return 0;
+}
+extern "C" int act_split_f16x2_kt_f32(const float* x, int R, int K, int ldx, float scale, uint16_t* h1, uint16_t* h2, int rows_total, act_stream_t stream) {
+    if (!x || !h1 || !h2) return ACT_E_NULLPTR;
+    if (R < 0 || K <= 0 || (K % BK) || ldx < K || (ldx & 3) || !(scale > 0.f) || rows_total < R || (long long)rows_total * BK > 0x7fffffffLL ||
+        ((uintptr_t)x & 15) || (((uintptr_t)h1 | (uintptr_t)h2) & 127))
+        return ACT_E_BADARG;
+    const long long n4 = (long long)R * K / 4; if (n4 == 0) return 0;
+    hipStream_t s = (hipStream_t)stream;
+    ActProfScope ps(KID_ELTWISE, s, 0.0, 8.0 * R * (double)K);
+    long long g = (n4 + 255) / 256; if (g > 8192) g = 8192;
+    hipLaunchKernelGGL(split_planes_kernel<true>, dim3((unsigned)g), dim3(256), 0, s, x, K / 4, ldx, K / 4, n4, scale, nullptr, h1, h2, nullptr, nullptr, rows_total);
+    ACT_LAUNCH_CHECK(); return 0;
+}
diff --git a/act_amd/kernels.py b/act_amd/kernels.py
--- a/act_amd/kernels.py
+++ b/act_amd/kernels.py
@@ -230,7 +230,7 @@
     return out
 
 
-def gemm_nt_f16x3_gmax(a, a_scale, b_planes, b_inv_scale, group, bias=None, col_scale=None, col_shift=None, tile=0):
+def gemm_nt_f16x3_gmax(a, a_scale, b_planes, b_inv_scale, group, bias=None, col_scale=None, col_shift=None, tile=0, b_layout=0):
     planes = a.dtype == torch.float16
     b_planes, b_inv_scale = b_planes.contiguous(), _f32c(b_inv_scale)
     N, Kd = b_planes.shape[1], b_planes.shape[2]
@@ -245,10 +245,63 @@
     if a.shape[-1] != Kd or b_inv_scale.numel() != N or M % int(group):
         raise _C.ActHipError("gemm_nt_f16x3_gmax: shapes do not match")
     out = torch.empty(M // int(group), N, dtype=torch.float32, device=a.device)
-    check(lib.act_sgemm_nt_f16x3_gmax_f32(M, N, Kd, *args, float(a_scale), ptr(b_planes[0]), ptr(b_planes[1]), ptr(b_inv_scale),
-                                          ptr(_f32c(bias)) if bias is not None else None, int(group), ptr(out), N, int(tile), stream()),
-          "act_sgemm_nt_f16x3_gmax_f32")
+    check(lib.act_sgemm_nt_f16x3_gmax_layout_f32(M, N, Kd, *args, float(a_scale), ptr(b_planes[0]), ptr(b_planes[1]), int(b_layout), N, ptr(b_inv_scale),
+                                                 ptr(_f32c(bias)) if bias is not None else None, int(group), ptr(out), N, int(tile), stream()),
+          "act_sgemm_nt_f16x3_gmax_layout_f32")
     return out
+
+
+X3_ROWMAJOR, X3_KTILE = 0, 1
+X3_BK = 32
+
+
+def ktile_index(r, k, rows_total):
+    return ((k // X3_BK) * rows_total + r) * X3_BK + k % X3_BK
+
+
+def ktile_rows(kt, R, Kd):
+    return kt.reshape(Kd // X3_BK, R, X3_BK).permute(1, 0, 2).reshape(R, Kd)
+
+
+def x3_kt(on=None):
+    return bool(lib.act_x3_kt(-1 if on is None else int(bool(on))))
+
+
+def repack_ktile(planes):
+    planes = planes.contiguous()
+    R, Kd = planes.shape[-2:]
+    if planes.element_size() != 2 or Kd % X3_BK:
+        raise _C.ActHipError("repack_ktile: 16-bit planes with K % 32 == 0 expected")
+    out = torch.empty_like(planes)
+    src, dst = planes.reshape(-1, R, Kd), out.view(-1, R, Kd)
+    for i in range(src.shape[0]):
+        check(lib.act_repack_ktile_u16(ptr(src[i]), ptr(dst[i]), R, Kd, stream()), "act_repack_ktile_u16")
+    return out
+
+
+def split_f16x2_kt(x, scale=1.0, out=None, rows_total=None):
+    x = _f32rows(x, "x")
+    R, Kd = x.shape
+    rows_total = R if rows_total is None else int(rows_total)
+    if out is None:
+        out = torch.empty(2, rows_total, Kd, dtype=torch.float16, device=x.device)
+    check(lib.act_split_f16x2_kt_f32(_C.ptr_rows(x), R, Kd, x.stride(0), float(scale), ptr(out[0]), ptr(out[1]), rows_total, stream()), "act_split_f16x2_kt_f32")
+    return out
+
+
+def gemm_nt_f16x3_layout(M, N, Kd, a, a_scale, b, b_inv_scale, a_layout=0, lda=0, a_rows_total=0, b_layout=0, b_rows_total=0, bias=None, act=EPI_NONE,
+                         res=None, out=None, want_c=True, planes_out=None, out_scale=1.0, out_layout=0, tile=0):
+    b_inv_scale = _f32c(b_inv_scale)
+    if want_c and out is None:
+        out = torch.empty(M, N, dtype=torch.float32, device=a[0].device)
+    e = GemmEpilogue(alpha=1.0, act=act, accumulate=0, rows_per_scale=0, ldr=(res.stride(0) if res is not None else 0), ldaux=0, res_row_div=0,
+                     bias=ptr(bias), rowscale=None, res=ptr(res), aux=None)
+    o1, o2 = (ptr(planes_out[0]), ptr(planes_out[1])) if planes_out is not None else (None, None)
+    check(lib.act_sgemm_nt_f16x3_planes_layout_f32(M, N, Kd, ptr(a[0]), ptr(a[1]), int(a_layout), int(lda), int(a_rows_total), float(a_scale), ptr(b[0]), ptr(b[1]),
+                                                   int(b_layout), int(b_rows_total), ptr(b_inv_scale), ptr(out) if want_c else None,
+                                                   out.stride(0) if want_c else N, o1, o2, float(out_scale), int(out_layout), ctypes.byref(e), stream(),
+                                                   int(tile)), "act_sgemm_nt_f16x3_planes_layout_f32")
+    return out if want_c else planes_out
 
 
 _GEMM_CACHE = {}
diff --git a/include/act_hip.h b/include/act_hip.h
--- a/include/act_hip.h
+++ b/include/act_hip.h
@@ -234,6 +234,14 @@
 int act_sgemm_nt_f16x3_planes_lda_f32(int M, int N, int K, const uint16_t* a_h1, const uint16_t* a_h2, int lda, float a_scale, const uint16_t* b_h1,
                                       const uint16_t* b_h2, const float* b_inv_scale, float* C, int ldc, uint16_t* out_h1, uint16_t* out_h2,
                                       float out_scale, const act_gemm_epilogue_t* epilogue, act_stream_t stream, int tile);
+enum { ACT_X3_ROWMAJOR = 0, ACT_X3_KTILE = 1 };
+int act_repack_ktile_u16(const uint16_t* src, uint16_t* dst, int R, int K, act_stream_t stream);
+int act_split_f16x2_kt_f32(const float* x, int R, int K, int ldx, float scale, uint16_t* h1, uint16_t* h2, int rows_total, act_stream_t stream);
+int act_sgemm_nt_f16x3_planes_layout_f32(int M, int N, int K, const uint16_t* a_h1, const uint16_t* a_h2, int a_layout, int lda, int a_rows_total,
+                                         float a_scale, const uint16_t* b_h1, const uint16_t* b_h2, int b_layout, int b_rows_total,
+                                         const float* b_inv_scale, float* C, int ldc, uint16_t* out_h1, uint16_t* out_h2, float out_scale,
+                                         int out_layout, const act_gemm_epilogue_t* epilogue, act_stream_t stream, int tile);
+int act_x3_kt(int on );
 int act_layernorm_fwd_f16_planes_f32(const float* x, const float* pos, const float* gamma, const float* beta, float* xin_out, float* y,
                                      uint16_t* y_h1, uint16_t* y_h2, float plane_scale, float* mean , float* rstd , int T, int D,
                                      float eps, act_stream_t stream);
@@ -249,6 +257,9 @@
 int act_sgemm_nt_f16x3_gmax_f32(int M, int N, int K, const float* A, int lda, const float* a_col_scale, const float* a_col_shift, const uint16_t* a_h1,
                                 const uint16_t* a_h2, float a_scale, const uint16_t* b_h1, const uint16_t* b_h2, const float* b_inv_scale,
                                 const float* bias, int group, float* out, int ldo, int tile, act_stream_t stream);
+int act_sgemm_nt_f16x3_gmax_layout_f32(int M, int N, int K, const float* A, int lda, const float* a_col_scale, const float* a_col_shift, const uint16_t* a_h1,
+                                       const uint16_t* a_h2, float a_scale, const uint16_t* b_h1, const uint16_t* b_h2, int b_layout, int b_rows_total,
+                                       const float* b_inv_scale, const float* bias, int group, float* out, int ldo, int tile, act_stream_t stream);
 
 int act_gemm_tune_set(int a_kmajor, int b_kmajor, int M, int N, int K, int tile, int splits);
 int act_gemm_tune_get(int a_kmajor, int b_kmajor, int M, int N, int K, int* tile, int* splits);
@@ -320,6 +331,10 @@
 int act_prompt_kv_fwd_f16x3_f32(const float* tok, const float* ppos, int B, int P, int D, int N, float drop_p, uint64_t seed, const uint64_t* seed_dev,
                                 const float* gamma, const float* beta, float eps, const uint16_t* w_h1, const uint16_t* w_h2, const float* w_inv,
                                 float a_scale, const float* bias, float* kv, uint16_t* planes, size_t planes_elems, int tile, act_stream_t stream);
+int act_prompt_kv_fwd_f16x3_layout_f32(const float* tok, const float* ppos, int B, int P, int D, int N, float drop_p, uint64_t seed, const uint64_t* seed_dev,
+                                       const float* gamma, const float* beta, float eps, const uint16_t* w_h1, const uint16_t* w_h2, int w_layout,
+                                       int w_rows_total, const float* w_inv, float a_scale, const float* bias, float* kv, uint16_t* planes,
+                                       size_t planes_elems, int tile, act_stream_t stream);
 size_t act_prefix_block_bwd_scratch_floats(const act_block_dims_t* d, int P);
 int act_prefix_block_bwd_f32(const act_block_dims_t* d, int P, const act_block_params_t* w, const float* prm, const float* saved,
                              const float* dout, float* dx, float* dprm, float* scratch, float* workspace, size_t workspace_bytes,
@@ -357,6 +372,7 @@
     const float* a_scale;
     uint16_t* a_planes;
     size_t a_planes_elems;
+    int w_layout;
 } act_vit_f16x3_t;
 int act_prefix_vit_fwd_f16x3_f32(const act_prefix_vit_t* m, const act_vit_f16x3_t* x3, const float* tokens, const float* center, float* out,
                                  float* scratch, float* workspace, size_t workspace_bytes, act_stream_t stream);
@@ -378,6 +394,7 @@
     const uint16_t* c4_planes;
     const float* c4_inv_scale;
     float a_scale;
+    int w_layout;
 } act_pointnet_f16x3_t;
 int act_pointnet_fwd_groups_f16x3_f32(const act_pointnet_dims_t* d, const act_pointnet_params_t* w, const act_pointnet_f16x3_t* x3, const float* x,
                                       int training, int keep_for_backward, float* saved, float* out, const int32_t* groups, int n_groups,
@@ -407,6 +424,7 @@
     int layers;
     const uint16_t* st_planes[3];
     const float* st_inv_scale[3];
+    int w_layout;
 } act_dgcnn_f16x3_t;
 int act_dgcnn_features_f16x3_f32(const act_dgcnn_t* m, const act_dgcnn_f16x3_t* x3, const float* f, const int64_t* idx, float* h, float* scratch,
                                  float* workspace, size_t workspace_bytes, act_stream_t stream);
```
